# sephiroce/srf

Hardware: AMD Instinct MI355X
Metric: acoustic frames/sec through SRF (123-d fbank, 3-iter DR) at 1/2/4/8 MI355X (higher is better)
Workload: dtype fp32; 1 GPU; wsj_c4: SRF L=6 PH=CH=16 DIM=32 LPAD=RPAD=2 DR iter=3, train step (fwd+bwd+allreduce+Adam); utterances_per_gpu=28, frames_per_utterance=800, global_batch=28, parallelism=dp1, launch=hipgraph (fwd+CTC+bwd)

## Files before the change

### include/srf.h

```cpp
#ifndef SRF_H_
#define SRF_H_
#include <stddef.h>

#ifdef __cplusplus
extern "C" {
#endif

int srf_version(void);
const char* srf_last_error(void);

int srf_route_dr_auto_chunks(int B, int T, int N, int din, int lpad, int rpad, int J, int dout);
size_t srf_route_dr_saved_floats(int B, int T, int J, int dout, int iters);
size_t srf_route_dr_fwd_workspace(int B, int T, int N, int din, int lpad, int rpad, int J, int dout, int iters,
                                  int n_chunks);
size_t srf_route_dr_bwd_workspace(int B, int T, int N, int din, int lpad, int rpad, int J, int dout, int iters,
                                  int n_chunks);
int srf_route_dr_fwd(const float* emb, const float* W, const float* bias, int B, int T, int N, int din, int lpad,
                     int rpad, int J, int dout, int iters, int mask_first, int n_chunks, float* v_out,
                     float* saved, void* workspace, size_t workspace_bytes, void* stream);
size_t srf_route_dr_coupling_floats(int B, int T, int N, int din, int lpad, int rpad, int J, int dout, int iters);
int srf_route_dr_fwd_ex(const float* emb, const float* W, const float* bias, int B, int T, int N, int din, int lpad,
                        int rpad, int J, int dout, int iters, int mask_first, int n_chunks, float* v_out,
                        float* saved, float* couplings, void* workspace, size_t workspace_bytes, void* stream);
int srf_route_dr_bwd_ex(const float* emb, const float* W, const float* bias, int B, int T, int N, int din, int lpad,
                        int rpad, int J, int dout, int iters, int mask_first, int n_chunks, const float* saved,
                        const float* couplings, const float* g_v, float* g_emb, float* g_W, float* g_bias,
                        void* workspace, size_t workspace_bytes, void* stream);
int srf_route_dr_bwd_weights_ex(const float* emb, int B, int T, int N, int din, int lpad, int rpad, int J, int dout,
                                int iters, int mask_first, int n_chunks, const float* saved, const float* couplings,
                                float* g_W, float* g_bias, void* workspace, size_t workspace_bytes, void* stream);
int srf_route_dr_bwd_data_ex(const float* emb, const float* W, const float* bias, int B, int T, int N, int din,
                             int lpad, int rpad, int J, int dout, int iters, int mask_first, int n_chunks,
                             const float* saved, const float* couplings, const float* g_v, float* g_emb,
                             void* workspace, size_t workspace_bytes, void* stream);
int srf_set_seed_source(const void* step_counter);
int srf_set_fault_flag(void* flag);
int srf_route_dr_bwd(const float* emb, const float* W, const float* bias, int B, int T, int N, int din, int lpad,
                     int rpad, int J, int dout, int iters, int mask_first, int n_chunks, const float* saved,
                     const float* g_v, float* g_emb, float* g_W, float* g_bias, void* workspace,
                     size_t workspace_bytes, void* stream);
int srf_route_dr_bwd_data(const float* emb, const float* W, const float* bias, int B, int T, int N, int din,
                          int lpad, int rpad, int J, int dout, int iters, int mask_first, int n_chunks,
                          const float* saved, const float* g_v, float* g_emb, void* workspace,
                          size_t workspace_bytes, void* stream);
int srf_route_dr_bwd_weights(const float* emb, int B, int T, int N, int din, int lpad, int rpad, int J, int dout,
                             int iters, int mask_first, int n_chunks, float* g_W, float* g_bias, void* workspace,
                             size_t workspace_bytes, void* stream);

size_t srf_route_sdr_saved_floats(int B, int T, int J, int dout);
size_t srf_route_sdr_fwd_workspace(int B, int T, int N, int din, int lpad, int rpad, int J, int dout);
size_t srf_route_sdr_bwd_workspace(int B, int T, int N, int din, int lpad, int rpad, int J, int dout, int iters);
int srf_route_sdr_fwd(const float* emb, const float* W, const float* bias, int B, int T, int N, int din, int lpad,
                      int rpad, int J, int dout, int iters, int mask_first, float* v_out, float* saved,
                      void* workspace, size_t workspace_bytes, void* stream);
int srf_route_sdr_bwd(const float* emb, const float* W, const float* bias, int B, int T, int N, int din, int lpad,
                      int rpad, int J, int dout, int iters, int mask_first, const float* saved, const float* g_v,
                      float* g_emb, float* g_W, float* g_bias, void* workspace, size_t workspace_bytes,
                      void* stream);

#define SRF_SDR_MAX_ITEMS 8
typedef struct {
  int t0, t1;
  const float* emb;
  const float* W;
  const float* bias;
  const float* WT;
  float* u;
  int v0, vn;
  float* v;
  float* couplings;
  void* workspace;
  size_t workspace_bytes;
  const float* g_v;
  float* carry;
  float* gu;
  int g0, gn;
  float* g_emb;
  float* g_W;
  float* g_bias;
  int accumulate;
  int u_bf16;
  int group;
  int gu_factored;
} srf_sdr_range;
int srf_route_sdr_pose_n(const srf_sdr_range* ranges, int n, int B, int T, int N, int din, int lpad, int rpad, int J,
                         int dout, int fp8, void* stream);
int srf_route_sdr_recur_fwd_n(const srf_sdr_range* ranges, int n, int B, int T, int in_n, int J, int dout, int iters,
                              int mask_first, void* stream);
int srf_route_sdr_recur_bwd_n(const srf_sdr_range* ranges, int n, int B, int T, int in_n, int J, int dout, int iters,
                              int mask_first, void* stream);
int srf_route_sdr_gx_n(const srf_sdr_range* ranges, int n, int B, int T, int N, int din, int lpad, int rpad, int J,
                       int dout, void* stream);
int srf_route_sdr_gw_n(const srf_sdr_range* ranges, int n, int B, int T, int N, int din, int lpad, int rpad, int J,
                       int dout, void* stream);
int srf_route_sdr_gx_gw_n(const srf_sdr_range* ranges, int n, int B, int T, int N, int din, int lpad, int rpad,
                          int J, int dout, void* stream);
int srf_route_sdr_gx_gw_fact_n(const srf_sdr_range* ranges, int n, int B, int T, int N, int din, int lpad, int rpad,
                               int J, int dout, int iters, void* stream);

int srf_route_sdr_pose(const float* emb, const float* W, const float* bias, int B, int T, int N, int din, int lpad,
                       int rpad, int J, int dout, int t0, int t1, float* u, int v0, int vn, void* stream);
int srf_route_sdr_pose_fp8(const float* emb, const float* W, const float* bias, int B, int T, int N, int din, int lpad,
                           int rpad, int J, int dout, int t0, int t1, float* u, int v0, int vn, void* stream);
size_t srf_route_sdr_recur_workspace(int B, int in_n, int J, int dout, int iters);
size_t srf_route_sdr_recur_zero_range(int B, int in_n, int J, int dout, int iters, size_t* offset_bytes);
size_t srf_route_sdr_coupling_floats(int in_n, int J, int dout, int iters);
int srf_route_sdr_couplings_required(int in_n, int J, int dout, int iters);
size_t srf_route_sdr_fact_floats(int in_n, int J, int dout, int iters);
int srf_route_sdr_recur_fwd(const float* u, int v0, int vn, int B, int T, int in_n, int J, int dout, int iters,
                            int mask_first, int t0, int t1, float* v_out, float* couplings, void* workspace,
                            size_t workspace_bytes, void* stream);
int srf_route_sdr_recur_bwd(const float* u, int v0, int vn, const float* v_saved, const float* couplings,
                            const float* g_v, int B, int T, int in_n, int J, int dout, int iters, int mask_first,
                            int t0, int t1, float* carry, float* gu, int g0, int gn, void* workspace,
                            size_t workspace_bytes, void* stream);
int srf_route_sdr_transpose_w(const float* W, int in_n, int J, int dout, int din, float* WT, void* stream);
int srf_route_sdr_gx(const float* gu, int g0, int gn, const float* WT, int B, int T, int N, int din, int lpad,
                     int rpad, int J, int dout, int t0, int t1, float* g_emb, void* stream);
int srf_route_sdr_gw(const float* gu, int g0, int gn, const float* emb, int B, int T, int N, int din, int lpad,
                     int rpad, int J, int dout, int t0, int t1, int accumulate, float* g_W, float* g_bias,
                     void* stream);

int srf_cnnfe_out_dims(int T, int feat_dim, int* T2, int* F2);
size_t srf_cnnfe_saved_bytes(int B, int T, int feat_dim, int nfilt);
size_t srf_cnnfe_fwd_workspace(int B, int T, int feat_dim, int nfilt);
size_t srf_cnnfe_bwd_workspace(int B, int T, int feat_dim, int nfilt);
int srf_cnnfe_fwd(const float* feats, const int* inp_len, int B, int T, int feat_dim, int nfilt,
                  const float* k0a, const float* b0a, const float* k0b, const float* b0b, const float* gamma0,
                  const float* beta0, const float* k1a, const float* b1a, const float* k1b, const float* b1b,
                  const float* gamma1, const float* beta1, float* mmean0, float* mvar0, float* mmean1, float* mvar1,
                  int training, float drop_p, unsigned long long seed, float* out, void* saved, size_t saved_bytes,
                  void* workspace, size_t workspace_bytes, void* stream);
int srf_cnnfe_bwd(const float* feats, const int* inp_len, int B, int T, int feat_dim, int nfilt, const float* gamma0,
                  const float* k1a, const float* k1b, const float* gamma1, float drop_p, unsigned long long seed,
                  const void* saved, const float* g_out, float* g_k0a, float* g_b0a, float* g_k0b, float* g_b0b,
                  float* g_gamma0, float* g_beta0, float* g_k1a, float* g_b1a, float* g_k1b, float* g_b1b,
                  float* g_gamma1, float* g_beta1, void* workspace, size_t workspace_bytes, void* stream);

#define SRF_CNNFE_BWD_PREP 1
#define SRF_CNNFE_BWD_DATA 2
#define SRF_CNNFE_BWD_WGRAD 4
#define SRF_CNNFE_BWD_ALL 7
int srf_cnnfe_bwd_parts(int parts, const float* feats, const int* inp_len, int B, int T, int feat_dim, int nfilt,
                        const float* gamma0, const float* k1a, const float* k1b, const float* gamma1, float drop_p,
                        unsigned long long seed, const void* saved, const float* g_out, float* g_k0a, float* g_b0a,
                        float* g_k0b, float* g_b0b, float* g_gamma0, float* g_beta0, float* g_k1a, float* g_b1a,
                        float* g_k1b, float* g_b1b, float* g_gamma1, float* g_beta1, void* workspace,
                        size_t workspace_bytes, void* stream);

size_t srf_primary_caps_saved_bytes(int B, int T, int PH, int PD);
size_t srf_primary_caps_bwd_workspace(int B, int T, int K, int PH, int PD);
int srf_primary_caps_fwd(const float* X, const int* inp_len, int B, int T, int K, int PH, int PD, const float* Wp,
                         const float* bp, const float* K1, const float* b1, const float* K2, const float* b2,
                         const float* gamma, const float* beta, int training, float p_caps, float p_in,
                         unsigned long long seed, float* z, void* saved, size_t saved_bytes, void* stream);
int srf_primary_caps_bwd(const float* X, const int* inp_len, int B, int T, int K, int PH, int PD, const float* Wp,
                         const float* K1, const float* K2, const float* gamma, const float* beta, int training,
                         float p_caps, float p_in, unsigned long long seed, const void* saved, const float* g_z,
                         float* g_X, float* g_Wp, float* g_bp, float* g_K1, float* g_b1, float* g_K2, float* g_b2,
                         float* g_gamma, float* g_beta, void* workspace, size_t workspace_bytes, void* stream);
int srf_primary_caps_fwd_ex(const float* X, const int* inp_len, int B, int T, int K, int PH, int PD, const float* Wp,
                            const float* bp, const float* K1, const float* b1, const float* K2, const float* b2,
                            const float* gamma, const float* beta, int training, float p_caps, float p_in,
                            unsigned long long seed, float proj_scale, int pos_enc, float* z, void* saved,
// ... 64 lines not shown
```

### srf_amd/_lib.py

```python
import ctypes
import os

_HERE = os.path.dirname(os.path.abspath(__file__))
LIB_PATH = os.environ.get('SRF_LIB_PATH') or os.path.join(_HERE, 'libsrf.so')

_c_int, _c_size, _vp = ctypes.c_int, ctypes.c_size_t, ctypes.c_void_p

SDR_MAX_ITEMS = 8


class SdrRange(ctypes.Structure):
    _fields_ = [('t0', _c_int), ('t1', _c_int), ('emb', _vp), ('W', _vp), ('bias', _vp), ('WT', _vp),
                ('u', _vp), ('v0', _c_int), ('vn', _c_int), ('v', _vp), ('couplings', _vp),
                ('workspace', _vp), ('workspace_bytes', _c_size), ('g_v', _vp), ('carry', _vp),
                ('gu', _vp), ('g0', _c_int), ('gn', _c_int), ('g_emb', _vp), ('g_W', _vp), ('g_bias', _vp),
                ('accumulate', _c_int), ('u_bf16', _c_int), ('group', _c_int), ('gu_factored', _c_int)]


_ranges = ctypes.POINTER(SdrRange)

CAPSNORM_MAX_ITEMS = 8


class CapsnormRange(ctypes.Structure):
    _fields_ = [('t0', _c_int), ('t1', _c_int), ('layer', _c_int), ('x', _vp), ('gamma', _vp), ('beta', _vp),
                ('y', _vp), ('stat', _vp), ('g_y', _vp), ('g_x', _vp), ('gpart', _vp)]


_cn_ranges = ctypes.POINTER(CapsnormRange)

_SIGNATURES = {
    'srf_version': (_c_int, []),
    'srf_last_error': (ctypes.c_char_p, []),
    'srf_set_seed_source': (_c_int, [_vp]),
    'srf_set_fault_flag': (_c_int, [_vp]),
    'srf_route_dr_auto_chunks': (_c_int, [_c_int] * 8),
    'srf_route_dr_saved_floats': (_c_size, [_c_int] * 5),
    'srf_route_dr_fwd_workspace': (_c_size, [_c_int] * 10),
    'srf_route_dr_bwd_workspace': (_c_size, [_c_int] * 10),
    'srf_route_dr_fwd': (_c_int, [_vp, _vp, _vp] + [_c_int] * 11 + [_vp, _vp, _vp, _c_size, _vp]),
    'srf_route_dr_bwd': (_c_int, [_vp, _vp, _vp] + [_c_int] * 11 + [_vp, _vp, _vp, _vp, _vp, _vp, _c_size, _vp]),
    'srf_route_dr_bwd_data': (_c_int, [_vp, _vp, _vp] + [_c_int] * 11 + [_vp, _vp, _vp, _vp, _c_size, _vp]),
    'srf_route_dr_bwd_weights': (_c_int, [_vp] + [_c_int] * 11 + [_vp, _vp, _vp, _c_size, _vp]),
    'srf_route_dr_coupling_floats': (_c_size, [_c_int] * 9),
    'srf_route_dr_fwd_ex': (_c_int, [_vp, _vp, _vp] + [_c_int] * 11 + [_vp, _vp, _vp, _vp, _c_size, _vp]),
    'srf_route_dr_bwd_ex': (_c_int, [_vp, _vp, _vp] + [_c_int] * 11 + [_vp] * 7 + [_c_size, _vp]),
    'srf_route_dr_bwd_data_ex': (_c_int, [_vp, _vp, _vp] + [_c_int] * 11 + [_vp] * 5 + [_c_size, _vp]),
    'srf_route_dr_bwd_weights_ex': (_c_int, [_vp] + [_c_int] * 11 + [_vp] * 5 + [_c_size, _vp]),
    'srf_route_sdr_saved_floats': (_c_size, [_c_int] * 4),
    'srf_route_sdr_fwd_workspace': (_c_size, [_c_int] * 8),
    'srf_route_sdr_bwd_workspace': (_c_size, [_c_int] * 9),
    'srf_route_sdr_fwd': (_c_int, [_vp, _vp, _vp] + [_c_int] * 10 + [_vp, _vp, _vp, _c_size, _vp]),
    'srf_route_sdr_bwd': (_c_int, [_vp, _vp, _vp] + [_c_int] * 10 + [_vp, _vp, _vp, _vp, _vp, _vp, _c_size, _vp]),
    'srf_route_sdr_pose': (_c_int, [_vp, _vp, _vp] + [_c_int] * 10 + [_vp, _c_int, _c_int, _vp]),
    'srf_route_sdr_pose_fp8': (_c_int, [_vp, _vp, _vp] + [_c_int] * 10 + [_vp, _c_int, _c_int, _vp]),
    'srf_route_sdr_recur_workspace': (_c_size, [_c_int] * 5),
    'srf_route_sdr_recur_zero_range': (_c_size, [_c_int] * 5 + [ctypes.POINTER(_c_size)]),
    'srf_route_sdr_coupling_floats': (_c_size, [_c_int] * 4),
    'srf_route_sdr_couplings_required': (_c_int, [_c_int] * 4),
    'srf_route_sdr_fact_floats': (_c_size, [_c_int] * 4),
    'srf_route_sdr_recur_fwd': (_c_int, [_vp] + [_c_int] * 11 + [_vp, _vp, _vp, _c_size, _vp]),
    'srf_route_sdr_recur_bwd': (_c_int, [_vp, _c_int, _c_int, _vp, _vp, _vp] + [_c_int] * 9
                                + [_vp, _vp, _c_int, _c_int, _vp, _c_size, _vp]),
    'srf_route_sdr_transpose_w': (_c_int, [_vp] + [_c_int] * 4 + [_vp, _vp]),
    'srf_route_sdr_gx': (_c_int, [_vp, _c_int, _c_int, _vp] + [_c_int] * 10 + [_vp, _vp]),
    'srf_route_sdr_gw': (_c_int, [_vp, _c_int, _c_int, _vp] + [_c_int] * 11 + [_vp, _vp, _vp]),
    'srf_route_sdr_pose_n': (_c_int, [_ranges] + [_c_int] * 10 + [_vp]),
    'srf_route_sdr_recur_fwd_n': (_c_int, [_ranges] + [_c_int] * 8 + [_vp]),
    'srf_route_sdr_recur_bwd_n': (_c_int, [_ranges] + [_c_int] * 8 + [_vp]),
    'srf_route_sdr_gx_n': (_c_int, [_ranges] + [_c_int] * 9 + [_vp]),
    'srf_route_sdr_gw_n': (_c_int, [_ranges] + [_c_int] * 9 + [_vp]),
    'srf_route_sdr_gx_gw_n': (_c_int, [_ranges] + [_c_int] * 9 + [_vp]),
    'srf_route_sdr_gx_gw_fact_n': (_c_int, [_ranges] + [_c_int] * 10 + [_vp]),
    'srf_cnnfe_out_dims': (_c_int, [_c_int, _c_int, ctypes.POINTER(_c_int), ctypes.POINTER(_c_int)]),
    'srf_cnnfe_saved_bytes': (_c_size, [_c_int] * 4),
    'srf_cnnfe_fwd_workspace': (_c_size, [_c_int] * 4),
    'srf_cnnfe_bwd_workspace': (_c_size, [_c_int] * 4),
    'srf_cnnfe_fwd': (_c_int, [_vp, _vp] + [_c_int] * 4 + [_vp] * 16 + [_c_int, ctypes.c_float, ctypes.c_ulonglong,
                                                                       _vp, _vp, _c_size, _vp, _c_size, _vp]),
    'srf_cnnfe_bwd': (_c_int, [_vp, _vp] + [_c_int] * 4 + [_vp] * 4 + [ctypes.c_float, ctypes.c_ulonglong]
                      + [_vp] * 15 + [_c_size, _vp]),
    'srf_cnnfe_bwd_parts': (_c_int, [_c_int, _vp, _vp] + [_c_int] * 4 + [_vp] * 4 + [ctypes.c_float, ctypes.c_ulonglong]
                            + [_vp] * 15 + [_c_size, _vp]),
    'srf_primary_caps_saved_bytes': (_c_size, [_c_int] * 4),
    'srf_primary_caps_bwd_workspace': (_c_size, [_c_int] * 5),
    'srf_primary_caps_fwd': (_c_int, [_vp, _vp] + [_c_int] * 5 + [_vp] * 8 + [_c_int, ctypes.c_float, ctypes.c_float,
                                                                           ctypes.c_ulonglong, _vp, _vp, _c_size, _vp]),
    'srf_primary_caps_bwd': (_c_int, [_vp, _vp] + [_c_int] * 5 + [_vp] * 5 + [_c_int, ctypes.c_float, ctypes.c_float,
                                                                           ctypes.c_ulonglong] + [_vp] * 12
                             + [_c_size, _vp]),
    'srf_primary_caps_fwd_ex': (_c_int, [_vp, _vp] + [_c_int] * 5 + [_vp] * 8
                                + [_c_int, ctypes.c_float, ctypes.c_float, ctypes.c_ulonglong, ctypes.c_float, _c_int,
                                   _vp, _vp, _c_size, _vp]),
    'srf_primary_caps_bwd_ex': (_c_int, [_vp, _vp] + [_c_int] * 5 + [_vp] * 5
                                + [_c_int, ctypes.c_float, ctypes.c_float, ctypes.c_ulonglong, ctypes.c_float]
                                + [_vp] * 12 + [_c_size, _vp]),
    'srf_capsnorm_bwd_workspace': (_c_size, [_c_int] * 3),
    'srf_capsnorm_fwd': (_c_int, [_vp, _c_int, _c_int, _vp, _vp, _c_int, ctypes.c_float, ctypes.c_ulonglong, _c_int,
                                  _vp, _vp, _vp]),
    'srf_capsnorm_bwd': (_c_int, [_vp, _c_int, _c_int, _vp, _vp, _c_int, ctypes.c_float, ctypes.c_ulonglong, _c_int]
                         + [_vp] * 6 + [_c_size, _vp]),
    'srf_capsnorm_fwd_range_n': (_c_int, [_cn_ranges] + [_c_int] * 5 + [ctypes.c_float, ctypes.c_ulonglong, _vp]),
    'srf_capsnorm_bwd_range_n': (_c_int, [_cn_ranges] + [_c_int] * 5 + [ctypes.c_float, ctypes.c_ulonglong, _vp]),
    'srf_capsnorm_fwd_range': (_c_int, [_vp] + [_c_int] * 5 + [_vp, _vp, _c_int, ctypes.c_float, ctypes.c_ulonglong,
                                                             _c_int, _vp, _vp, _vp]),
    'srf_capsnorm_bwd_range': (_c_int, [_vp] + [_c_int] * 5 + [_vp, _vp, _c_int, ctypes.c_float, ctypes.c_ulonglong,
                                                             _c_int, _vp, _vp, _vp, _vp, _vp]),
    'srf_capsnorm_params_workspace': (_c_size, [_c_int] * 2),
    'srf_capsnorm_bwd_params': (_c_int, [_vp, _c_int, _c_int, _vp, _vp, _vp, _c_size, _vp]),
    'srf_caps_head_fwd': (_c_int, [_vp, _c_int, _c_int, _c_int] + [_vp] * 4 + [_c_int, ctypes.c_float,
                                                                              ctypes.c_ulonglong, _c_int]
                          + [_vp] * 4),
    'srf_caps_head_fwd_ex': (_c_int, [_vp, _c_int, _c_int, _c_int] + [_vp] * 4
                             + [_c_int, ctypes.c_float, ctypes.c_ulonglong, _c_int, ctypes.c_float] + [_vp] * 4),
    'srf_caps_head_bwd': (_c_int, [_vp, _c_int, _c_int, _c_int] + [_vp] * 3 + [_c_int, ctypes.c_float,
                                                                              ctypes.c_ulonglong, _c_int]
                          + [_vp] * 9 + [_c_size, _vp]),
    'srf_ctc_workspace': (_c_size, [_c_int] * 4),
    'srf_ctc_loss': (_c_int, [_vp] * 4 + [_c_int] * 5 + [ctypes.c_float, _vp, _vp, _vp, _c_size, _vp]),
    'srf_adam_step': (_c_int, [_vp, _vp, _vp, _vp, _c_size, ctypes.c_float, ctypes.c_float, ctypes.c_float,
                               ctypes.c_float, _vp]),
}

_PROF_SIGNATURES = {
    'srf_route_dr_set_timing_events': (_c_int, [_vp, _vp, _c_int]),
}


class SrfError(RuntimeError):
    pass


_lib = None


def lib():
    global _lib
    if _lib is None:
        if not os.path.exists(LIB_PATH):
            raise ImportError(f'{LIB_PATH} is missing: build it with `make -C srf_amd/csrc` '
                              '(or __graft_entry__.build()); there is no fallback path')
        import torch
        h = ctypes.CDLL(LIB_PATH)
        for name, (res, args) in list(_SIGNATURES.items()) + list(_PROF_SIGNATURES.items()):
            fn = getattr(h, name)
            fn.restype = res
            fn.argtypes = args
        _lib = h
    return _lib


def exported_symbols():
    return list(_SIGNATURES)


def prof_symbols():
    return list(_PROF_SIGNATURES)


def check(rc, what):
    if rc != 0:
        msg = lib().srf_last_error().decode(errors='replace')
        raise SrfError(f'{what} failed (rc={rc}): {msg}')
```

### srf_amd/csrc/route_dr.hip

```cpp
#include <algorithm>
#include <cmath>

#include "srf_common.h"
#include "route_fwd32.h"
#include "../../include/srf.h"
#include "../../include/srf_prof.h"

namespace {

constexpr float kSquashEps = 1e-7f;

thread_local hipEvent_t* t_ev_start = nullptr;
thread_local hipEvent_t* t_ev_stop = nullptr;
thread_local int t_ev_n = 0;
constexpr int MODE_FWD = 0;
constexpr int MODE_BWD = 1;

struct Geom {
  int B, T, N, din, lpad, rpad, J, dout, iters, mask_first;
  int F() const { return B * T; }
  int in_n() const { return N * (lpad + rpad + 1); }
  int JD() const { return J * dout; }
  int NT() const { return (J * dout + 15) / 16; }
};
// ... 1437 lines not shown
    } else {
      const int x = idx - NCPL, k = x >> 7, xr = x & 127;
      const int p = xr >> 6, e = (xr >> 1) & 31, hf = xr & 1;
      const int i = i0 + min(k, ncap - 1);
      src[q] = reinterpret_cast<const char*>(x16 + (((size_t)i * NFT * 2 + p) * 32 + e) * 16 + hf * 8);
      dst[q] = k * PCB + CG * 4 + p * (D * 16 * 2) + (e * 16 + ((hf ^ ((e >> 3) & 1)) * 8)) * 2;
      step[q] = 2 * 32 * 16 * 2;
    }
  }
  f4 sv[NQ];
  auto stage_load = [&](int ft) {
#pragma unroll
    for (int q = 0; q < NQ; ++q) sv[q] = *reinterpret_cast<const f4*>(src[q] + (size_t)ft * step[q]);
  };
  auto stage_store = [&](int buf) {
#pragma unroll
    for (int q = 0; q < NQ; ++q) {
      const int idx = q * 256 + threadIdx.x;
      if ((CAP * PQ) % 256 != 0 && idx >= CAP * PQ) continue;
      *reinterpret_cast<f4*>(&stg[buf][dst[q]]) = sv[q];
    }
  };
  const uint32_t nrec = (uint32_t)(FJD * 4);
  __amdgpu_buffer_rsrc_t rs_g[R], rs_v[RV];
#pragma unroll
  for (int r = 0; r < R; ++r) {
    rs_g[r] = __builtin_amdgcn_make_buffer_rsrc(const_cast<float*>(gs + (size_t)r * FJD), 0, (int)nrec, 0x00020000);
    if (r > 0)
      rs_v[r - 1] = __builtin_amdgcn_make_buffer_rsrc(const_cast<float*>(saved + (size_t)(2 * (r - 1) + 1) * FJD), 0,
                                                      (int)nrec, 0x00020000);
  }
  const uint32_t vo0 = (uint32_t)((8 * h) * JD + row) * 4;
  f2 nx[R + RV][4];
  auto vec_load = [&](int ft) {
#pragma unroll
    for (int v = 0; v < 8; ++v) {
      const uint32_t so = (uint32_t)((ft * 16 + v) * JD) * 4;
#pragma unroll
      for (int r = 0; r < R; ++r) {
        nx[r][v >> 1][v & 1] = __builtin_bit_cast(float, __builtin_amdgcn_raw_buffer_load_b32(rs_g[r], vo0, so, 0));
        if (r > 0) nx[R + r - 1][v >> 1][v & 1] = __builtin_bit_cast(float, __builtin_amdgcn_raw_buffer_load_b32(rs_v[r - 1], vo0, so, 0));
      }
    }
  };

  f16v acc[CAP];
  f2 gb[CAP];
#pragma unroll
  for (int k = 0; k < CAP; ++k) {
    gb[k] = f2{0.f, 0.f};
    acc[k] = f16v{};
  }
  if (ft0 < ft1) {
    stage_load(ft0);
    vec_load(ft0);
    stage_store(0);
    if (ft0 + 1 < ft1) stage_load(ft0 + 1);
  }
  const int xoff = CG * 4 + (n * 16 + ((h ^ ((n >> 3) & 1)) * 8)) * 2;
  const float s0 = c0 * sg;
  for (int ft = ft0; ft < ft1; ++ft) {
    const int buf = (ft - ft0) & 1;
    f2 fv[R + RV][4];
#pragma unroll
    for (int v = 0; v < 4; ++v) {
      fv[0][v] = nx[0][v] * s0;
#pragma unroll
      for (int a = 1; a < R + RV; ++a) fv[a][v] = nx[a][v] * sg;
    }
    __syncthreads();
    if (ft + 1 < ft1) {
      stage_store(buf ^ 1);
      if (ft + 2 < ft1) stage_load(ft + 2);
    }
    vec_load(ft + 1 < ft1 ? ft + 1 : ft);
    const unsigned char* sb = stg[buf];
#pragma unroll
    for (int k = 0; k < CAP; ++k) {
      const unsigned char* ck = sb + k * PCB;
      const float* ckf = reinterpret_cast<const float*>(ck);
      f2 gu[4];
#pragma unroll
      for (int v = 0; v < 4; ++v) gu[v] = fv[0][v];
#pragma unroll
      for (int r = 0; r < RV; ++r) {
        const float* cp = ckf + ((r * 2 + 0) * 4 + wv) * 16 + 8 * h;
        const float* gp = ckf + ((r * 2 + 1) * 4 + wv) * 16 + 8 * h;
        const f4 ca = ld4(cp), cb = ld4(cp + 4), ga = ld4(gp), gbv = ld4(gp + 4);
        const f2 c2[4] = {f2{ca[0], ca[1]}, f2{ca[2], ca[3]}, f2{cb[0], cb[1]}, f2{cb[2], cb[3]}};
        const f2 g2[4] = {f2{ga[0], ga[1]}, f2{ga[2], ga[3]}, f2{gbv[0], gbv[1]}, f2{gbv[2], gbv[3]}};
#pragma unroll
        for (int v = 0; v < 4; ++v) {
          gu[v] = __builtin_elementwise_fma(c2[v], fv[r + 1][v], gu[v]);
          gu[v] = __builtin_elementwise_fma(g2[v], fv[R + r][v], gu[v]);
        }
      }
      gb[k] += (gu[0] + gu[1]) + (gu[2] + gu[3]);
      h8 bh, bl;
#pragma unroll
      for (int v = 0; v < 4; ++v) {
        const f2 hi = __builtin_bit_cast(f2, __builtin_bit_cast(u2, gu[v]) & 0xFFFFE000u);
        const f2 lo = gu[v] - hi;
        const h2 ph = __builtin_convertvector(hi, h2);
        const h2 pl = __builtin_convertvector(lo, h2);
        bh[2 * v] = ph[0];
        bh[2 * v + 1] = ph[1];
        bl[2 * v] = pl[0];
        bl[2 * v + 1] = pl[1];
      }
      const h8 xh = *reinterpret_cast<const h8*>(ck + xoff);
      const h8 xl = *reinterpret_cast<const h8*>(ck + xoff + D * 16 * 2);
      acc[k] = mfma32h(xh, bh, acc[k]);
      acc[k] = mfma32h(xh, bl, acc[k]);
      acc[k] = mfma32h(xl, bh, acc[k]);
    }
  }
  float* gw = gwp + (size_t)s * pstride;
  float* gbo = gbp + (size_t)s * pstride;
  const float un = srf_exp2i(-(bx + eg)), ug = srf_exp2i(-eg);
#pragma unroll
  for (int k = 0; k < CAP; ++k) {
    const float a = gb[k][0] + gb[k][1];
    float pa, pb;
    xpair32(a, pa, pb);
    if (k >= ncap || !wave_on) continue;
    const int i = i0 + k;
    if (h == 0) gbo[(size_t)i * JD + row] = (pa + pb) * ug;
#pragma unroll
    for (int q = 0; q < 4; ++q)
      st4(gw + ((size_t)i * JD + row) * D + 8 * q + 4 * h,
          f4{acc[k][4 * q] * un, acc[k][4 * q + 1] * un, acc[k][4 * q + 2] * un, acc[k][4 * q + 3] * un});
  }
}

__global__ void gw_reduce_kernel(const float* __restrict__ part, int S, size_t n4, size_t stride, float* __restrict__ gW,
                                 size_t nw4, float* __restrict__ gb) {
  const size_t idx = (size_t)blockIdx.x * blockDim.x + threadIdx.x;
  if (idx >= n4) return;
  f4 a = ld4(part + idx * 4);
  for (int s = 1; s < S; ++s) a += ld4(part + (size_t)s * stride + idx * 4);
  if (idx < nw4)
    st4(gW + idx * 4, a);
  else
    st4(gb + (idx - nw4) * 4, a);
}

template <int Q>
__device__ __forceinline__ float qsum(float v) {
#pragma unroll
  for (int o = 1; o < Q; o <<= 1) v += __shfl_xor(v, o, 64);
  return v;
}

__device__ __forceinline__ f4 sum_slab4(const float* __restrict__ slab, int n, size_t FJD, size_t off) {
  f4 a = ld4(slab + off);
#pragma unroll 4
  for (int c = 1; c < n; ++c) a += ld4(slab + (size_t)c * FJD + off);
  return a;
}

template <int DOUT>
__global__ void fwd_finish_kernel(const float* __restrict__ slab, int n_chunks, size_t FJD,
                                  const float* __restrict__ vc_in, float* __restrict__ s_out,
                                  float* __restrict__ vc_out, float* __restrict__ v_out) {
  constexpr int Q = DOUT / 4;
  const size_t idx = (size_t)blockIdx.x * blockDim.x + threadIdx.x;
  const bool ok = idx < FJD / 4;
  const size_t off = (ok ? idx : 0) * 4;
  const f4 sv = sum_slab4(slab, n_chunks, FJD, off);
  const float n2 = qsum<Q>((sv.x * sv.x + sv.y * sv.y) + (sv.z * sv.z + sv.w * sv.w));
  if (!ok) return;
  const float fac = n2 / (1.f + n2) / sqrtf(n2 + kSquashEps);
  const f4 v = sv * fac;
  st4(s_out + off, sv);
  st4(vc_out + off, vc_in ? v + ld4(vc_in + off) : v);
  if (v_out) st4(v_out + off, v);
}

template <int DOUT>
__global__ void bwd_finish_kernel(const float* __restrict__ slab, int n_chunks, size_t FJD,
                                  const float* __restrict__ a_init, float* __restrict__ A,
                                  const float* __restrict__ s, float* __restrict__ gs, float* __restrict__ zero4,
                                  size_t nz4, float* __restrict__ zero1) {
  constexpr int Q = DOUT / 4;
  const size_t idx = (size_t)blockIdx.x * blockDim.x + threadIdx.x;
  if (idx < nz4) st4(zero4 + idx * 4, f4{0.f, 0.f, 0.f, 0.f});
  if (zero1 != nullptr && idx == 0) *zero1 = 0.f;
  const bool ok = idx < FJD / 4;
  const size_t off = (ok ? idx : 0) * 4;
  f4 a;
  if (a_init) {
    a = ld4(a_init + off);
    if (ok) st4(A + off, f4{0.f, 0.f, 0.f, 0.f});
  } else {
    a = ld4(A + off) + sum_slab4(slab, n_chunks, FJD, off);
    if (ok) st4(A + off, a);
  }
  const f4 sv = ld4(s + off);
  const float n2 = qsum<Q>((sv.x * sv.x + sv.y * sv.y) + (sv.z * sv.z + sv.w * sv.w));
  const float sa = qsum<Q>((sv.x * a.x + sv.y * a.y) + (sv.z * a.z + sv.w * a.w));
  if (!ok) return;
  const float rs = 1.f / sqrtf(n2 + kSquashEps);
  const float ip = 1.f / (1.f + n2);
  const float gfac = n2 * ip * rs;
  const float dg2 = 2.f * rs * ip * (ip - 0.5f * n2 / (n2 + kSquashEps)) * sa;
  st4(gs + off, a * gfac + sv * dg2);
}

struct PassCfg {
  int TW, NW;
};

PassCfg pass_cfg(const Geom& g) {
  const int NT = g.NT();
  int TW = 8;
  int NW = (NT + TW - 1) / TW;
  if (NW > 8) {
    TW = 16;
    NW = (NT + TW - 1) / TW;
  }
  return {TW, NW};
}

int auto_chunks(const Geom& g, int NW) {
  const int n_ftiles = (g.F() + 15) / 16;
  const int wg_per_cu = std::max(1, 8 / NW);
  const int slots = 256 * wg_per_cu;
  int best = 1;
  double best_cost = 1e30;
  for (int c = 1; c <= std::min(g.in_n(), 96); ++c) {
    const int rounds = (n_ftiles * c + slots - 1) / slots;
    const int len = (g.in_n() + c - 1) / c;
    double cost = (double)rounds * (len + 2);
    if (8 % c != 0 && c % 8 != 0) cost *= 1.05;
    cost *= 1.0 + 0.002 * c;
    if (cost < best_cost) {
      best_cost = cost;
      best = c;
    }
  }
  return best;
}

int check_geom(const Geom& g) {
  SRF_REQUIRE(g.B > 0 && g.T > 0 && g.N > 0 && g.J > 1, "bad shape B=%d T=%d N=%d J=%d", g.B, g.T, g.N, g.J);
  SRF_REQUIRE(g.lpad >= 0 && g.rpad >= 0, "negative window pad");
  SRF_REQUIRE(g.iters >= 1 && g.iters <= 5, "routing iterations must be in [1,5], got %d", g.iters);
  SRF_REQUIRE(g.din == 8 || g.din == 16 || g.din == 32 || g.din == 64, "unsupported in_d %d", g.din);
  SRF_REQUIRE(g.dout == g.din, "in_d (%d) != out_d (%d) is not supported", g.din, g.dout);
  SRF_REQUIRE((long long)g.F() * g.in_n() * g.JD() < (1LL << 40), "problem too large");
  return SRF_OK;
}

template <int D, int TW, int MODE>
void launch_pass(const Geom& g, int NW, int n_chunks, const float* emb, const float* W, const float* bias, int r,
                 const float* vc, const float* gsv, float* slab, float* stats, int want_acc, hipStream_t st) {
  const int n_ftiles = (g.F() + 15) / 16;
  const int chunk_len = (g.in_n() + n_chunks - 1) / n_chunks;
  const size_t shmem = (NW > 1) ? (size_t)2 * NW * 48 * sizeof(float) : 16;
  auto kern = r == 0 ? route_pass_kernel<D, D, TW, MODE, true> : route_pass_kernel<D, D, TW, MODE, false>;
  hipLaunchKernelGGL(kern, dim3(n_ftiles * n_chunks), dim3(64 * NW), shmem, st,
                     emb, W, bias, g.F(), g.T, g.N, g.lpad, g.in_n(), g.J, n_chunks, chunk_len, g.mask_first, r,
                     vc, gsv, slab, stats, want_acc);
}

template <int D, int MODE>
void dispatch_pass(const Geom& g, const PassCfg& pc, int n_chunks, const float* emb, const float* W,
                   const float* bias, int r, const float* vc, const float* gsv, float* slab, float* stats,
                   int want_acc, hipStream_t st) {
  if (pc.TW == 8)
    launch_pass<D, 8, MODE>(g, pc.NW, n_chunks, emb, W, bias, r, vc, gsv, slab, stats, want_acc, st);
  else
    launch_pass<D, 16, MODE>(g, pc.NW, n_chunks, emb, W, bias, r, vc, gsv, slab, stats, want_acc, st);
}

template <int D>
void launch_fwd_finish(const Geom& g, const float* slab, int n_chunks, const float* vc_in, float* s_out,
                       float* vc_out, float* v_out, hipStream_t st) {
  const size_t FJD = (size_t)g.F() * g.JD();
  hipLaunchKernelGGL((fwd_finish_kernel<D>), dim3((FJD / 4 + 255) / 256), dim3(256), 0, st, slab, n_chunks, FJD,
                     vc_in, s_out, vc_out, v_out);
}

template <int D>
void launch_bwd_finish(const Geom& g, const float* slab, int n_chunks, const float* a_init, float* A,
                       const float* s, float* gs, hipStream_t st, float* zero = nullptr, size_t n_zero = 0,
                       float* zero1 = nullptr) {
  const size_t FJD = (size_t)g.F() * g.JD();
  const size_t nz4 = zero ? n_zero / 4 : 0;
  const size_t n = std::max(FJD / 4, nz4);
  hipLaunchKernelGGL((bwd_finish_kernel<D>), dim3((n + 255) / 256), dim3(256), 0, st, slab, n_chunks, FJD, a_init,
                     A, s, gs, zero, nz4, zero1);
}

constexpr int gu_tw(int d) { return d >= 64 ? 4 : 2; }
constexpr int kGuNW = 4;

inline int gu_wgroups(const Geom& g) { return (g.NT() + kGuNW * gu_tw(g.dout) - 1) / (kGuNW * gu_tw(g.dout)); }
inline int padded_frames(const Geom& g) { return (g.F() + 15) / 16 * 16; }
inline int gu_window(const Geom& g) { return g.lpad + g.rpad + 1; }
inline size_t gu_lds_bytes(const Geom& g, int nw, int n_per) {
  return (size_t)nw * (15 + gu_window(g)) * gu_row_stride(n_per, g.din) * sizeof(float);
}
constexpr size_t kGuLdsMax = 64 * 1024;

int gu_n_per(const Geom& g, int nw) {
  const int base = (g.F() + 15) / 16 * gu_wgroups(g);
  const int slots = 256 * 4;
  int best = 1;
  double best_cost = 1e30;
  for (int n_per = 1; n_per <= g.N; ++n_per) {
    if (n_per > 1 && gu_lds_bytes(g, nw, n_per) > kGuLdsMax) break;
    const int chunks = (g.N + n_per - 1) / n_per;
    const int rounds = (base * chunks + slots - 1) / slots;
    const double cost = (double)rounds * (gu_window(g) * n_per + 4);
    if (cost < best_cost) {
      best_cost = cost;
      best = n_per;
    }
  }
  return best;
}

inline size_t gux16_lds_bytes(const Geom& g, int n_per) {
  return (size_t)kGux16NW * (31 + gu_window(g)) * (n_per * 32 + 4) * sizeof(float);
}
constexpr size_t kGux16LdsMax = (160 / kGux16Occ - 4) * 1024;
inline bool use_gux16(const Geom& g) {
  return g.din == 32 && g.dout == 32 && g.iters >= 2 && g.iters <= 4 &&
         gux16_lds_bytes(g, 1) <= kGux16LdsMax;
}
int gux16_n_per(const Geom& g, int jgpw) {
  const int base = (g.F() + 31) / 32 * ((g.J + kGux16NW - 1) / kGux16NW / jgpw);
  const int slots = 256 * kGux16Occ;
  int best = 1;
  double best_cost = 1e30;
  for (int n_per = 1; n_per <= g.N; ++n_per) {
    if (n_per > 1 && gux16_lds_bytes(g, n_per) > kGux16LdsMax) break;
    const int chunks = (g.N + n_per - 1) / n_per;
    const int rounds = (base * chunks + slots - 1) / slots;
    const double cost = (double)rounds * (gu_window(g) * n_per * jgpw + 4);
    if (cost < best_cost) {
      best_cost = cost;
      best = n_per;
    }
  }
  return best;
}

#ifndef SRF_GUX16_JGPW
#define SRF_GUX16_JGPW 2
#endif
template <int R>
void launch_gux16(const Geom& g, const float* WT, const float* hdr, const float* saved, const float* gs,
                  float* g_emb, const float* cst, const float* glst, int JP, float* gumax, hipStream_t st) {
  const int n_all = (g.J + kGux16NW - 1) / kGux16NW;
  const int jgpw = n_all % SRF_GUX16_JGPW == 0 ? SRF_GUX16_JGPW : 1;
  const int n_wgroups = n_all / jgpw;
  const int n_per = gux16_n_per(g, jgpw);
  const int n_chunks = (g.N + n_per - 1) / n_per;
  int grid = (g.F() + 31) / 32 * n_wgroups * n_chunks;
  if (SRF_GUX16_XCD) grid = (grid + 7) / 8 * 8;
  hipLaunchKernelGGL((route_gux16_kernel<R>), dim3(grid), dim3(64 * kGux16NW), gux16_lds_bytes(g, n_per), st, WT, hdr,
                     g.F(), g.T, g.N, g.lpad, g.in_n(), g.J, g.mask_first, n_wgroups, n_chunks, n_per, saved, gs, g_emb,
                     cst, glst, JP, gumax, jgpw);
}

template <int D, int R>
void launch_gu(const Geom& g, const float* emb, const float* W, const float* WT, const float* bias,
               const float* saved, const float* gs, const float* stats, float* gu_t, float* g_emb, hipStream_t st,
               const float* cst, const float* glst, int JP, const float* hdr = nullptr, float* gumax = nullptr) {
  if constexpr (R >= 2 && D == 32) {
    if (cst != nullptr && hdr != nullptr && gumax != nullptr && use_gux16(g)) {
      launch_gux16<R>(g, WT, hdr, saved, gs, g_emb, cst, glst, JP, gumax, st);
      return;
    }
  }
  const int n_ftiles = (g.F() + 15) / 16;
  const int n_wgroups = gu_wgroups(g);
  constexpr int TW = gu_tw(D);
  const int nw = std::min(kGuNW, (g.NT() + TW - 1) / TW);
  const int n_per = gu_n_per(g, nw);
  const int n_chunks = (g.N + n_per - 1) / n_per;
  const int nslots = 15 + gu_window(g);
  const size_t lds = gu_lds_bytes(g, nw, n_per);
  if constexpr (R >= 2 && D <= 32) {
    if (lds <= kGuLdsMax && cst != nullptr) {
      hipLaunchKernelGGL((route_gux_kernel<D, TW, R>), dim3(n_ftiles * n_wgroups * n_chunks), dim3(64 * nw), lds, st,
                         WT, g.F(), g.T, g.N, g.lpad, g.in_n(), g.J, g.mask_first, n_wgroups, n_chunks, n_per, saved,
                         gs, g_emb, nslots, cst, glst, JP);
      return;
    }
  }
  if (lds <= kGuLdsMax)
    hipLaunchKernelGGL((route_gu_kernel<D, D, TW, R, true>), dim3(n_ftiles * n_wgroups * n_chunks),
                       dim3(64 * nw), lds, st, emb, W, WT, bias, g.F(), padded_frames(g), g.T, g.N, g.lpad, g.rpad,
                       g.in_n(), g.J, g.mask_first, n_wgroups, n_chunks, n_per, saved, gs, stats, gu_t, g_emb, nslots,
                       nullptr, nullptr, 0);
  else
    hipLaunchKernelGGL((route_gu_kernel<D, D, TW, R, false>), dim3(n_ftiles * n_wgroups * n_chunks),
                       dim3(64 * nw), 0, st, emb, W, WT, bias, g.F(), padded_frames(g), g.T, g.N, g.lpad, g.rpad,
                       g.in_n(), g.J, g.mask_first, n_wgroups, n_chunks, n_per, saved, gs, stats, gu_t, g_emb, nslots,
                       nullptr, nullptr, 0);
}

template <int D>
void launch_gu_r(const Geom& g, const float* emb, const float* W, const float* WT, const float* bias,
                 const float* saved, const float* gs, const float* stats, float* gu_t, float* g_emb, hipStream_t st,
                 const float* cst = nullptr, const float* glst = nullptr, int JP = 0, const float* hdr = nullptr,
                 float* gumax = nullptr) {
  switch (g.iters) {
    case 1: launch_gu<D, 1>(g, emb, W, WT, bias, saved, gs, stats, gu_t, g_emb, st, nullptr, nullptr, 0); break;
    case 2: launch_gu<D, 2>(g, emb, W, WT, bias, saved, gs, stats, gu_t, g_emb, st, cst, glst, JP, hdr, gumax); break;
    case 3: launch_gu<D, 3>(g, emb, W, WT, bias, saved, gs, stats, gu_t, g_emb, st, cst, glst, JP, hdr, gumax); break;
    case 4: launch_gu<D, 4>(g, emb, W, WT, bias, saved, gs, stats, gu_t, g_emb, st, cst, glst, JP, hdr, gumax); break;
    default: launch_gu<D, 5>(g, emb, W, WT, bias, saved, gs, stats, gu_t, g_emb, st, cst, glst, JP, hdr, gumax); break;
  }
}


struct Gw2Plan {
  int cap, n_rt, n_cc, S, ft_per;
  size_t pstride;
};

inline int gw2_cap_rt(int d) { return d <= 16 ? 8 : (d == 32 ? 4 : 2); }

inline int gw3_cap(const Geom& g) {
  if (g.iters > 3) return 0;
  return g.din <= 16 ? 8 : g.din == 32 ? 4 : 0;
}

inline bool use_gw16s(const Geom& g) { return use_gux16(g) && g.iters <= 3; }

Gw2Plan gw2_plan(const Geom& g) {
  const bool g16 = use_gw16s(g);
  Gw2Plan p{};
  const int NT = g.NT();
  const int NCT = g16 ? 2 : (g.din + 15) / 16;
  p.n_rt = g16 ? (g.J + 3) / 4 : (NT + 3) / 4;
  p.cap = g16 ? kGw16Cap : gw3_cap(g) ? gw3_cap(g) : gw2_cap_rt(g.din);
  const int slots = g16 ? 512 : gw3_cap(g) ? 2 * 768 : 512;
  const double per_tile = g16 ? 120.0 : 200.0;
  p.n_cc = (g.in_n() + p.cap - 1) / p.cap;
  const int NFT = padded_frames(g) / 16;
  p.pstride = (size_t)g.in_n() * g.JD() * (g.din + 1);
  const int base = p.n_rt * p.n_cc;
  double best = 1e30;
  for (int S0 = 1; S0 <= NFT; ++S0) {
    const int ft_per = (NFT + S0 - 1) / S0;
    const int S = (NFT + ft_per - 1) / ft_per;
    const int rounds = (base * S + slots - 1) / slots;
    const double work = (double)rounds * ft_per * p.cap * NCT * per_tile / 2.4e9;
    const double slab = S > 1 ? 2.0 * S * p.pstride * 4 / 4e12 : 0.0;
    if (work + slab < best) {
      best = work + slab;
      p.S = S;
      p.ft_per = ft_per;
    }
  }
  return p;
}
size_t gw2_part_floats(const Geom& g) { return (size_t)gw2_plan(g).S * gw2_plan(g).pstride; }

template <int D>
int launch_gw2(const Geom& g, const Gw2Plan& p, const float* xT, const float* saved, const float* gs,
               const float* cst, const float* glst, int JP, float* gwp, float* gbp, hipStream_t st,
               const float* hdr = nullptr, const float* gumax = nullptr) {
  const int grid = p.n_rt * p.n_cc * p.S;
  if constexpr (D == 32) {
    if (use_gw16s(g)) {
      const int grid16 = SRF_GW16S_XCD ? (grid + 7) / 8 * 8 : grid;
      SRF_REQUIRE(hdr != nullptr && gumax != nullptr, "route_gw16s: needs the forward's header and the gx pass's max");
      const _Float16* x16 = reinterpret_cast<const _Float16*>(xT);
#define SRF_GW16S(R_)                                                                                              \
  hipLaunchKernelGGL((route_gw16s_kernel<R_, kGw16Cap>), dim3(grid16), dim3(256), 0, st, x16, hdr, gumax, saved, gs, \
                     cst, glst, g.F(), padded_frames(g), g.in_n(), g.J, g.mask_first, JP, p.n_rt, p.S, p.ft_per, gwp, \
                     gbp, p.pstride)
      if (g.iters == 2)
        SRF_GW16S(2);
      else
        SRF_GW16S(3);
#undef SRF_GW16S
      SRF_LAUNCH_CHECK("route_gw16s");
      return SRF_OK;
    }
  }
  if constexpr (D <= 32) {
    if (gw3_cap(g)) {
#define SRF_GW3(R_, C_)                                                                                           \
  hipLaunchKernelGGL((route_gw3_kernel<D, R_, C_>), dim3(grid), dim3(256), 0, st, xT, saved, gs, cst, glst, g.F(), \
                     padded_frames(g), g.in_n(), g.J, g.mask_first, JP, p.n_rt, p.S, p.ft_per, gwp, gbp, p.pstride)
#define SRF_GW3C(R_) \
  if (p.cap == 4) SRF_GW3(R_, 4); else SRF_GW3(R_, 8);
      switch (g.iters) {
        case 2: SRF_GW3C(2) break;
        default: SRF_GW3C(3) break;
      }
#undef SRF_GW3C
#undef SRF_GW3
      SRF_LAUNCH_CHECK("route_gw3");
      return SRF_OK;
    }
  }
#define SRF_GW2(R_)                                                                                              \
  hipLaunchKernelGGL((route_gw2_kernel<D, R_>), dim3(grid), dim3(256), 0, st, xT, saved, gs, cst, glst, g.F(),    \
                     padded_frames(g), g.in_n(), g.J, g.mask_first, JP, p.n_rt, p.n_cc, p.S, p.ft_per, gwp, gbp,   \
                     p.pstride)
  switch (g.iters) {
    case 2: SRF_GW2(2); break;
    case 3: SRF_GW2(3); break;
    case 4: SRF_GW2(4); break;
    default: SRF_GW2(5); break;
  }
#undef SRF_GW2
  SRF_LAUNCH_CHECK("route_gw2");
  return SRF_OK;
}

inline bool use_fwd32(const Geom& g) { return srf::fwd32_supported(g.din, g.dout, g.J); }

inline bool coupling_sizes_fit(const Geom& g) {
  constexpr size_t kLim = size_t(1) << 31;
  const srf::Fwd32Plan plan = srf::fwd32_plan(g.B, g.T, g.N, g.din, g.lpad, g.rpad, g.J, g.dout);
  const size_t total = srf::fwd32_cpl_layout(plan, g.F(), g.in_n(), g.din, g.dout, g.J, g.iters).total;
  return total * 4 < kLim && (size_t)g.F() * g.JD() * 4 * g.iters < kLim;
}

inline bool couplings_ok(const Geom& g) {
  if (!use_fwd32(g) || g.iters < 2 || g.din > 32) return false;
  const int TW = gu_tw(g.dout);
  const int nw = std::min(kGuNW, (g.NT() + TW - 1) / TW);
  return gu_lds_bytes(g, nw, 1) <= kGuLdsMax && coupling_sizes_fit(g);
}


template <int D>
int fwd_impl(const Geom& g, int n_chunks, const float* emb, const float* W, const float* bias, float* v_out,
             float* saved, float* couplings, float* slab, hipStream_t st) {
  const PassCfg pc = pass_cfg(g);
  const size_t FJD = (size_t)g.F() * g.JD();
  hipEvent_t* ev0 = t_ev_start;
  hipEvent_t* ev1 = t_ev_stop;
  const int nev = t_ev_n;
  t_ev_start = t_ev_stop = nullptr;
  t_ev_n = 0;
  const bool p32 = use_fwd32(g);
  srf::Fwd32Plan plan{};
  srf::Fwd32Cpl cl{};
  float* bsum = slab + (size_t)n_chunks * FJD;
  void* planes = slab;
  void* scratch = slab;
  if (p32) {
    plan = srf::fwd32_plan(g.B, g.T, g.N, g.din, g.lpad, g.rpad, g.J, g.dout, n_chunks);
    float *WT = nullptr, *xT = nullptr;
    if (couplings != nullptr) {
      cl = srf::fwd32_cpl_layout(plan, g.F(), g.in_n(), g.din, g.dout, g.J, g.iters);
      planes = couplings + cl.planes;
      WT = couplings + cl.WT;
      xT = couplings + cl.xT;
    } else {
      scratch = static_cast<char*>(static_cast<void*>(slab)) + srf::fwd32_planes_bytes(plan);
    }
    const int rc = srf::fwd32_prepare(plan, emb, W, bias, g.B, g.T, g.N, g.din, g.lpad, g.rpad, g.J, g.dout, planes,
                                      scratch, WT, xT, st, WT != nullptr && use_gux16(g),
                                      xT != nullptr && use_gw16s(g));
    if (rc) return rc;
  } else {
    const int chunk_len = (g.in_n() + n_chunks - 1) / n_chunks;
    hipLaunchKernelGGL(bias_chunk_sum_kernel, dim3((n_chunks * g.JD() + 255) / 256), dim3(256), 0, st, bias,
                       g.in_n(), g.JD(), n_chunks, chunk_len, bsum);
    SRF_LAUNCH_CHECK("bias_chunk_sum");
  }
  for (int r = 0; r < g.iters; ++r) {
    const float* vc = r > 0 ? saved + (size_t)(2 * (r - 1) + 1) * FJD : nullptr;
    if (r < nev) SRF_HIP_TRY(hipEventRecord(ev0[r], st));
    if (p32 && r == 0 && srf::fwd32_first_full_supported(plan, g.din, g.dout)) {
      const int rc = srf::fwd32_first_full(plan, planes, scratch, g.B, g.T, g.N, g.din, g.lpad, g.rpad, g.J, g.dout,
                                           g.mask_first, saved, saved + FJD, g.iters == 1 ? v_out : nullptr, st);
      if (rc) return rc;
      if (r < nev) SRF_HIP_TRY(hipEventRecord(ev1[r], st));
      continue;
    }
    if (p32) {
      float *cst = nullptr, *lzst = nullptr;
      if (couplings != nullptr && r > 0) {
        const size_t blk = (size_t)srf::fwd32_frame_stride(g.F()) * g.in_n();
        cst = couplings + cl.c + (size_t)(r - 1) * blk * (plan.JDp / g.dout);
        lzst = couplings + cl.lz + (size_t)(r - 1) * blk;
      }
      const int rc = srf::fwd32_pass(plan, r == 0, planes, scratch, g.B, g.T, g.N, g.din, g.lpad, g.rpad, g.J,
                                     g.dout, g.mask_first, vc, cst, lzst, st);
      if (rc) return rc;
    } else {
      dispatch_pass<D, MODE_FWD>(g, pc, n_chunks, emb, W, bias, r, vc, r == 0 ? bsum : nullptr, slab, nullptr, 1, st);
    }
    SRF_LAUNCH_CHECK("route_pass(fwd)");
    if (r < nev) SRF_HIP_TRY(hipEventRecord(ev1[r], st));
    launch_fwd_finish<D>(g, p32 ? srf::fwd32_slab(plan, scratch) : slab,
                         p32 ? plan.n_chunks : n_chunks, vc,
                         saved + (size_t)(2 * r) * FJD, saved + (size_t)(2 * r + 1) * FJD,
                         r == g.iters - 1 ? v_out : nullptr, st);
    SRF_LAUNCH_CHECK("fwd_finish");
  }
  return SRF_OK;
}

struct BwdWs {
  float *A, *gs, *slab, *stats, *gu_t, *xT, *WT;
  void* p32;
  float* gl;
  float* gwpart;
  float* gumax;
  size_t bytes;
};

BwdWs bwd_layout(const Geom& g, int n_chunks, void* base) {
  const size_t F = g.F(), JD = g.JD(), in_n = g.in_n(), Fp = padded_frames(g);
  size_t off = 0;
  auto take = [&](size_t nfloat) {
    size_t o = off;
    off += srf::align_up(nfloat * sizeof(float), 256);
    return o;
  };
  const size_t oA = take(F * JD), ogs = take((size_t)g.iters * F * JD), oslab = take((size_t)n_chunks * F * JD),
               ostats = take((size_t)(g.iters - 1) * F * in_n * 2), ogu = take(in_n * (size_t)g.NT() * 16 * Fp),
               oxt = take(in_n * g.din * Fp), owt = take(in_n * JD * g.din);
  size_t op32 = 0, ogl = 0, ogwp = 0;
  const size_t ogm = take(64);
  if (use_fwd32(g)) {
    const srf::Fwd32Plan plan = srf::fwd32_plan(g.B, g.T, g.N, g.din, g.lpad, g.rpad, g.J, g.dout, n_chunks);
    op32 = take((srf::fwd32_scratch_bytes(plan) + 3) / 4);
    ogl = take((size_t)std::max(g.iters - 1, 1) * srf::fwd32_frame_stride(g.F()) * in_n * (plan.JDp / g.dout));
    ogwp = take(gw2_part_floats(g));
  }
  char* b = static_cast<char*>(base);
  BwdWs w;
  w.A = (float*)(b + oA);
  w.gs = (float*)(b + ogs);
  w.slab = (float*)(b + oslab);
  w.stats = (float*)(b + ostats);
  w.gu_t = (float*)(b + ogu);
  w.xT = (float*)(b + oxt);
  w.WT = (float*)(b + owt);
  w.p32 = op32 ? (void*)(b + op32) : nullptr;
  w.gl = ogl ? (float*)(b + ogl) : nullptr;
  w.gwpart = ogwp ? (float*)(b + ogwp) : nullptr;
  w.gumax = (float*)(b + ogm);
  w.bytes = off;
  return w;
}

template <int D>
int bwd_weights_impl(const Geom& g, const float* emb, float* g_W, float* g_bias, const BwdWs& w, hipStream_t st,
                     const float* saved = nullptr, const float* couplings = nullptr) {
  const int Fp = padded_frames(g);
  if (couplings != nullptr && w.gl != nullptr && g.iters > 1) {
    const Gw2Plan p = gw2_plan(g);
    const srf::Fwd32Plan plan = srf::fwd32_plan(g.B, g.T, g.N, g.din, g.lpad, g.rpad, g.J, g.dout);
    const srf::Fwd32Cpl cl = srf::fwd32_cpl_layout(plan, g.F(), g.in_n(), g.din, g.dout, g.J, g.iters);
    const bool direct = p.S == 1;
    float* gwp = direct ? g_W : w.gwpart;
    float* gbp = direct ? g_bias : w.gwpart + (size_t)g.in_n() * g.JD() * g.din;
    int rc = launch_gw2<D>(g, p, couplings + cl.xT, saved, w.gs, couplings + cl.c, w.gl, plan.JDp / g.dout, gwp, gbp,
                           st, srf::fwd32_hdr(plan, couplings + cl.planes), w.gumax);
    if (rc || direct) return rc;
    const size_t nw4 = (size_t)g.in_n() * g.JD() * g.din / 4, n4 = p.pstride / 4;
    hipLaunchKernelGGL(gw_reduce_kernel, dim3((n4 + 255) / 256), dim3(256), 0, st, w.gwpart, p.S, n4, p.pstride, g_W,
                       nw4, g_bias);
    SRF_LAUNCH_CHECK("gw_reduce");
    return SRF_OK;
  }
  {
    SRF_REQUIRE(g.din <= 64, "window_xt tile holds din <= 64, got %d", g.din);
    const int tiles = (Fp + kXtFrames - 1) / kXtFrames;
    hipLaunchKernelGGL(window_xt_kernel, dim3(g.in_n() * tiles), dim3(256), 0, st, emb, g.F(), Fp, g.T, g.N, g.din,
                       g.lpad, g.in_n(), w.xT);
    SRF_LAUNCH_CHECK("window_xt");
  }
  {
    const int tasks = g.in_n() * g.NT();
    hipLaunchKernelGGL((route_gw_kernel<D>), dim3((tasks + 3) / 4), dim3(256), 0, st, w.gu_t, w.xT, Fp, g.in_n(),
                       g.JD(), g_W, g_bias);
    SRF_LAUNCH_CHECK("route_gw");
  }
  return SRF_OK;
}

template <int D>
int bwd_impl(const Geom& g, int n_chunks, const float* emb, const float* W, const float* bias, const float* saved,
             const float* couplings, const float* g_v, float* g_emb, float* g_W, float* g_bias, const BwdWs& w,
             hipStream_t st, bool with_weights) {
  const PassCfg pc = pass_cfg(g);
  const size_t FJD = (size_t)g.F() * g.JD();
  const int R = g.iters;
  const int Fp = padded_frames(g);
  const bool p32 = couplings != nullptr && w.p32 != nullptr && R > 1;
  const size_t n_emb = (size_t)g.F() * g.N * g.din;
  launch_bwd_finish<D>(g, nullptr, n_chunks, g_v, w.A, saved + (size_t)(2 * (R - 1)) * FJD,
                       w.gs + (size_t)(R - 1) * FJD, st, p32 ? g_emb : nullptr, n_emb, p32 ? w.gumax : nullptr);
  SRF_LAUNCH_CHECK("bwd_finish");
  srf::Fwd32Plan plan{};
  srf::Fwd32Cpl cl{};
  if (p32) {
    plan = srf::fwd32_plan(g.B, g.T, g.N, g.din, g.lpad, g.rpad, g.J, g.dout, n_chunks);
    cl = srf::fwd32_cpl_layout(plan, g.F(), g.in_n(), g.din, g.dout, g.J, g.iters);
  }
  for (int r = R - 1; r >= 1; --r) {
    const float* vc = saved + (size_t)(2 * (r - 1) + 1) * FJD;
    float* stats_r = w.stats + (size_t)(r - 1) * g.F() * g.in_n() * 2;
    if (p32) {
      const size_t blk = (size_t)srf::fwd32_frame_stride(g.F()) * g.in_n();
      const int JP = plan.JDp / g.dout;
      const int rc = srf::bwd32_pass(plan, couplings + cl.planes, w.p32, g.B, g.T, g.N, g.din, g.lpad, g.rpad, g.J,
                                     g.dout, couplings + cl.c + (size_t)(r - 1) * blk * JP,
                                     couplings + cl.lz + (size_t)(r - 1) * blk,
                                     w.gs + (size_t)r * FJD, stats_r, w.gl + (size_t)(r - 1) * blk * JP, st);
      if (rc) return rc;
      launch_bwd_finish<D>(g, srf::fwd32_slab(plan, w.p32), plan.n_chunks, nullptr, w.A,
                             saved + (size_t)(2 * (r - 1)) * FJD, w.gs + (size_t)(r - 1) * FJD, st);
    } else {
      dispatch_pass<D, MODE_BWD>(g, pc, n_chunks, emb, W, bias, r, vc, w.gs + (size_t)r * FJD, w.slab, stats_r, 1,
                                 st);
      SRF_LAUNCH_CHECK("route_pass(bwd)");
      launch_bwd_finish<D>(g, w.slab, n_chunks, nullptr, w.A, saved + (size_t)(2 * (r - 1)) * FJD,
                           w.gs + (size_t)(r - 1) * FJD, st);
    }
    SRF_LAUNCH_CHECK("bwd_finish");
  }
  if (!p32) {
    const size_t total = (size_t)g.in_n() * g.JD() * g.din + n_emb;
    hipLaunchKernelGGL(transpose_w_kernel, dim3((total + 255) / 256), dim3(256), 0, st, W, g.in_n(), g.JD(), g.din,
                       w.WT, g_emb, n_emb);
    SRF_LAUNCH_CHECK("transpose_w");
  }
  if (p32) {
    launch_gu_r<D>(g, emb, W, couplings + cl.WT, bias, saved, w.gs, w.stats, w.gu_t, g_emb, st, couplings + cl.c,
                   w.gl, plan.JDp / g.dout, srf::fwd32_hdr(plan, couplings + cl.planes), w.gumax);
  } else
    launch_gu_r<D>(g, emb, W, w.WT, bias, saved, w.gs, w.stats, w.gu_t, g_emb, st);
  SRF_LAUNCH_CHECK("route_gu");
  (void)Fp;
  return with_weights ? bwd_weights_impl<D>(g, emb, g_W, g_bias, w, st, saved, p32 ? couplings : nullptr) : SRF_OK;
}

}

extern "C" {

int srf_route_dr_set_timing_events(void* const* starts, void* const* stops, int n) {
  SRF_REQUIRE(n >= 0 && (n == 0 || (starts && stops)), "bad timing event arrays");
  t_ev_start = (hipEvent_t*)starts;
  t_ev_stop = (hipEvent_t*)stops;
  t_ev_n = n;
  return SRF_OK;
}

int srf_route_dr_auto_chunks(int B, int T, int N, int din, int lpad, int rpad, int J, int dout) {
  Geom g{B, T, N, din, lpad, rpad, J, dout, 1, 0};
  if (use_fwd32(g)) return srf::fwd32_plan(B, T, N, din, lpad, rpad, J, dout).n_chunks;
  return auto_chunks(g, pass_cfg(g).NW);
}

size_t srf_route_dr_saved_floats(int B, int T, int J, int dout, int iters) {
  return (size_t)2 * iters * B * T * J * dout;
}

size_t srf_route_dr_fwd_workspace(int B, int T, int N, int din, int lpad, int rpad, int J, int dout, int iters,
                                  int n_chunks) {
  (void)iters;
  size_t need = (size_t)n_chunks * ((size_t)B * T + 1) * J * dout * sizeof(float);
  Geom g{B, T, N, din, lpad, rpad, J, dout, 1, 0};
  if (use_fwd32(g))
    need = std::max(need, srf::fwd32_workspace(srf::fwd32_plan(B, T, N, din, lpad, rpad, J, dout, n_chunks)));
  return need;
}

size_t srf_route_dr_bwd_workspace(int B, int T, int N, int din, int lpad, int rpad, int J, int dout, int iters,
                                  int n_chunks) {
  Geom g{B, T, N, din, lpad, rpad, J, dout, iters, 0};
  return bwd_layout(g, n_chunks, nullptr).bytes;
}

size_t srf_route_dr_coupling_floats(int B, int T, int N, int din, int lpad, int rpad, int J, int dout, int iters) {
  Geom g{B, T, N, din, lpad, rpad, J, dout, iters, 0};
  if (!couplings_ok(g)) return 0;
  return srf::fwd32_cpl_layout(srf::fwd32_plan(B, T, N, din, lpad, rpad, J, dout), B * T, g.in_n(), din, dout, J, iters)
      .total;
}

int srf_route_dr_fwd(const float* emb, const float* W, const float* bias, int B, int T, int N, int din, int lpad,
                     int rpad, int J, int dout, int iters, int mask_first, int n_chunks, float* v_out, float* saved,
                     void* workspace, size_t workspace_bytes, void* stream) {
  return srf_route_dr_fwd_ex(emb, W, bias, B, T, N, din, lpad, rpad, J, dout, iters, mask_first, n_chunks, v_out,
                             saved, nullptr, workspace, workspace_bytes, stream);
}

int srf_route_dr_fwd_ex(const float* emb, const float* W, const float* bias, int B, int T, int N, int din, int lpad,
                        int rpad, int J, int dout, int iters, int mask_first, int n_chunks, float* v_out,
                        float* saved, float* couplings, void* workspace, size_t workspace_bytes, void* stream) {
  Geom g{B, T, N, din, lpad, rpad, J, dout, iters, mask_first ? 1 : 0};
  int rc = check_geom(g);
  if (rc) return rc;
  SRF_REQUIRE(emb && W && bias && v_out && saved && workspace, "null pointer argument");
  SRF_REQUIRE(n_chunks >= 1 && n_chunks <= g.in_n(), "n_chunks %d out of [1, %d]", n_chunks, g.in_n());
  const size_t need = srf_route_dr_fwd_workspace(B, T, N, din, lpad, rpad, J, dout, iters, n_chunks);
  if (workspace_bytes < need) {
    srf::set_error("forward workspace too small: %zu < %zu", workspace_bytes, need);
    return SRF_EWORKSPACE;
  }
  hipStream_t st = static_cast<hipStream_t>(stream);
  float* slab = static_cast<float*>(workspace);
  if (couplings != nullptr && !couplings_ok(g)) couplings = nullptr;
  switch (din) {
    case 8: return fwd_impl<8>(g, n_chunks, emb, W, bias, v_out, saved, couplings, slab, st);
    case 16: return fwd_impl<16>(g, n_chunks, emb, W, bias, v_out, saved, couplings, slab, st);
    case 32: return fwd_impl<32>(g, n_chunks, emb, W, bias, v_out, saved, couplings, slab, st);
    default: return fwd_impl<64>(g, n_chunks, emb, W, bias, v_out, saved, couplings, slab, st);
  }
}

namespace {
int route_dr_bwd_entry(const float* emb, const float* W, const float* bias, int B, int T, int N, int din, int lpad,
                       int rpad, int J, int dout, int iters, int mask_first, int n_chunks, const float* saved,
                       const float* couplings, const float* g_v, float* g_emb, float* g_W, float* g_bias,
                       void* workspace, size_t workspace_bytes, void* stream, bool with_weights) {
  Geom g{B, T, N, din, lpad, rpad, J, dout, iters, mask_first ? 1 : 0};
  int rc = check_geom(g);
  if (rc) return rc;
  SRF_REQUIRE(emb && W && bias && saved && g_v && g_emb && g_W && g_bias && workspace, "null pointer argument");
  SRF_REQUIRE(n_chunks >= 1 && n_chunks <= g.in_n(), "n_chunks %d out of [1, %d]", n_chunks, g.in_n());
  BwdWs w = bwd_layout(g, n_chunks, workspace);
  if (workspace_bytes < w.bytes) {
    srf::set_error("backward workspace too small: %zu < %zu", workspace_bytes, w.bytes);
    return SRF_EWORKSPACE;
  }
  hipStream_t st = static_cast<hipStream_t>(stream);
  if (couplings != nullptr && !couplings_ok(g)) couplings = nullptr;
  switch (din) {
    case 8:
      return bwd_impl<8>(g, n_chunks, emb, W, bias, saved, couplings, g_v, g_emb, g_W, g_bias, w, st, with_weights);
    case 16:
      return bwd_impl<16>(g, n_chunks, emb, W, bias, saved, couplings, g_v, g_emb, g_W, g_bias, w, st, with_weights);
    case 32:
      return bwd_impl<32>(g, n_chunks, emb, W, bias, saved, couplings, g_v, g_emb, g_W, g_bias, w, st, with_weights);
    default:
      return bwd_impl<64>(g, n_chunks, emb, W, bias, saved, couplings, g_v, g_emb, g_W, g_bias, w, st, with_weights);
  }
}
}

int srf_route_dr_bwd(const float* emb, const float* W, const float* bias, int B, int T, int N, int din, int lpad,
                     int rpad, int J, int dout, int iters, int mask_first, int n_chunks, const float* saved,
                     const float* g_v, float* g_emb, float* g_W, float* g_bias, void* workspace,
                     size_t workspace_bytes, void* stream) {
  return route_dr_bwd_entry(emb, W, bias, B, T, N, din, lpad, rpad, J, dout, iters, mask_first, n_chunks, saved,
                            nullptr, g_v, g_emb, g_W, g_bias, workspace, workspace_bytes, stream, true);
}

int srf_route_dr_bwd_ex(const float* emb, const float* W, const float* bias, int B, int T, int N, int din, int lpad,
                        int rpad, int J, int dout, int iters, int mask_first, int n_chunks, const float* saved,
                        const float* couplings, const float* g_v, float* g_emb, float* g_W, float* g_bias,
                        void* workspace, size_t workspace_bytes, void* stream) {
  return route_dr_bwd_entry(emb, W, bias, B, T, N, din, lpad, rpad, J, dout, iters, mask_first, n_chunks, saved,
                            couplings, g_v, g_emb, g_W, g_bias, workspace, workspace_bytes, stream, true);
}

int srf_route_dr_bwd_data(const float* emb, const float* W, const float* bias, int B, int T, int N, int din,
                          int lpad, int rpad, int J, int dout, int iters, int mask_first, int n_chunks,
                          const float* saved, const float* g_v, float* g_emb, void* workspace,
                          size_t workspace_bytes, void* stream) {
  float* unused = reinterpret_cast<float*>(workspace);
  return route_dr_bwd_entry(emb, W, bias, B, T, N, din, lpad, rpad, J, dout, iters, mask_first, n_chunks, saved,
                            nullptr, g_v, g_emb, unused, unused, workspace, workspace_bytes, stream, false);
}

int srf_route_dr_bwd_data_ex(const float* emb, const float* W, const float* bias, int B, int T, int N, int din,
                             int lpad, int rpad, int J, int dout, int iters, int mask_first, int n_chunks,
                             const float* saved, const float* couplings, const float* g_v, float* g_emb,
                             void* workspace, size_t workspace_bytes, void* stream) {
  float* unused = reinterpret_cast<float*>(workspace);
  return route_dr_bwd_entry(emb, W, bias, B, T, N, din, lpad, rpad, J, dout, iters, mask_first, n_chunks, saved,
                            couplings, g_v, g_emb, unused, unused, workspace, workspace_bytes, stream, false);
}

int srf_route_dr_bwd_weights(const float* emb, int B, int T, int N, int din, int lpad, int rpad, int J, int dout,
                             int iters, int mask_first, int n_chunks, float* g_W, float* g_bias, void* workspace,
                             size_t workspace_bytes, void* stream) {
  return srf_route_dr_bwd_weights_ex(emb, B, T, N, din, lpad, rpad, J, dout, iters, mask_first, n_chunks, nullptr,
                                     nullptr, g_W, g_bias, workspace, workspace_bytes, stream);
}

int srf_route_dr_bwd_weights_ex(const float* emb, int B, int T, int N, int din, int lpad, int rpad, int J, int dout,
                                int iters, int mask_first, int n_chunks, const float* saved, const float* couplings,
                                float* g_W, float* g_bias, void* workspace, size_t workspace_bytes, void* stream) {
  Geom g{B, T, N, din, lpad, rpad, J, dout, iters, mask_first ? 1 : 0};
  int rc = check_geom(g);
  if (rc) return rc;
  SRF_REQUIRE(emb && g_W && g_bias && workspace, "null pointer argument");
  SRF_REQUIRE(n_chunks >= 1 && n_chunks <= g.in_n(), "n_chunks %d out of [1, %d]", n_chunks, g.in_n());
  BwdWs w = bwd_layout(g, n_chunks, workspace);
  if (workspace_bytes < w.bytes) {
    srf::set_error("backward workspace too small: %zu < %zu", workspace_bytes, w.bytes);
    return SRF_EWORKSPACE;
  }
  hipStream_t st = static_cast<hipStream_t>(stream);
  if (couplings != nullptr && (!couplings_ok(g) || saved == nullptr)) couplings = nullptr;
  switch (din) {
    case 8: return bwd_weights_impl<8>(g, emb, g_W, g_bias, w, st, saved, couplings);
    case 16: return bwd_weights_impl<16>(g, emb, g_W, g_bias, w, st, saved, couplings);
    case 32: return bwd_weights_impl<32>(g, emb, g_W, g_bias, w, st, saved, couplings);
    default: return bwd_weights_impl<64>(g, emb, g_W, g_bias, w, st, saved, couplings);
  }
}

}
```

### srf_amd/csrc/route_fwd32.h

```cpp
#pragma once
#include <hip/hip_runtime.h>
#include <cstddef>

namespace srf {

constexpr int kFwd32TW = 4;
__host__ __device__ inline int fwd32_frame_stride(int F) { return (F + 31) / 32 * 32; }

struct Fwd32Plan {
  int NW;
  int TW;
  int JDp;
  int xpad;
  int n_chunks, chunk_len, n_ftiles;
  size_t xplane;
  size_t ws_w, ws_b, ws_x, ws_h, ws_bsum, ws_slab;
};

bool fwd32_supported(int din, int dout, int J);
Fwd32Plan fwd32_plan(int B, int T, int N, int din, int lpad, int rpad, int J, int dout, int n_chunks = 0);
size_t fwd32_planes_bytes(const Fwd32Plan& p);
size_t fwd32_scratch_bytes(const Fwd32Plan& p);
size_t fwd32_workspace(const Fwd32Plan& p);
size_t fwd32_lds(const Fwd32Plan& p);
float* fwd32_slab(const Fwd32Plan& p, void* scratch);
const float* fwd32_hdr(const Fwd32Plan& p, const void* planes);
int fwd32_prepare(const Fwd32Plan& p, const float* emb, const float* W, const float* bias, int B, int T, int N,
                  int din, int lpad, int rpad, int J, int dout, void* planes, void* scratch, float* WT, float* xT,
                  hipStream_t st, bool wt16 = false, bool xt16 = false);
int fwd32_pass(const Fwd32Plan& p, bool first, const void* planes, void* scratch, int B, int T,
               int N, int din, int lpad, int rpad, int J, int dout, int mask_first, const float* vc, float* cst,
               float* lzst, hipStream_t st);
bool fwd32_first_full_supported(const Fwd32Plan& p, int din, int dout);
int fwd32_first_full(const Fwd32Plan& p, const void* planes, void* scratch, int B, int T, int N, int din, int lpad,
                     int rpad, int J, int dout, int mask_first, float* s_out, float* vc_out, float* v_out,
                     hipStream_t st);
struct Fwd32Cpl {
  size_t c, lz, planes, WT, xT, total;
};
Fwd32Cpl fwd32_cpl_layout(const Fwd32Plan& p, int F, int in_n, int din, int dout, int J, int iters);
int bwd32_pass(const Fwd32Plan& p, const void* planes, void* scratch, int B, int T, int N, int din, int lpad,
               int rpad, int J, int dout, const float* cst, const float* lz, const float* gs, float* stats,
               float* glst, hipStream_t st);

}
```

### srf_amd/csrc/route_fwd32.hip

```cpp
#include <cmath>
#include <cstdint>
#include <cstdlib>
#include <algorithm>
#include <type_traits>

#include "srf_common.h"
#include "route_fwd32.h"


#ifndef SRF_DR_IL
#define SRF_DR_IL 1
#endif

namespace {

typedef __bf16 bf8 __attribute__((ext_vector_type(8)));
typedef __bf16 bf4 __attribute__((ext_vector_type(4)));
typedef _Float16 h8 __attribute__((ext_vector_type(8)));
typedef float f16v __attribute__((ext_vector_type(16)));

__device__ __forceinline__ f16v mfma32(const bf8& a, const bf8& b, const f16v& c) {
  return __builtin_amdgcn_mfma_f32_32x32x16_bf16(a, b, c, 0, 0, 0);
}
__device__ __forceinline__ f16v mfma32h(const h8& a, const h8& b, const f16v& c) {
  return __builtin_amdgcn_mfma_f32_32x32x16_f16(a, b, c, 0, 0, 0);
}

__device__ __forceinline__ float exp2i(int e) { return srf_exp2i(e); }
__device__ __forceinline__ int split_exp(float m) { return srf_split_exp(m); }

__device__ __forceinline__ void split3(float a, __bf16& a1, __bf16& a2, __bf16& a3) {
  a1 = (__bf16)a;
  const float r = a - (float)a1;
  a2 = (__bf16)r;
  a3 = (__bf16)(r - (float)a2);
}

__device__ __forceinline__ void split2h(float a, _Float16& a1, _Float16& a2) { srf_split2h(a, a1, a2); }

__device__ __forceinline__ void split8h(const float* __restrict__ src, bool ok, float s, _Float16* d1,
                                        _Float16* d2) {
  f4 lo = {0.f, 0.f, 0.f, 0.f}, hi = lo;
  if (ok) {
    lo = *reinterpret_cast<const f4*>(src);
    hi = *reinterpret_cast<const f4*>(src + 4);
  }
  const float v[8] = {lo.x, lo.y, lo.z, lo.w, hi.x, hi.y, hi.z, hi.w};
  h8 p1, p2;
#pragma unroll
  for (int k = 0; k < 8; ++k) {
    _Float16 a1, a2;
    split2h(v[k] * s, a1, a2);
    p1[k] = a1;
    p2[k] = a2;
  }
  *reinterpret_cast<h8*>(d1) = p1;
  *reinterpret_cast<h8*>(d2) = p2;
}

constexpr int kAbsBlocks = 128;
__global__ __launch_bounds__(256) void absmax_kernel(const float* __restrict__ a, size_t na,
                                                     const float* __restrict__ b, size_t nb, float* part) {
  const float* p = blockIdx.y ? b : a;
  const size_t n = blockIdx.y ? nb : na;
  float m = 0.f;
  const size_t stride = (size_t)gridDim.x * blockDim.x;
  size_t i = (size_t)blockIdx.x * blockDim.x + threadIdx.x;
  if ((reinterpret_cast<uintptr_t>(p) & 15) == 0) {
    const size_t n4 = n / 4;
    for (; i < n4; i += stride) {
      const f4 v = reinterpret_cast<const f4*>(p)[i];
      m = fmaxf(m, fmaxf(fmaxf(fabsf(v.x), fabsf(v.y)), fmaxf(fabsf(v.z), fabsf(v.w))));
    }
    i = n4 * 4 + (size_t)blockIdx.x * blockDim.x + threadIdx.x;
  }
  for (; i < n; i += stride) m = fmaxf(m, fabsf(p[i]));
#pragma unroll
  for (int o = 32; o >= 1; o >>= 1) m = fmaxf(m, __shfl_xor(m, o, 64));
  __shared__ float wm[4];
  if ((threadIdx.x & 63) == 0) wm[threadIdx.x >> 6] = m;
  __syncthreads();
  if (threadIdx.x == 0) part[blockIdx.y * kAbsBlocks + blockIdx.x] = fmaxf(fmaxf(wm[0], wm[1]), fmaxf(wm[2], wm[3]));
}

struct PrepArgs {
  const float *W, *bias, *emb;
  _Float16 *Ws, *xs;
  __bf16* bs;
  float *bsum, *WT, *xT;
  const float* part;
  float* hdr;
  int in_n, JD, JDp, din, n_chunks, chunk_len, F, N, T, lpad, Fp;
  int wt16;
  int xt16;
  size_t xplane;
  size_t n_a, n_b, n_c, n_d, n_e;
  size_t n_f, xt_block0;
};

constexpr int kXtTile = 64;

__global__ __launch_bounds__(256) void prep32_kernel(PrepArgs P) {
  if (P.n_f && blockIdx.x >= P.xt_block0) {
    __shared__ float tile[kXtTile][32 + 1];
    __shared__ int sbx;
    const int ntile = (P.Fp + kXtTile - 1) / kXtTile;
    const int blk = blockIdx.x - (int)P.xt_block0;
    const int i = blk / ntile, f0 = (blk - i * ntile) * kXtTile;
    const int w = i / P.N, n = i - w * P.N;
    if (P.xt16 && threadIdx.x < 64) {
      float m = 0.f;
      for (int k = threadIdx.x; k < kAbsBlocks; k += 64) m = fmaxf(m, P.part[kAbsBlocks + k]);
#pragma unroll
      for (int o = 32; o >= 1; o >>= 1) m = fmaxf(m, __shfl_xor(m, o, 64));
      if (threadIdx.x == 0) sbx = split_exp(m);
    }
    for (int k = threadIdx.x; k < kXtTile * P.din; k += blockDim.x) {
      const int fl = k / P.din, e = k - fl * P.din;
      const int f = f0 + fl;
      float v = 0.f;
      if (f < P.F) {
        const int b = f / P.T, t = f - b * P.T;
        const int ts = t + w - P.lpad;
        if (ts >= 0 && ts < P.T) v = P.emb[((size_t)(b * P.T + ts) * P.N + n) * P.din + e];
      }
      tile[fl][e] = v;
    }
    __syncthreads();
    if (P.xt16) {
      const float sc = exp2i(sbx);
      _Float16* x16 = reinterpret_cast<_Float16*>(P.xT);
      for (int k = threadIdx.x; k < (kXtTile / 16) * 32 * 2; k += blockDim.x) {
        const int hf = k & 1, e = (k >> 1) & 31, kb = k >> 6;
        const int fb = f0 + kb * 16;
        if (fb >= P.Fp) continue;
        h8 p1, p2;
#pragma unroll
        for (int q = 0; q < 8; ++q) {
          _Float16 a1, a2;
          split2h(tile[kb * 16 + hf * 8 + q][e] * sc, a1, a2);
          p1[q] = a1;
          p2[q] = a2;
        }
        const size_t base = (((size_t)i * (P.Fp / 16) + fb / 16) * 2 * 32 + e) * 16 + hf * 8;
        *reinterpret_cast<h8*>(x16 + base) = p1;
        *reinterpret_cast<h8*>(x16 + base + 32 * 16) = p2;
      }
      return;
    }
    for (int k = threadIdx.x; k < kXtTile * P.din; k += blockDim.x) {
      const int e = k / kXtTile, fl = k - e * kXtTile;
      const int f = f0 + fl;
      if (f < P.Fp) P.xT[((size_t)i * P.din + e) * P.Fp + f] = tile[fl][e];
    }
    return;
  }
  __shared__ int sexp[2];
  const size_t b0 = (size_t)blockIdx.x * blockDim.x, b1 = b0 + blockDim.x;
  const size_t ec = P.n_a + P.n_b, sd = ec + P.n_c, ed = sd + P.n_d;
  const bool split_work = b0 < ec || (b1 > sd && b0 < ed) || (P.wt16 && b1 > ed && b0 < ed + P.n_e);
  if (split_work && threadIdx.x < 128) {
    const int y = threadIdx.x >> 6, l = threadIdx.x & 63;
    float m = 0.f;
    for (int k = l; k < kAbsBlocks; k += 64) m = fmaxf(m, P.part[y * kAbsBlocks + k]);
// ... 270 lines not shown
    if constexpr (XJ) {
    } else if constexpr (XL) {
      fr.b[1] = xl_read(xl + 1 * kXlPiece);
      fr.b[3] = xl_read(xl + 3 * kXlPiece);
    } else {
      fr.b[1] = hload(rs.x, xvo, xplane_b);
      fr.b[3] = hload(rs.x, xvo, xplane_b + 32);
    }
    __builtin_amdgcn_sched_barrier(0);
#pragma unroll
    for (int t = 0; t < TW; ++t) {
      u[t] = mfma32h(fr.a[t][0], fr.b[0], u[t]);
      u[t] = mfma32h(fr.a[t][2], fr.b[2], u[t]);
    }
    __builtin_amdgcn_sched_barrier(0);
#pragma unroll
    for (int t = 0; t < TW; ++t) {
      fr.a[t][0] = hload(rs.w, wvo + t * TSTEP, wcap_b);
      fr.a[t][2] = hload(rs.w, wvo + t * TSTEP, wcap_b + 32);
    }
    if constexpr (XJ) {
    } else if constexpr (XL) {
      fr.b[0] = xl_read(xl);
      fr.b[2] = xl_read(xl + 2 * kXlPiece);
    } else {
      fr.b[0] = hload(rs.x, xvo, 0);
      fr.b[2] = hload(rs.x, xvo, 32);
    }
    __builtin_amdgcn_sched_barrier(0);
    return;
  } else if constexpr (DIN == 16) {
#pragma unroll
    for (int t = 0; t < TW; ++t) u[t] = mfma32h(fr.a[t][1], fr.b[0], u[t]);
    __builtin_amdgcn_sched_barrier(0);
    {
#pragma unroll
      for (int t = 0; t < TW; ++t) fr.a[t][1] = hload(rs.w, wvo + t * TSTEP, wcap_b + wplane_b);
    }
    __builtin_amdgcn_sched_barrier(0);
#pragma unroll
    for (int t = 0; t < TW; ++t) u[t] = mfma32h(fr.a[t][0], fr.b[1], u[t]);
    __builtin_amdgcn_sched_barrier(0);
    fr.b[1] = hload(rs.x, xvo, xplane_b);
    __builtin_amdgcn_sched_barrier(0);
  } else {
#pragma unroll
    for (int t = 0; t < TW; ++t) u[t] = mfma32h(fr.a[t][0], fr.b[1], u[t]);
    __builtin_amdgcn_sched_barrier(0);
    fr.b[1] = hload(rs.x, h ? zero_off : xvo, h ? 0u : xplane_b);
    __builtin_amdgcn_sched_barrier(0);
  }
#pragma unroll
  for (int t = 0; t < TW; ++t) u[t] = mfma32h(fr.a[t][0], fr.b[0], u[t]);
  __builtin_amdgcn_sched_barrier(0);
  {
#pragma unroll
    for (int t = 0; t < TW; ++t) fr.a[t][0] = hload(rs.w, wvo + t * TSTEP + (DIN == 8 && h ? wplane_b : 0), wcap_b);
    fr.b[0] = hload(rs.x, xvo, 0);
  }
  __builtin_amdgcn_sched_barrier(0);
}

template <int K, int V>
__device__ __forceinline__ void mfma_valu_hint() {
#pragma unroll
  for (int k = 0; k < K; ++k) {
    __builtin_amdgcn_sched_group_barrier(0x008, 1, 0);
    __builtin_amdgcn_sched_group_barrier(0x002, V, 0);
  }
}

template <int TW, int V1, int V2, int V3, class Fill>
__device__ __forceinline__ void pose_prog32i(Frags32<32, TW>& fr, const bf8& ones, f16v (&u)[TW], const Rsrc3& rs,
                                             uint32_t wvo, uint32_t bvo, uint32_t wplane_b, uint32_t wcap_b,
                                             uint32_t bcap_b, const char* xl, Fill&& fill) {
  constexpr uint32_t TSTEP = 32 * 32 * 2;
  asm volatile("s_waitcnt lgkmcnt(0)" : "+v"(fr.b[0]), "+v"(fr.b[1]), "+v"(fr.b[2]), "+v"(fr.b[3]));
  fill(std::integral_constant<int, 0>{});
#pragma unroll
  for (int t = 0; t < TW; ++t) u[t] = mfma32(fr.bias[t], ones, f16v{});
  __builtin_amdgcn_sched_barrier(0);
#pragma unroll
  for (int t = 0; t < TW; ++t) {
    const auto v2 = __builtin_amdgcn_raw_buffer_load_b64(rs.b, bvo + t * 32 * 8, bcap_b, 0);
    fr.bias[t] = __builtin_bit_cast(bf8, (unsigned __attribute__((ext_vector_type(4)))){v2[0], v2[1], 0u, 0u});
  }
  __builtin_amdgcn_sched_barrier(0);
#pragma unroll
  for (int t = 0; t < TW; ++t) {
    u[t] = mfma32h(fr.a[t][1], fr.b[0], u[t]);
    u[t] = mfma32h(fr.a[t][3], fr.b[2], u[t]);
  }
  fill(std::integral_constant<int, 1>{});
  mfma_valu_hint<2 * TW, V1>();
  __builtin_amdgcn_sched_barrier(0);
#pragma unroll
  for (int t = 0; t < TW; ++t) {
    fr.a[t][1] = hload(rs.w, wvo + t * TSTEP, wcap_b + wplane_b);
    fr.a[t][3] = hload(rs.w, wvo + t * TSTEP, wcap_b + wplane_b + 32);
  }
  __builtin_amdgcn_sched_barrier(0);
#pragma unroll
  for (int t = 0; t < TW; ++t) {
    u[t] = mfma32h(fr.a[t][0], fr.b[1], u[t]);
    u[t] = mfma32h(fr.a[t][2], fr.b[3], u[t]);
  }
  fill(std::integral_constant<int, 2>{});
  mfma_valu_hint<2 * TW, V2>();
  __builtin_amdgcn_sched_barrier(0);
  fr.b[1] = xl_read(xl + 1 * kXlPiece);
  fr.b[3] = xl_read(xl + 3 * kXlPiece);
  __builtin_amdgcn_sched_barrier(0);
#pragma unroll
  for (int t = 0; t < TW; ++t) {
    u[t] = mfma32h(fr.a[t][0], fr.b[0], u[t]);
    u[t] = mfma32h(fr.a[t][2], fr.b[2], u[t]);
  }
  fill(std::integral_constant<int, 3>{});
  mfma_valu_hint<2 * TW, V3>();
  __builtin_amdgcn_sched_barrier(0);
#pragma unroll
  for (int t = 0; t < TW; ++t) {
    fr.a[t][0] = hload(rs.w, wvo + t * TSTEP, wcap_b);
    fr.a[t][2] = hload(rs.w, wvo + t * TSTEP, wcap_b + 32);
  }
  fr.b[0] = xl_read(xl);
  fr.b[2] = xl_read(xl + 2 * kXlPiece);
  __builtin_amdgcn_sched_barrier(0);
}

__device__ __forceinline__ bf8 ones_frag(int h) {
  const __bf16 o = (__bf16)(h == 0 ? 1.f : 0.f), z = (__bf16)0.f;
  bf8 v = {o, o, o, z, z, z, z, z};
  return v;
}

template <int DOUT>
__device__ __forceinline__ constexpr int kpart(int t, int v) {
  return DOUT == 8 ? 4 * t + (v >> 2) : DOUT == 16 ? 2 * t + (v >> 3) : t;
}

struct Args32 {
  const void *Ws, *bs, *xs;
  const float* hdr;
  size_t ws_bytes, bs_bytes, xs_bytes;
  uint32_t wplane_b, xplane_b, zero_off;
  int F, T, N, lpad, in_n, J, JDp, n_chunks, chunk_len, mask_first, n_tgroups;
  const float* vc;
  const float* bsum;
  float* slab;
  float* cst;
  float* lzst;
  int JP, Fs;
};



constexpr int kFTW = 2;
constexpr int kFFB = 2;

template <int DIN>
struct FirstFrags {
  h8 a[kFTW][SplitFrags<DIN>::NA];
  h8 b[kFFB][SplitFrags<DIN>::NB];
};

template <int DIN, int DOUT>
__global__ __launch_bounds__(256) __attribute__((amdgpu_waves_per_eu(2))) void route_fwd32_first_kernel(Args32 A) {
  const int lane = threadIdx.x & 63, r = lane & 31, h = lane >> 5;
  int blk = blockIdx.x;
  {
    const int nb = gridDim.x, q = nb >> 3, rem = nb & 7, x = blk & 7, idx = blk >> 3;
    blk = (x < rem ? x * (q + 1) : rem * (q + 1) + (x - rem) * q) + idx;
  }
  const int task = blk * 4 + (threadIdx.x >> 6);
  const int nfp = (A.F + 32 * kFFB - 1) / (32 * kFFB);
  const int tg = task % A.n_tgroups;
  const int rest = task / A.n_tgroups;
  const int fp = rest % nfp, chunk = rest / nfp;
  if (chunk >= A.n_chunks) return;
  const int tbase = tg * kFTW;
  const int JD = A.J * DOUT;
  const Rsrc3 rs{make_rsrc(A.Ws, A.ws_bytes), make_rsrc(A.bs, A.bs_bytes), make_rsrc(A.xs, A.xs_bytes)};
  int f[kFFB], ftt[kFFB];
  bool fv[kFFB];
#pragma unroll
  for (int b = 0; b < kFFB; ++b) {
    f[b] = (fp * kFFB + b) * 32 + r;
    const int fc = min(f[b], A.F - 1);
    ftt[b] = fc - (fc / A.T) * A.T;
    fv[b] = f[b] < A.F;
  }
  const uint32_t wvo = (uint32_t)(((tbase * 32 + r) * DIN + (DIN >= 16 ? 8 * h : 0)) * 2);
  const int i0 = chunk * A.chunk_len, i1 = min(A.in_n, i0 + A.chunk_len);
  const uint32_t capb = (uint32_t)A.JDp * DIN * 2;
  constexpr uint32_t TSTEP = 32 * DIN * 2;
  f16v acc[kFTW][kFFB];
#pragma unroll
  for (int t = 0; t < kFTW; ++t)
#pragma unroll
    for (int b = 0; b < kFFB; ++b) acc[t][b] = f16v{};
  auto fetch = [&](int i, FirstFrags<DIN>& fr) {
#pragma unroll
    for (int b = 0; b < kFFB; ++b)
      fetch_x<DIN>(rs, x_voff<DIN>(i, A.N, A.lpad, A.T, A.F, f[b], ftt[b], fv[b], h, A.zero_off), h, A.xplane_b,
                   A.zero_off, fr.b[b]);
#pragma unroll
    for (int t = 0; t < kFTW; ++t) fetch_w<DIN>(rs, wvo + t * TSTEP, h, A.wplane_b, (uint32_t)i * capb, fr.a[t]);
  };
  auto mfmas = [&](const FirstFrags<DIN>& fr) {
#pragma unroll
    for (int t = 0; t < kFTW; ++t)
#pragma unroll
      for (int b = 0; b < kFFB; ++b) acc[t][b] = pose_chain<DIN>(fr.a[t], fr.b[b], acc[t][b]);
  };
  if (i0 < i1) {
    FirstFrags<DIN> f0, f1;
    fetch(i0, f0);
    int i = i0;
    for (; i + 1 < i1; i += 2) {
      fetch(i + 1, f1);
      mfmas(f0);
      if (i + 2 < i1) fetch(i + 2, f0);
      mfmas(f1);
    }
    if (i < i1) mfmas(f0);
  }
  const int Jeff = A.J - (A.mask_first ? 1 : 0);
  const float inv = A.hdr[0];
#pragma unroll
  for (int t = 0; t < kFTW; ++t)
#pragma unroll
    for (int q = 0; q < 4; ++q) {
      const int row = (tbase + t) * 32 + 8 * q + 4 * h;
      const int j = row / DOUT;
      const float c0 = (j < A.J && !(A.mask_first && j == 0)) ? 1.f / (float)Jeff : 0.f;
      if (row < JD) {
        const f4 bsv = *reinterpret_cast<const f4*>(A.bsum + (size_t)chunk * JD + row);
#pragma unroll
        for (int b = 0; b < kFFB; ++b) {
          if (!fv[b]) continue;
          f4 v = {acc[t][b][4 * q], acc[t][b][4 * q + 1], acc[t][b][4 * q + 2], acc[t][b][4 * q + 3]};
          *reinterpret_cast<f4*>(A.slab + ((size_t)chunk * A.F + f[b]) * JD + row) = (v * inv + bsv) * c0;
        }
      }
    }
}

constexpr int kFfBM = 128;
constexpr int kFfA = 2 * kFfBM * 64;
template <int BN>
constexpr int ff_stage() { return kFfA + 2 * BN * 64; }


__device__ __forceinline__ uint32_t ff_slot(int r, int c) { return (uint32_t)(4 * r + (c ^ ((r >> 2) & 3))); }

__device__ __forceinline__ void glds16(const void* src, char* lds_dst) {
  __builtin_amdgcn_global_load_lds((const __attribute__((address_space(1))) void*)src,
                                   (__attribute__((address_space(3))) void*)lds_dst, 16, 0, 0);
}

__device__ __forceinline__ void x_dma(const char* xs, uint32_t xplane_b, uint32_t xvo, int wv, char* dst) {
  const int q = __builtin_amdgcn_readfirstlane(wv) & 3;
  const char* base = xs + (q & 1) * xplane_b + (q >> 1) * 32;
  const uint32_t m0 = __builtin_amdgcn_readfirstlane((uint32_t)reinterpret_cast<uintptr_t>(dst + q * kXlPiece));
  asm volatile("s_mov_b32 m0, %0\n\ts_nop 0\n\tglobal_load_lds_dwordx4 %1, %2" ::"s"(m0), "v"(xvo), "s"(base)
               : "memory", "m0");
}
__device__ __forceinline__ int lane_asm() {
  int lid;
  asm volatile("v_mbcnt_lo_u32_b32 %0, -1, 0\n\tv_mbcnt_hi_u32_b32 %0, -1, %0" : "=v"(lid));
  return lid;
}
template <int K = 0>
__device__ __forceinline__ void xl_wait() {
  asm volatile("s_waitcnt vmcnt(%0)" ::"n"(K) : "memory");
}

template <int BN, int CPS = 1>
__global__ __launch_bounds__(64 * 2 * (BN / 32)) void route_fwd32_first_full_kernel(
    Args32 A, float* __restrict__ s_out, float* __restrict__ vc_out, float* __restrict__ v_out) {
  constexpr int NWF = BN / 32, NWV = 2 * NWF;
  constexpr int NPA = kFfA / 1024, NPB = 2 * BN * 64 / 1024, NP = NPA + NPB;
  constexpr int NPW = (NP + NWV - 1) / NWV;
  constexpr int BPP = BN / 16;
  constexpr int kCap = ff_stage<BN>();
  constexpr int kStage = CPS * kCap;
  extern __shared__ __attribute__((aligned(16))) char smem[];
  const int tid = threadIdx.x, lane = tid & 63, wv = tid >> 6;
  const int r32 = lane & 31, h = lane >> 5;
  const int n_rt = A.JDp / kFfBM;
  int blk = blockIdx.x;
  {
    const int nb = gridDim.x, q = nb >> 3, rem = nb & 7, x = blk & 7, idx = blk >> 3;
    blk = (x < rem ? x * (q + 1) : rem * (q + 1) + (x - rem) * q) + idx;
  }
  const int rt = blk % n_rt, ft = blk / n_rt;
  const int row0 = rt * kFfBM, f0 = ft * BN;
  const int wr = wv / NWF, wc = wv - wr * NWF;
  const char* Wb = static_cast<const char*>(A.Ws);
  const char* Xb = static_cast<const char*>(A.xs);
  const size_t capb = (size_t)A.JDp * 64;
  uint32_t src_o[NPW];
  const char* src_b[NPW];
  bool is_b[NPW], live[NPW];
  int bf_[NPW], btt[NPW];
  bool bok[NPW];
#pragma unroll
  for (int k = 0; k < NPW; ++k) {
    const int q = wv + k * NWV;
    live[k] = q < NP;
    is_b[k] = q >= NPA;
    if (!is_b[k]) {
      const int slot = (q & 7) * 64 + lane, r = slot >> 2, c = (slot & 3) ^ ((r >> 2) & 3);
      src_b[k] = Wb + (size_t)(q >> 3) * A.wplane_b;
      src_o[k] = (uint32_t)((row0 + r) * 64 + c * 16);
      bf_[k] = 0, btt[k] = 0, bok[k] = false;
    } else {
      const int qb = q - NPA;
      const int slot = (qb % BPP) * 64 + lane, r = slot >> 2, c = (slot & 3) ^ ((r >> 2) & 3);
      src_b[k] = Xb + (size_t)(qb / BPP) * A.xplane_b;
      src_o[k] = (uint32_t)(c * 16);
      bf_[k] = f0 + r;
      bok[k] = bf_[k] < A.F;
      const int fc = min(bf_[k], A.F - 1);
      btt[k] = fc - (fc / A.T) * A.T;
    }
  }
  auto stage = [&](int i0, int buf) {
#pragma unroll
    for (int c = 0; c < CPS; ++c) {
      const int i = min(i0 + c, A.in_n - 1);
      char* dst = smem + buf * kStage + c * kCap;
#pragma unroll
      for (int k = 0; k < NPW; ++k) {
        if (!live[k]) continue;
        const int q = wv + k * NWV;
        if (!is_b[k])
          glds16(src_b[k] + (size_t)i * capb + src_o[k], dst + q * 1024);
        else
          glds16(src_b[k] +
                     x_voff<32>(i, A.N, A.lpad, A.T, A.F, bf_[k], btt[k], bok[k] && i0 + c < A.in_n, 0,
                                A.zero_off) +
                     src_o[k],
                 dst + q * 1024);
      }
    }
  };
  auto afrag = [&](const char* base, int t, int plane, int sstep) -> h8 {
    const int r = wr * 64 + t * 32 + r32;
    return *reinterpret_cast<const h8*>(base + plane * (kFfBM * 64) + ff_slot(r, 2 * sstep + h) * 16);
  };
  auto bfrag = [&](const char* base, int plane, int sstep) -> h8 {
    const int r = wc * 32 + r32;
    return *reinterpret_cast<const h8*>(base + kFfA + plane * (BN * 64) + ff_slot(r, 2 * sstep + h) * 16);
  };
  f16v acc[2] = {f16v{}, f16v{}};
  const int n_in = A.in_n;
  stage(0, 0);
  for (int i = 0, buf = 0; i < n_in; i += CPS, buf ^= 1) {
    asm volatile("s_waitcnt vmcnt(0)" ::: "memory");
    __syncthreads();
    if (i + CPS < n_in) stage(i + CPS, buf ^ 1);
    auto frags = [&](const char* base, h8 (&b)[4], h8 (&a)[2][4]) {
#pragma unroll
      for (int s = 0; s < 4; ++s) b[s] = bfrag(base, s & 1, s >> 1);
#pragma unroll
      for (int t = 0; t < 2; ++t)
#pragma unroll
        for (int s = 0; s < 4; ++s) a[t][s] = afrag(base, t, s & 1, s >> 1);
    };
    auto pose2 = [&](const h8 (&a)[2][4], const h8 (&b)[4]) {
      constexpr int ka[6] = {1, 3, 0, 2, 0, 2}, kb[6] = {0, 2, 1, 3, 0, 2};
#pragma unroll
      for (int k = 0; k < 6; ++k)
#pragma unroll
        for (int t = 0; t < 2; ++t) acc[t] = mfma32h(a[t][ka[k]], b[kb[k]], acc[t]);
    };
    const char* base0 = smem + buf * kStage;
    h8 b0[4], a0[2][4];
    frags(base0, b0, a0);
    if constexpr (CPS == 2) {
      h8 b1[4], a1[2][4];
      __builtin_amdgcn_sched_barrier(0);
      frags(base0 + kCap, b1, a1);
      pose2(a0, b0);
#pragma unroll
      for (int k = 0; k < 12; ++k) {
        __builtin_amdgcn_sched_group_barrier(0x008, 1, 0);
        __builtin_amdgcn_sched_group_barrier(0x100, 1, 0);
      }
      __builtin_amdgcn_sched_barrier(0);
      pose2(a1, b1);
    } else {
      pose2(a0, b0);
    }
  }
  const int f = f0 + wc * 32 + r32;
  const bool fv = f < A.F;
  const int JD = A.J * 32;
  const int Jeff = A.J - (A.mask_first ? 1 : 0);
  const float inv = A.hdr[0];
#pragma unroll
  for (int t = 0; t < 2; ++t) {
    const int rbase = row0 + wr * 64 + t * 32;
    const int j = rbase / 32;
    const float c0 = (j < A.J && !(A.mask_first && j == 0)) ? 1.f / (float)Jeff : 0.f;
    f4 sv[4];
    float n2 = 0.f;
#pragma unroll
    for (int q = 0; q < 4; ++q) {
      const int row = rbase + 8 * q + 4 * h;
      f4 bs = {0.f, 0.f, 0.f, 0.f};
      if (row < JD)
        for (int ch = 0; ch < A.n_chunks; ++ch) bs += *reinterpret_cast<const f4*>(A.bsum + (size_t)ch * JD + row);
      const f4 u = {acc[t][4 * q], acc[t][4 * q + 1], acc[t][4 * q + 2], acc[t][4 * q + 3]};
      sv[q] = (u * inv + bs) * c0;
      n2 += (sv[q].x * sv[q].x + sv[q].y * sv[q].y) + (sv[q].z * sv[q].z + sv[q].w * sv[q].w);
    }
    n2 = xor32_sum(n2);
    const float fac = n2 / (1.f + n2) / sqrtf(n2 + 1e-7f);
    if (fv && rbase < JD) {
#pragma unroll
      for (int q = 0; q < 4; ++q) {
        const size_t o = (size_t)f * JD + rbase + 8 * q + 4 * h;
        *reinterpret_cast<f4*>(s_out + o) = sv[q];
        const f4 v = sv[q] * fac;
        *reinterpret_cast<f4*>(vc_out + o) = v;
        if (v_out) *reinterpret_cast<f4*>(v_out + o) = v;
      }
    }
  }
}

template <int DIN, int DOUT, int NW, int TW>
__global__ __launch_bounds__(64 * NW) __attribute__((amdgpu_waves_per_eu(kWavesPerEU))) void route_fwd32_kernel(Args32 A) {
  constexpr int CP = TW * 32 / DOUT;
  constexpr int OWN = CP / 2;
  extern __shared__ __attribute__((aligned(16))) float lds[];
  const int JD = A.J * DOUT;
  const int lane = threadIdx.x & 63, wv = threadIdx.x >> 6;
  const int wvu = __builtin_amdgcn_readfirstlane(wv);
  const int r = lane & 31, h = lane >> 5;
  const int bid = blockIdx.x;
  const int ft = bid / A.n_chunks, chunk = bid - ft * A.n_chunks;
  const int f = ft * 32 + r;
  const int fc = min(f, A.F - 1);
  const int fb = fc / A.T, ftt = fc - fb * A.T;
  const bool fvalid = f < A.F;
  const int i0 = chunk * A.chunk_len, i1 = min(A.in_n, i0 + A.chunk_len);
  const int tbase = __builtin_amdgcn_readfirstlane(wv * TW);
  const int j0 = tbase * 32 / DOUT;
  const Rsrc3 rs{make_rsrc(A.Ws, A.ws_bytes), make_rsrc(A.bs, A.bs_bytes), make_rsrc(A.xs, A.xs_bytes)};
  if (DIN <= 16 && NW > 1 && wv >= NW / 2) __builtin_amdgcn_s_setprio(1);
  const uint32_t wvo = (uint32_t)(((tbase * 32 + r) * DIN + (DIN >= 16 ? 8 * h : 0)) * 2);
  const uint32_t bvo = (uint32_t)((tbase * 32 + r) * 8);
  const __amdgpu_buffer_rsrc_t crs = make_rsrc(A.cst, A.cst ? (size_t)A.in_n * A.JP * A.Fs * 4 : 0);
  const __amdgpu_buffer_rsrc_t lzs = make_rsrc(A.lzst, A.cst ? (size_t)A.in_n * A.Fs * 4 : 0);

  f4* vcl = reinterpret_cast<f4*>(lds) + (size_t)wv * TW * 4 * 64;
  float2* st = reinterpret_cast<float2*>(lds + (size_t)NW * TW * 4 * 64 * 4);
  constexpr bool XJ = DIN == 32 && NW > 1;
  __shared__ __attribute__((aligned(16))) char xls[XJ ? 2 * 4 * kXlPiece : 16];
  const char* xs_b = static_cast<const char*>(A.xs);
  auto xsrc = [&](int c) { return x_voff<DIN>(min(c, i1 - 1), A.N, A.lpad, A.T, A.F, f, ftt, fvalid, h, A.zero_off); };
  auto xbuf = [&](int c) { return xls + (c & 1) * 4 * kXlPiece; };
#pragma unroll
  for (int t = 0; t < TW; ++t)
#pragma unroll
    for (int q = 0; q < 4; ++q) {
      const int row = (tbase + t) * 32 + 8 * q + 4 * h;
      f4 v = {0.f, 0.f, 0.f, 0.f};
      if (fvalid && row < JD) v = *reinterpret_cast<const f4*>(A.vc + (size_t)f * JD + row);
      vcl[(t * 4 + q) * 64 + lane] = v;
    }
  float mk[OWN];
#pragma unroll
  for (int a = 0; a < OWN; ++a) {
    const int j = j0 + 2 * a + h;
    mk[a] = (j < A.J && !(A.mask_first && j == 0)) ? 0.f : -INFINITY;
  }
  const bf8 ones = ones_frag(h);
  const float inv = A.hdr[0];
  f16v acc[TW];
#pragma unroll
  for (int t = 0; t < TW; ++t) acc[t] = f16v{};
  int par = 0;
  if (i0 < i1) {
    Frags32<DIN, TW> fr;
    fetch32<DIN, TW, true>(rs, wvo, bvo, x_voff<DIN>(i0, A.N, A.lpad, A.T, A.F, f, ftt, fvalid, h, A.zero_off), h,
                           A.wplane_b, A.xplane_b, A.zero_off, (uint32_t)i0 * A.JDp * DIN * 2, (uint32_t)i0 * A.JDp * 8,
                           fr);
    if constexpr (XJ) {
      x_dma(xs_b, A.xplane_b, xsrc(i0), wv, xbuf(i0));
      x_dma(xs_b, A.xplane_b, xsrc(i0 + 1), wv, xbuf(i0 + 1));
      xl_wait();
      __syncthreads();
    }
    for (int i = i0; i < i1; ++i) {
      f16v u[TW];
      f2 P2[CP];
#pragma unroll
      for (int k = 0; k < CP; ++k) P2[k] = f2{0.f, 0.f};
      if constexpr (DIN <= 16) {
      {
        constexpr uint32_t TSTEP = 32 * DIN * 2;
        const int in = min(i + 1, i1 - 1);
        const uint32_t wcap = (uint32_t)in * A.JDp * DIN * 2, bcap = (uint32_t)in * A.JDp * 8;
        const uint32_t xvn = x_voff<DIN>(in, A.N, A.lpad, A.T, A.F, f, ftt, fvalid, h, A.zero_off);
        f4 vv[4];
        auto dots = [&](int t) {
#pragma unroll
          for (int q = 0; q < 4; ++q) {
            const int k = kpart<DOUT>(t, 4 * q);
            P2[k] += f2{u[t][4 * q], u[t][4 * q + 1]} * f2{vv[q].x, vv[q].y};
            P2[k] += f2{u[t][4 * q + 2], u[t][4 * q + 3]} * f2{vv[q].z, vv[q].w};
          }
        };
#pragma unroll
        for (int t = 0; t < TW; ++t) {
          if (t > 0) {
#pragma unroll
            for (int q = 0; q < 4; ++q) vv[q] = vcl[((t - 1) * 4 + q) * 64 + lane];
          }
          __builtin_amdgcn_sched_barrier(0);
          u[t] = pose_chain<DIN>(fr.a[t], fr.b, mfma32(fr.bias[t], ones, f16v{}));
          __builtin_amdgcn_sched_barrier(0);
          fetch_w<DIN>(rs, wvo + t * TSTEP, h, A.wplane_b, wcap, fr.a[t]);
          {
            const auto v2 = __builtin_amdgcn_raw_buffer_load_b64(rs.b, bvo + t * 32 * 8, bcap, 0);
            fr.bias[t] = __builtin_bit_cast(bf8, (unsigned __attribute__((ext_vector_type(4)))){v2[0], v2[1], 0u, 0u});
          }
          if (t == TW - 1) fetch_x<DIN>(rs, xvn, h, A.xplane_b, A.zero_off, fr.b);
          __builtin_amdgcn_sched_barrier(0);
          if (t > 0) dots(t - 1);
          __builtin_amdgcn_sched_barrier(0);
        }
#pragma unroll
        for (int q = 0; q < 4; ++q) vv[q] = vcl[((TW - 1) * 4 + q) * 64 + lane];
        dots(TW - 1);
      }
      } else {
      const int in = min(i + 1, i1 - 1);
      pose_prog<DIN, TW, XJ, XJ>(fr, ones, u, rs, wvo, bvo,
                                 x_voff<DIN>(in, A.N, A.lpad, A.T, A.F, f, ftt, fvalid, h, A.zero_off), h,
                                 A.wplane_b, A.xplane_b, A.zero_off, (uint32_t)in * A.JDp * DIN * 2,
                                 (uint32_t)in * A.JDp * 8, xbuf(i) + lane * 16);
#pragma unroll
      for (int t = 0; t < TW; ++t)
#pragma unroll
        for (int q = 0; q < 4; ++q) {
          const f4 vv = vcl[(t * 4 + q) * 64 + lane];
          const int k = kpart<DOUT>(t, 4 * q);
          P2[k] += f2{u[t][4 * q], u[t][4 * q + 1]} * f2{vv.x, vv.y};
          P2[k] += f2{u[t][4 * q + 2], u[t][4 * q + 3]} * f2{vv.z, vv.w};
        }
      }
      float L[OWN], e[OWN];
      float m = -1e30f;
#pragma unroll
      for (int a = 0; a < OWN; ++a) {
        const float pa = P2[2 * a].x + P2[2 * a].y, pb = P2[2 * a + 1].x + P2[2 * a + 1].y;
        const auto sw = __builtin_amdgcn_permlane32_swap(__float_as_uint(pa), __float_as_uint(pb), false, false);
        L[a] = (__uint_as_float(sw[0]) + __uint_as_float(sw[1])) * inv + mk[a];
        m = fmaxf(m, L[a]);
      }
      float z = 0.f;
#pragma unroll
      for (int a = 0; a < OWN; ++a) {
        e[a] = __expf(L[a] - m);
        z += e[a];
      }
      float M, Z;
      {
        float m0, m1, z0, z1;
        xpair32(m, m0, m1);
        xpair32(z, z0, z1);
        M = fmaxf(m0, m1);
        Z = z0 * __expf(m0 - M) + z1 * __expf(m1 - M);
      }
      if constexpr (NW > 1) {
        int lid;
        asm volatile("v_mbcnt_lo_u32_b32 %0, -1, 0\n\tv_mbcnt_hi_u32_b32 %0, -1, %0" : "=v"(lid));
        const int sr = lid & 31, sh = lid >> 5;
        float2* slot = st + par * NW * 32;
        if (sh == 0) slot[wvu * 32 + sr] = make_float2(M, Z);
        if constexpr (XJ) xl_wait<5 * TW + OWN + 1>();
        __syncthreads();
        if constexpr (XJ) x_dma(xs_b, A.xplane_b, xsrc(i + 2), wv, xbuf(i + 2));
        constexpr int HW = NW / 2;
        float2 sv[HW];
#pragma unroll
        for (int w = 0; w < HW; ++w) sv[w] = slot[(sh * HW + w) * 32 + sr];
        float mh = sv[0].x;
#pragma unroll
        for (int w = 1; w < HW; ++w) mh = fmaxf(mh, sv[w].x);
        float zh = 0.f;
#pragma unroll
        for (int w = 0; w < HW; ++w) zh += sv[w].y * __expf(sv[w].x - mh);
        float m0, m1, z0, z1;
        xpair32(mh, m0, m1);
        xpair32(zh, z0, z1);
        const float MM = fmaxf(m0, m1);
        Z = z0 * __expf(m0 - MM) + z1 * __expf(m1 - MM);
        M = MM;
        par ^= 1;
      }
      __builtin_amdgcn_sched_barrier(0);
      const float sc = __expf(m - M) * __builtin_amdgcn_rcpf(Z);
      {
#pragma unroll
        for (int a = 0; a < OWN; ++a)
          bstore(crs, fvalid ? e[a] * sc : 0.f, (uint32_t)((j0 + h + 2 * a) * A.Fs + f) * 4u,
                 (uint32_t)i * A.JP * A.Fs * 4u);
        bstore(lzs, M + __builtin_amdgcn_logf(Z) * 0.69314718f, (h == 0 && wv == 0 && fvalid) ? (uint32_t)f * 4u : kNoStore,
               (uint32_t)i * A.Fs * 4u);
      }
      float c[CP];
#pragma unroll
      for (int a = 0; a < OWN; ++a) {
        float c0, c1;
        xpair32(e[a] * sc, c0, c1);
        c[2 * a] = c0;
        c[2 * a + 1] = c1;
      }
#pragma unroll
      for (int t = 0; t < TW; ++t)
#pragma unroll
        for (int v = 0; v < 16; v += 2) {
          const float cv = c[kpart<DOUT>(t, v)];
          f2 a2 = {acc[t][v], acc[t][v + 1]};
          a2 += f2{cv, cv} * f2{u[t][v], u[t][v + 1]};
          acc[t][v] = a2.x;
          acc[t][v + 1] = a2.y;
        }
    }
  }
#pragma unroll
  for (int t = 0; t < TW; ++t)
#pragma unroll
    for (int q = 0; q < 4; ++q) {
      const int row = (tbase + t) * 32 + 8 * q + 4 * h;
      if (fvalid && row < JD) {
        f4 v = {acc[t][4 * q], acc[t][4 * q + 1], acc[t][4 * q + 2], acc[t][4 * q + 3]};
        *reinterpret_cast<f4*>(A.slab + ((size_t)chunk * A.F + f) * JD + row) = v * inv;
      }
    }
}


template <int DIN, int DOUT, int NW, int TW>
__global__ __launch_bounds__(64 * NW) __attribute__((amdgpu_waves_per_eu(kWavesPerEU))) void route_fwd32p_kernel(Args32 A) {
  constexpr int CP = TW * 32 / DOUT;
  constexpr int OWN = CP / 2;
  static_assert(NW > 1, "the pipelined pass exchanges softmax stats between waves");
  extern __shared__ __attribute__((aligned(16))) float lds[];
  const int JD = A.J * DOUT;
  const int lane = threadIdx.x & 63, wv = threadIdx.x >> 6;
  const int r = lane & 31, h = lane >> 5;
  const int bid = blockIdx.x;
  const int ft = bid / A.n_chunks, chunk = bid - ft * A.n_chunks;
  const int f = ft * 32 + r;
  const int fc = min(f, A.F - 1);
  const int fb = fc / A.T, ftt = fc - fb * A.T;
  const bool fvalid = f < A.F;
  const int i0 = chunk * A.chunk_len, i1 = min(A.in_n, i0 + A.chunk_len);
  const int tbase = __builtin_amdgcn_readfirstlane(wv * TW);
  const int j0 = tbase * 32 / DOUT;
  const Rsrc3 rs{make_rsrc(A.Ws, A.ws_bytes), make_rsrc(A.bs, A.bs_bytes), make_rsrc(A.xs, A.xs_bytes)};
  const uint32_t wvo = (uint32_t)(((tbase * 32 + r) * DIN + (DIN >= 16 ? 8 * h : 0)) * 2);
  const uint32_t bvo = (uint32_t)((tbase * 32 + r) * 8);
  const __amdgpu_buffer_rsrc_t crs = make_rsrc(A.cst, A.cst ? (size_t)A.in_n * A.JP * A.Fs * 4 : 0);
  const __amdgpu_buffer_rsrc_t lzs = make_rsrc(A.lzst, A.cst ? (size_t)A.in_n * A.Fs * 4 : 0);
  float2* st = reinterpret_cast<float2*>(lds);
  constexpr bool XL = DIN == 32;
  f4 vcr[TW][4];
  __shared__ __attribute__((aligned(16))) char xls[XL ? 2 * 4 * kXlPiece : 16];
  char* xb = xls;
  const char* xs_b = static_cast<const char*>(A.xs);
  auto xsrc = [&](int c) { return x_voff<DIN>(min(c, i1 - 1), A.N, A.lpad, A.T, A.F, f, ftt, fvalid, h, A.zero_off); };
  auto xbuf = [&](int c) { return xb + (c & 1) * 4 * kXlPiece; };
#pragma unroll
  for (int t = 0; t < TW; ++t)
#pragma unroll
    for (int q = 0; q < 4; ++q) {
      const int row = (tbase + t) * 32 + 8 * q + 4 * h;
      f4 v = {0.f, 0.f, 0.f, 0.f};
      if (fvalid && row < JD) v = *reinterpret_cast<const f4*>(A.vc + (size_t)f * JD + row);
      vcr[t][q] = v;
    }
  float mk[OWN];
#pragma unroll
  for (int a = 0; a < OWN; ++a) {
    const int j = j0 + 2 * a + h;
    mk[a] = (j < A.J && !(A.mask_first && j == 0)) ? 0.f : -INFINITY;
  }
  const bf8 ones = ones_frag(h);
  const float inv = A.hdr[0];
  f16v acc[TW];
#pragma unroll
  for (int t = 0; t < TW; ++t) acc[t] = f16v{};
  if (i0 < i1) {
    Frags32<DIN, TW> fr;
    fetch32<DIN, TW, true>(rs, wvo, bvo, x_voff<DIN>(i0, A.N, A.lpad, A.T, A.F, f, ftt, fvalid, h, A.zero_off), h,
                           A.wplane_b, A.xplane_b, A.zero_off, (uint32_t)i0 * A.JDp * DIN * 2, (uint32_t)i0 * A.JDp * 8,
                           fr);
    f16v uc[TW], un[TW];
    float e[OWN], m;
    if constexpr (XL) {
      x_dma(xs_b, A.xplane_b, xsrc(i0 + 1), wv, xbuf(i0 + 1));
      x_dma(xs_b, A.xplane_b, xsrc(i0 + 2), wv, xbuf(i0 + 2));
      xl_wait();
      __syncthreads();
    }
    auto logits = [&](const f16v (&u)[TW], int slot_par) {
      f2 P2[CP];
#pragma unroll
      for (int k = 0; k < CP; ++k) P2[k] = f2{0.f, 0.f};
#pragma unroll
      for (int t = 0; t < TW; ++t)
#pragma unroll
        for (int q = 0; q < 4; ++q) {
          const f4 vv = vcr[t][q];
          const int k = kpart<DOUT>(t, 4 * q);
          P2[k] += f2{u[t][4 * q], u[t][4 * q + 1]} * f2{vv.x, vv.y};
          P2[k] += f2{u[t][4 * q + 2], u[t][4 * q + 3]} * f2{vv.z, vv.w};
        }
      float L[OWN];
      m = -1e30f;
#pragma unroll
      for (int a = 0; a < OWN; ++a) {
        const float pa = P2[2 * a].x + P2[2 * a].y, pb = P2[2 * a + 1].x + P2[2 * a + 1].y;
        const auto sw = __builtin_amdgcn_permlane32_swap(__float_as_uint(pa), __float_as_uint(pb), false, false);
        L[a] = (__uint_as_float(sw[0]) + __uint_as_float(sw[1])) * inv + mk[a];
        m = fmaxf(m, L[a]);
      }
      float z = 0.f;
#pragma unroll
      for (int a = 0; a < OWN; ++a) {
        e[a] = __expf(L[a] - m);
        z += e[a];
      }
      float m0, m1, z0, z1;
      xpair32(m, m0, m1);
      xpair32(z, z0, z1);
      const float M = fmaxf(m0, m1);
      const float Z = z0 * __expf(m0 - M) + z1 * __expf(m1 - M);
      if (h == 0) st[(slot_par * NW + wv) * 32 + r] = make_float2(M, Z);
    };
    int par = 0;
    pose_prog<DIN, TW, XL>(fr, ones, uc, rs, wvo, bvo,
                           x_voff<DIN>(min(i0 + 1, i1 - 1), A.N, A.lpad, A.T, A.F, f, ftt, fvalid, h, A.zero_off), h,
                           A.wplane_b, A.xplane_b, A.zero_off, (uint32_t)min(i0 + 1, i1 - 1) * A.JDp * DIN * 2,
                           (uint32_t)min(i0 + 1, i1 - 1) * A.JDp * 8, xbuf(i0 + 1) + lane * 16);
    logits(uc, par);
    __syncthreads();
    auto step_il = [&](int i, f16v (&ucur)[TW], f16v (&unext)[TW]) __attribute__((always_inline)) {
      if constexpr (DIN == 32) {
      const bool more = i + 1 < i1;
      x_dma(xs_b, A.xplane_b, xsrc(i + 3), wv, xbuf(i + 3));
      constexpr int HW = NW / 2;
      float2 sv[HW];
      float M, Z, sc;
      float c[CP];
      auto cfma = [&](int t0, int t1) __attribute__((always_inline)) {
#pragma unroll
        for (int t = t0; t < t1; ++t) {
#pragma unroll
          for (int v = 0; v < 16; ++v) acc[t][v] = fmaf(c[kpart<DOUT>(t, v)], ucur[t][v], acc[t][v]);
          asm volatile("" : "+v"(acc[t]));
        }
      };
      auto fill = [&](auto stage) __attribute__((always_inline)) {
        constexpr int S = decltype(stage)::value;
        if constexpr (S == 0) {
          const float2* slot = st + par * NW * 32;
#pragma unroll
          for (int w = 0; w < HW; ++w) sv[w] = slot[(h * HW + w) * 32 + r];
        } else if constexpr (S == 1) {
          float mh = sv[0].x;
#pragma unroll
          for (int w = 1; w < HW; ++w) mh = fmaxf(mh, sv[w].x);
          float zh = 0.f;
#pragma unroll
          for (int w = 0; w < HW; ++w) zh += sv[w].y * __expf(sv[w].x - mh);
          float m0, m1, z0, z1;
          xpair32(mh, m0, m1);
          xpair32(zh, z0, z1);
          M = fmaxf(m0, m1);
          Z = z0 * __expf(m0 - M) + z1 * __expf(m1 - M);
          sc = __expf(m - M) * __builtin_amdgcn_rcpf(Z);
        } else if constexpr (S == 2) {
#pragma unroll
          for (int a = 0; a < OWN; ++a)
            bstore(crs, fvalid ? e[a] * sc : 0.f, (uint32_t)((j0 + h + 2 * a) * A.Fs + f) * 4u,
                   (uint32_t)i * A.JP * A.Fs * 4u);
          bstore(lzs, M + __builtin_amdgcn_logf(Z) * 0.69314718f,
                 (h == 0 && wv == 0 && fvalid) ? (uint32_t)f * 4u : kNoStore, (uint32_t)i * A.Fs * 4u);
#pragma unroll
          for (int a = 0; a < OWN; ++a) {
            float c0, c1;
            xpair32(e[a] * sc, c0, c1);
            c[2 * a] = c0;
            c[2 * a + 1] = c1;
          }
          cfma(0, TW / 2);
        } else {
          cfma(TW / 2, TW);
        }
      };
      {
        const int in = min(i + 2, i1 - 1);
        pose_prog32i<TW, 6, 6, 5>(fr, ones, unext, rs, wvo, bvo, A.wplane_b, (uint32_t)in * A.JDp * DIN * 2,
                                  (uint32_t)in * A.JDp * 8, xbuf(i + 2) + lane * 16, fill);
      }
      if (more) {
        par ^= 1;
        logits(unext, par);
        xl_wait<5 * TW + OWN + 1>();
        __syncthreads();
      }
      }
    };
    auto step = [&](int i, f16v (&ucur)[TW], f16v (&unext)[TW]) __attribute__((always_inline)) {
      const bool more = i + 1 < i1;
      if constexpr (XL)
        x_dma(xs_b, A.xplane_b, xsrc(i + 3), wv, xbuf(i + 3));
      if (more) {
        const int in = min(i + 2, i1 - 1);
        pose_prog<DIN, TW, XL>(fr, ones, unext, rs, wvo, bvo,
                               x_voff<DIN>(in, A.N, A.lpad, A.T, A.F, f, ftt, fvalid, h, A.zero_off), h, A.wplane_b,
                               A.xplane_b, A.zero_off, (uint32_t)in * A.JDp * DIN * 2, (uint32_t)in * A.JDp * 8,
                               xbuf(i + 2) + lane * 16);
      }
      float M, Z;
      {
        constexpr int HW = NW / 2;
        const float2* slot = st + par * NW * 32;
        float2 sv[HW];
#pragma unroll
        for (int w = 0; w < HW; ++w) sv[w] = slot[(h * HW + w) * 32 + r];
        float mh = sv[0].x;
#pragma unroll
        for (int w = 1; w < HW; ++w) mh = fmaxf(mh, sv[w].x);
        float zh = 0.f;
#pragma unroll
        for (int w = 0; w < HW; ++w) zh += sv[w].y * __expf(sv[w].x - mh);
        float m0, m1, z0, z1;
        xpair32(mh, m0, m1);
        xpair32(zh, z0, z1);
        M = fmaxf(m0, m1);
        Z = z0 * __expf(m0 - M) + z1 * __expf(m1 - M);
      }
      const float sc = __expf(m - M) * __builtin_amdgcn_rcpf(Z);
#pragma unroll
      for (int a = 0; a < OWN; ++a)
        bstore(crs, fvalid ? e[a] * sc : 0.f, (uint32_t)((j0 + h + 2 * a) * A.Fs + f) * 4u,
               (uint32_t)i * A.JP * A.Fs * 4u);
      bstore(lzs, M + __builtin_amdgcn_logf(Z) * 0.69314718f, (h == 0 && wv == 0 && fvalid) ? (uint32_t)f * 4u : kNoStore,
             (uint32_t)i * A.Fs * 4u);
      float c[CP];
#pragma unroll
      for (int a = 0; a < OWN; ++a) {
        float c0, c1;
        xpair32(e[a] * sc, c0, c1);
        c[2 * a] = c0;
        c[2 * a + 1] = c1;
      }
#pragma unroll
      for (int t = 0; t < TW; ++t)
#pragma unroll
        for (int v = 0; v < 16; v += 2) {
          const float cv = c[kpart<DOUT>(t, v)];
          f2 a2 = {acc[t][v], acc[t][v + 1]};
          a2 += f2{cv, cv} * f2{ucur[t][v], ucur[t][v + 1]};
          acc[t][v] = a2.x;
          acc[t][v + 1] = a2.y;
        }
      if (more) {
        par ^= 1;
        logits(unext, par);
        if constexpr (XL) xl_wait<5 * TW + OWN + 1>();
        __syncthreads();
      }
    };
    if constexpr (XL && SRF_DR_IL) {
      for (int i = i0; i < i1; i += 2) {
        step_il(i, uc, un);
        if (i + 1 < i1) step_il(i + 1, un, uc);
      }
    } else {
      for (int i = i0; i < i1; i += 2) {
        step(i, uc, un);
        if (i + 1 < i1) step(i + 1, un, uc);
      }
    }
    if constexpr (XL) xl_wait();
  }
#pragma unroll
  for (int t = 0; t < TW; ++t)
#pragma unroll
    for (int q = 0; q < 4; ++q) {
      const int row = (tbase + t) * 32 + 8 * q + 4 * h;
      if (fvalid && row < JD) {
        f4 v = {acc[t][4 * q], acc[t][4 * q + 1], acc[t][4 * q + 2], acc[t][4 * q + 3]};
        *reinterpret_cast<f4*>(A.slab + ((size_t)chunk * A.F + f) * JD + row) = v * inv;
      }
    }
}

struct Bwd32Args {
  const float* cst;
  const float* lz;
  const float* gs;
  float* stats;
  float* glst;
};

template <int OWN>
__device__ __forceinline__ void load_c(const float* __restrict__ p, size_t fs, float (&c)[OWN]) {
#pragma unroll
  for (int a = 0; a < OWN; ++a) c[a] = p[2 * a * fs];
}

template <int DIN, int DOUT, int NW, int TW>
__global__ __launch_bounds__(64 * NW) __attribute__((amdgpu_waves_per_eu(kWavesPerEU))) void route_bwd32_kernel(
    Args32 A, Bwd32Args Bk) {
  constexpr int CP = TW * 32 / DOUT;
  constexpr int OWN = CP / 2;
  extern __shared__ __attribute__((aligned(16))) float lds[];
  const int JD = A.J * DOUT;
  const int lane = threadIdx.x & 63, wv = threadIdx.x >> 6;
  const int wvu = __builtin_amdgcn_readfirstlane(wv);
  const int r = lane & 31, h = lane >> 5;
  const int bid = blockIdx.x;
  const int ft = bid / A.n_chunks, chunk = bid - ft * A.n_chunks;
  const int f = ft * 32 + r;
  const int fc = min(f, A.F - 1);
  const int fb = fc / A.T, ftt = fc - fb * A.T;
  const bool fvalid = f < A.F;
  const int i0 = chunk * A.chunk_len, i1 = min(A.in_n, i0 + A.chunk_len);
  const int tbase = __builtin_amdgcn_readfirstlane(wv * TW);
  const int j0 = tbase * 32 / DOUT;
  const Rsrc3 rs{make_rsrc(A.Ws, A.ws_bytes), make_rsrc(A.bs, A.bs_bytes), make_rsrc(A.xs, A.xs_bytes)};
  if (DIN <= 16 && NW > 1 && wv >= NW / 2) __builtin_amdgcn_s_setprio(1);
  const uint32_t wvo = (uint32_t)(((tbase * 32 + r) * DIN + (DIN >= 16 ? 8 * h : 0)) * 2);
  const uint32_t bvo = (uint32_t)((tbase * 32 + r) * 8);
  const __amdgpu_buffer_rsrc_t lzr = make_rsrc(Bk.lz, (size_t)A.in_n * A.Fs * 4);

  f4* gsl = reinterpret_cast<f4*>(lds) + (size_t)wv * TW * 4 * 64;
  float* st = lds + (size_t)NW * TW * 4 * 64 * 4;
  constexpr bool XJ = DIN == 32 && NW > 1;
  __shared__ __attribute__((aligned(16))) char xls[XJ ? 2 * 4 * kXlPiece : 16];
  const char* xs_b = static_cast<const char*>(A.xs);
  auto xsrc = [&](int c) { return x_voff<DIN>(min(c, i1 - 1), A.N, A.lpad, A.T, A.F, f, ftt, fvalid, h, A.zero_off); };
  auto xbuf = [&](int c) { return xls + (c & 1) * 4 * kXlPiece; };
#pragma unroll
  for (int t = 0; t < TW; ++t)
#pragma unroll
    for (int q = 0; q < 4; ++q) {
      const int row = (tbase + t) * 32 + 8 * q + 4 * h;
      f4 v = {0.f, 0.f, 0.f, 0.f};
      if (fvalid && row < JD) v = *reinterpret_cast<const f4*>(Bk.gs + (size_t)f * JD + row);
      gsl[(t * 4 + q) * 64 + lane] = v;
    }
  const bf8 ones = ones_frag(h);
  const float inv = A.hdr[0];
  f16v acc[TW];
#pragma unroll
  for (int t = 0; t < TW; ++t) acc[t] = f16v{};
  const float* crow = Bk.cst + (size_t)(j0 + h) * A.Fs + fc;
  const __amdgpu_buffer_rsrc_t sts = make_rsrc(Bk.stats, (size_t)A.F * A.in_n * 8);
  const size_t cstep = (size_t)A.JP * A.Fs;
  int par = 0;
  if (i0 < i1) {
    Frags32<DIN, TW> fr;
    fetch32<DIN, TW, true>(rs, wvo, bvo, x_voff<DIN>(i0, A.N, A.lpad, A.T, A.F, f, ftt, fvalid, h, A.zero_off), h,
                           A.wplane_b, A.xplane_b, A.zero_off, (uint32_t)i0 * A.JDp * DIN * 2, (uint32_t)i0 * A.JDp * 8,
                           fr);
    if constexpr (XJ) {
      x_dma(xs_b, A.xplane_b, xsrc(i0), wv, xbuf(i0));
      x_dma(xs_b, A.xplane_b, xsrc(i0 + 1), wv, xbuf(i0 + 1));
      xl_wait();
      __syncthreads();
    }
    for (int i = i0; i < i1; ++i) {
      f16v u[TW];
      f2 P2[CP];
#pragma unroll
      for (int k = 0; k < CP; ++k) P2[k] = f2{0.f, 0.f};
      float cc[OWN];
      if constexpr (DIN <= 16) {
      load_c<OWN>(crow + (size_t)i * cstep, A.Fs, cc);
      {
        constexpr uint32_t TSTEP = 32 * DIN * 2;
        const int in = min(i + 1, i1 - 1);
        const uint32_t wcap = (uint32_t)in * A.JDp * DIN * 2, bcap = (uint32_t)in * A.JDp * 8;
        const uint32_t xvn = x_voff<DIN>(in, A.N, A.lpad, A.T, A.F, f, ftt, fvalid, h, A.zero_off);
        f4 gq[4];
        auto dots = [&](int t) {
#pragma unroll
          for (int q = 0; q < 4; ++q) {
            const int k = kpart<DOUT>(t, 4 * q);
            P2[k] += f2{u[t][4 * q], u[t][4 * q + 1]} * f2{gq[q].x, gq[q].y};
            P2[k] += f2{u[t][4 * q + 2], u[t][4 * q + 3]} * f2{gq[q].z, gq[q].w};
          }
        };
#pragma unroll
        for (int t = 0; t < TW; ++t) {
          if (t > 0) {
#pragma unroll
            for (int q = 0; q < 4; ++q) gq[q] = gsl[((t - 1) * 4 + q) * 64 + lane];
          }
          __builtin_amdgcn_sched_barrier(0);
          u[t] = pose_chain<DIN>(fr.a[t], fr.b, mfma32(fr.bias[t], ones, f16v{}));
          __builtin_amdgcn_sched_barrier(0);
          fetch_w<DIN>(rs, wvo + t * TSTEP, h, A.wplane_b, wcap, fr.a[t]);
          {
            const auto v2 = __builtin_amdgcn_raw_buffer_load_b64(rs.b, bvo + t * 32 * 8, bcap, 0);
            fr.bias[t] = __builtin_bit_cast(bf8, (unsigned __attribute__((ext_vector_type(4)))){v2[0], v2[1], 0u, 0u});
          }
          if (t == TW - 1) fetch_x<DIN>(rs, xvn, h, A.xplane_b, A.zero_off, fr.b);
          __builtin_amdgcn_sched_barrier(0);
          if (t > 0) dots(t - 1);
          __builtin_amdgcn_sched_barrier(0);
        }
#pragma unroll
        for (int q = 0; q < 4; ++q) gq[q] = gsl[((TW - 1) * 4 + q) * 64 + lane];
        dots(TW - 1);
      }
      } else {
      const int in = min(i + 1, i1 - 1);
      pose_prog<DIN, TW, XJ, XJ>(fr, ones, u, rs, wvo, bvo,
                                 x_voff<DIN>(in, A.N, A.lpad, A.T, A.F, f, ftt, fvalid, h, A.zero_off), h,
                                 A.wplane_b, A.xplane_b, A.zero_off, (uint32_t)in * A.JDp * DIN * 2,
                                 (uint32_t)in * A.JDp * 8, xbuf(i) + lane_asm() * 16);
      load_c<OWN>(crow + (size_t)i * cstep, A.Fs, cc);
#pragma unroll
      for (int t = 0; t < TW; ++t)
#pragma unroll
        for (int q = 0; q < 4; ++q) {
          const f4 gv = gsl[(t * 4 + q) * 64 + lane];
          const int k = kpart<DOUT>(t, 4 * q);
          P2[k] += f2{u[t][4 * q], u[t][4 * q + 1]} * f2{gv.x, gv.y};
          P2[k] += f2{u[t][4 * q + 2], u[t][4 * q + 3]} * f2{gv.z, gv.w};
        }
      }
      float Q[OWN];
      float sp = 0.f;
#pragma unroll
      for (int a = 0; a < OWN; ++a) {
        const float pa = P2[2 * a].x + P2[2 * a].y, pb = P2[2 * a + 1].x + P2[2 * a + 1].y;
        const auto sw = __builtin_amdgcn_permlane32_swap(__float_as_uint(pa), __float_as_uint(pb), false, false);
        Q[a] = (__uint_as_float(sw[0]) + __uint_as_float(sw[1])) * inv;
        sp += cc[a] * Q[a];
      }
      float S;
      {
        float s0, s1;
        xpair32(sp, s0, s1);
        S = s0 + s1;
      }
      if constexpr (NW > 1) {
        int lid;
        asm volatile("v_mbcnt_lo_u32_b32 %0, -1, 0\n\tv_mbcnt_hi_u32_b32 %0, -1, %0" : "=v"(lid));
        const int sr = lid & 31, shf = lid >> 5;
        float* slot = st + par * NW * 32;
        if (shf == 0) slot[wvu * 32 + sr] = S;
        if constexpr (XJ) xl_wait();
        __syncthreads();
        if constexpr (XJ) x_dma(xs_b, A.xplane_b, xsrc(i + 2), wv, xbuf(i + 2));
        constexpr int HW = NW / 2;
        float sh = 0.f;
#pragma unroll
        for (int w = 0; w < HW; ++w) sh += slot[(shf * HW + w) * 32 + sr];
        float s0, s1;
        xpair32(sh, s0, s1);
        S = s0 + s1;
        par ^= 1;
      }
      const float lzv =
          __builtin_bit_cast(float, __builtin_amdgcn_raw_buffer_load_b32(lzr, (uint32_t)fc * 4u, (uint32_t)i * A.Fs * 4u, 0));
      __builtin_amdgcn_sched_barrier(0);
      {
        __builtin_amdgcn_raw_buffer_store_b64(
            (unsigned __attribute__((ext_vector_type(2)))){__float_as_uint(lzv), __float_as_uint(S)}, sts,
            (wv == 0 && h == 0 && fvalid) ? (uint32_t)(f * A.in_n) * 8u : kNoStore, (uint32_t)i * 8u, 0);
      }
      float gown[OWN];
#pragma unroll
      for (int a = 0; a < OWN; ++a) gown[a] = cc[a] * (Q[a] - S);
      {
        float* dst = Bk.glst + ((size_t)i * A.JP + j0 + h) * A.Fs + f;
#pragma unroll
        for (int a = 0; a < OWN; ++a) dst[(size_t)2 * a * A.Fs] = fvalid ? gown[a] : 0.f;
      }
      float g[CP];
#pragma unroll
      for (int a = 0; a < OWN; ++a) {
        float g0, g1;
        xpair32(gown[a], g0, g1);
        g[2 * a] = g0;
        g[2 * a + 1] = g1;
      }
#pragma unroll
      for (int t = 0; t < TW; ++t)
#pragma unroll
        for (int v = 0; v < 16; v += 2) {
          const float gv = g[kpart<DOUT>(t, v)];
          f2 a2 = {acc[t][v], acc[t][v + 1]};
          a2 += f2{gv, gv} * f2{u[t][v], u[t][v + 1]};
          acc[t][v] = a2.x;
          acc[t][v + 1] = a2.y;
        }
    }
  }
#pragma unroll
  for (int t = 0; t < TW; ++t)
#pragma unroll
    for (int q = 0; q < 4; ++q) {
      const int row = (tbase + t) * 32 + 8 * q + 4 * h;
      if (fvalid && row < JD) {
        f4 v = {acc[t][4 * q], acc[t][4 * q + 1], acc[t][4 * q + 2], acc[t][4 * q + 3]};
        *reinterpret_cast<f4*>(A.slab + ((size_t)chunk * A.F + f) * JD + row) = v * inv;
      }
    }
}


template <int DIN, int DOUT, int NW, int TW>
__global__ __launch_bounds__(64 * NW) __attribute__((amdgpu_waves_per_eu(kWavesPerEU))) void route_bwd32p_kernel(
    Args32 A, Bwd32Args Bk) {
  constexpr int CP = TW * 32 / DOUT;
  constexpr int OWN = CP / 2;
  static_assert(NW > 1, "the pipelined pass exchanges sigma partials between waves");
  extern __shared__ __attribute__((aligned(16))) float lds[];
  const int JD = A.J * DOUT;
  const int lane = threadIdx.x & 63, wv = threadIdx.x >> 6;
  const int r = lane & 31, h = lane >> 5;
  const int bid = blockIdx.x;
  const int ft = bid / A.n_chunks, chunk = bid - ft * A.n_chunks;
  const int f = ft * 32 + r;
  const int fc = min(f, A.F - 1);
  const int fb = fc / A.T, ftt = fc - fb * A.T;
  const bool fvalid = f < A.F;
  const int i0 = chunk * A.chunk_len, i1 = min(A.in_n, i0 + A.chunk_len);
  const int tbase = __builtin_amdgcn_readfirstlane(wv * TW);
  const int j0 = tbase * 32 / DOUT;
  const Rsrc3 rs{make_rsrc(A.Ws, A.ws_bytes), make_rsrc(A.bs, A.bs_bytes), make_rsrc(A.xs, A.xs_bytes)};
  const uint32_t wvo = (uint32_t)(((tbase * 32 + r) * DIN + (DIN >= 16 ? 8 * h : 0)) * 2);
  const uint32_t bvo = (uint32_t)((tbase * 32 + r) * 8);
  f4* gsl = reinterpret_cast<f4*>(lds) + (size_t)wv * TW * 4 * 64;
  float* st = lds + (size_t)NW * TW * 4 * 64 * 4;
  constexpr bool XL = DIN == 32;
  __shared__ __attribute__((aligned(16))) char xls[XL ? 2 * 4 * kXlPiece : 16];
  char* xb = xls;
  const char* xs_b = static_cast<const char*>(A.xs);
  auto xsrc = [&](int c) { return x_voff<DIN>(min(c, i1 - 1), A.N, A.lpad, A.T, A.F, f, ftt, fvalid, h, A.zero_off); };
  auto xbuf = [&](int c) { return xb + (c & 1) * 4 * kXlPiece; };
#pragma unroll
  for (int t = 0; t < TW; ++t)
#pragma unroll
    for (int q = 0; q < 4; ++q) {
      const int row = (tbase + t) * 32 + 8 * q + 4 * h;
      f4 v = {0.f, 0.f, 0.f, 0.f};
      if (fvalid && row < JD) v = *reinterpret_cast<const f4*>(Bk.gs + (size_t)f * JD + row);
      gsl[(t * 4 + q) * 64 + lane] = v;
    }
  const bf8 ones = ones_frag(h);
  const float inv = A.hdr[0];
  f16v acc[TW];
#pragma unroll
  for (int t = 0; t < TW; ++t) acc[t] = f16v{};
  const float* crow = Bk.cst + (size_t)(j0 + h) * A.Fs + fc;
  const __amdgpu_buffer_rsrc_t sts = make_rsrc(Bk.stats, (size_t)A.F * A.in_n * 8);
  const size_t cstep = (size_t)A.JP * A.Fs;
  if (i0 < i1) {
    Frags32<DIN, TW> fr;
    fetch32<DIN, TW, true>(rs, wvo, bvo, x_voff<DIN>(i0, A.N, A.lpad, A.T, A.F, f, ftt, fvalid, h, A.zero_off), h,
                           A.wplane_b, A.xplane_b, A.zero_off, (uint32_t)i0 * A.JDp * DIN * 2, (uint32_t)i0 * A.JDp * 8,
                           fr);
    f16v uc[TW], un[TW];
    float cc[OWN], cn[OWN], Q[OWN];
    auto dots = [&](const f16v (&u)[TW], const float (&c)[OWN], int slot_par) {
      f2 P2[CP];
#pragma unroll
      for (int k = 0; k < CP; ++k) P2[k] = f2{0.f, 0.f};
#pragma unroll
      for (int t = 0; t < TW; ++t)
#pragma unroll
        for (int q = 0; q < 4; ++q) {
          const f4 gv = gsl[(t * 4 + q) * 64 + lane];
          const int k = kpart<DOUT>(t, 4 * q);
          P2[k] += f2{u[t][4 * q], u[t][4 * q + 1]} * f2{gv.x, gv.y};
          P2[k] += f2{u[t][4 * q + 2], u[t][4 * q + 3]} * f2{gv.z, gv.w};
        }
      float sp = 0.f;
#pragma unroll
      for (int a = 0; a < OWN; ++a) {
        const float pa = P2[2 * a].x + P2[2 * a].y, pb = P2[2 * a + 1].x + P2[2 * a + 1].y;
        const auto sw = __builtin_amdgcn_permlane32_swap(__float_as_uint(pa), __float_as_uint(pb), false, false);
        Q[a] = (__uint_as_float(sw[0]) + __uint_as_float(sw[1])) * inv;
        sp += c[a] * Q[a];
      }
      float s0, s1;
      xpair32(sp, s0, s1);
      if (h == 0) st[(slot_par * NW + wv) * 32 + r] = s0 + s1;
    };
    int par = 0;
    if constexpr (XL) {
      x_dma(xs_b, A.xplane_b, xsrc(i0 + 1), wv, xbuf(i0 + 1));
      x_dma(xs_b, A.xplane_b, xsrc(i0 + 2), wv, xbuf(i0 + 2));
      xl_wait();
      __syncthreads();
    }
    load_c<OWN>(crow + (size_t)i0 * cstep, A.Fs, cc);
    pose_prog<DIN, TW, XL>(fr, ones, uc, rs, wvo, bvo,
                           x_voff<DIN>(min(i0 + 1, i1 - 1), A.N, A.lpad, A.T, A.F, f, ftt, fvalid, h, A.zero_off), h,
                           A.wplane_b, A.xplane_b, A.zero_off, (uint32_t)min(i0 + 1, i1 - 1) * A.JDp * DIN * 2,
                           (uint32_t)min(i0 + 1, i1 - 1) * A.JDp * 8, xbuf(i0 + 1) + lane * 16);
    dots(uc, cc, par);
    __syncthreads();
    auto step_il = [&](int i, f16v (&ucur)[TW], f16v (&unext)[TW], float (&ccur)[OWN], float (&cnext)[OWN])
        __attribute__((always_inline)) {
      if constexpr (DIN == 32) {
      const bool more = i + 1 < i1;
      x_dma(xs_b, A.xplane_b, xsrc(i + 3), wv, xbuf(i + 3));
      const float lzv = Bk.lz[(size_t)i * A.Fs + fc];
      load_c<OWN>(crow + (size_t)min(i + 1, i1 - 1) * cstep, A.Fs, cnext);
      constexpr int HW = NW / 2;
      float sv[HW];
      float g[CP];
      auto gfma = [&](int t0, int t1) __attribute__((always_inline)) {
#pragma unroll
        for (int t = t0; t < t1; ++t) {
#pragma unroll
          for (int v = 0; v < 16; ++v) acc[t][v] = fmaf(g[kpart<DOUT>(t, v)], ucur[t][v], acc[t][v]);
          asm volatile("" : "+v"(acc[t]));
        }
      };
      auto fill = [&](auto stage) __attribute__((always_inline)) {
        constexpr int S = decltype(stage)::value;
        if constexpr (S == 0) {
          const float* slot = st + par * NW * 32;
#pragma unroll
          for (int w = 0; w < HW; ++w) sv[w] = slot[(h * HW + w) * 32 + r];
        } else if constexpr (S == 1) {
          float sh = 0.f;
#pragma unroll
          for (int w = 0; w < HW; ++w) sh += sv[w];
          float s0, s1;
          xpair32(sh, s0, s1);
          const float Sg = s0 + s1;
          __builtin_amdgcn_raw_buffer_store_b64(
              (unsigned __attribute__((ext_vector_type(2)))){__float_as_uint(lzv), __float_as_uint(Sg)}, sts,
              (wv == 0 && h == 0 && fvalid) ? (uint32_t)(f * A.in_n) * 8u : kNoStore, (uint32_t)i * 8u, 0);
          float gown[OWN];
#pragma unroll
          for (int a = 0; a < OWN; ++a) gown[a] = ccur[a] * (Q[a] - Sg);
          float* dst = Bk.glst + ((size_t)i * A.JP + j0 + h) * A.Fs + f;
#pragma unroll
          for (int a = 0; a < OWN; ++a) dst[(size_t)2 * a * A.Fs] = fvalid ? gown[a] : 0.f;
#pragma unroll
          for (int a = 0; a < OWN; ++a) {
            float g0, g1;
            xpair32(gown[a], g0, g1);
            g[2 * a] = g0;
            g[2 * a + 1] = g1;
          }
        } else if constexpr (S == 2) {
          gfma(0, TW / 2);
        } else {
          gfma(TW / 2, TW);
        }
      };
      {
        const int in = min(i + 2, i1 - 1);
        pose_prog32i<TW, 4, 6, 6>(fr, ones, unext, rs, wvo, bvo, A.wplane_b, (uint32_t)in * A.JDp * DIN * 2,
                                  (uint32_t)in * A.JDp * 8, xbuf(i + 2) + lane * 16, fill);
      }
      if (more) {
        par ^= 1;
        dots(unext, cnext, par);
        xl_wait<1 + OWN + 5 * TW + 1 + OWN>();
        __syncthreads();
      }
      }
    };
    auto step = [&](int i, f16v (&ucur)[TW], f16v (&unext)[TW], float (&ccur)[OWN], float (&cnext)[OWN])
        __attribute__((always_inline)) {
      const bool more = i + 1 < i1;
      if constexpr (XL)
        x_dma(xs_b, A.xplane_b, xsrc(i + 3), wv, xbuf(i + 3));
      const float lzv = Bk.lz[(size_t)i * A.Fs + fc];
      {
        load_c<OWN>(crow + (size_t)min(i + 1, i1 - 1) * cstep, A.Fs, cnext);
        const int in = min(i + 2, i1 - 1);
        pose_prog<DIN, TW, XL>(fr, ones, unext, rs, wvo, bvo,
                               x_voff<DIN>(in, A.N, A.lpad, A.T, A.F, f, ftt, fvalid, h, A.zero_off), h, A.wplane_b,
                               A.xplane_b, A.zero_off, (uint32_t)in * A.JDp * DIN * 2, (uint32_t)in * A.JDp * 8,
                               xbuf(i + 2) + lane * 16);
      }
      float S;
      {
        constexpr int HW = NW / 2;
        const float* slot = st + par * NW * 32;
        float sh = 0.f;
#pragma unroll
        for (int w = 0; w < HW; ++w) sh += slot[(h * HW + w) * 32 + r];
        float s0, s1;
        xpair32(sh, s0, s1);
        S = s0 + s1;
      }
      __builtin_amdgcn_raw_buffer_store_b64(
          (unsigned __attribute__((ext_vector_type(2)))){__float_as_uint(lzv), __float_as_uint(S)}, sts,
          (wv == 0 && h == 0 && fvalid) ? (uint32_t)(f * A.in_n) * 8u : kNoStore, (uint32_t)i * 8u, 0);
      float gown[OWN];
#pragma unroll
      for (int a = 0; a < OWN; ++a) gown[a] = ccur[a] * (Q[a] - S);
      {
        float* dst = Bk.glst + ((size_t)i * A.JP + j0 + h) * A.Fs + f;
#pragma unroll
        for (int a = 0; a < OWN; ++a) dst[(size_t)2 * a * A.Fs] = fvalid ? gown[a] : 0.f;
      }
      float g[CP];
#pragma unroll
      for (int a = 0; a < OWN; ++a) {
        float g0, g1;
        xpair32(gown[a], g0, g1);
        g[2 * a] = g0;
        g[2 * a + 1] = g1;
      }
#pragma unroll
      for (int t = 0; t < TW; ++t)
#pragma unroll
        for (int v = 0; v < 16; v += 2) {
          const float gv = g[kpart<DOUT>(t, v)];
          f2 a2 = {acc[t][v], acc[t][v + 1]};
          a2 += f2{gv, gv} * f2{ucur[t][v], ucur[t][v + 1]};
          acc[t][v] = a2.x;
          acc[t][v + 1] = a2.y;
        }
      if (more) {
        par ^= 1;
        dots(unext, cnext, par);
        if constexpr (XL) xl_wait<1 + OWN + 5 * TW + 1 + OWN>();
        __syncthreads();
      }
    };
    if constexpr (XL && SRF_DR_IL) {
      for (int i = i0; i < i1; i += 2) {
        step_il(i, uc, un, cc, cn);
        if (i + 1 < i1) step_il(i + 1, un, uc, cn, cc);
      }
    } else {
      for (int i = i0; i < i1; i += 2) {
        step(i, uc, un, cc, cn);
        if (i + 1 < i1) step(i + 1, un, uc, cn, cc);
      }
    }
    if constexpr (XL) xl_wait();
  }
#pragma unroll
  for (int t = 0; t < TW; ++t)
#pragma unroll
    for (int q = 0; q < 4; ++q) {
      const int row = (tbase + t) * 32 + 8 * q + 4 * h;
      if (fvalid && row < JD) {
        f4 v = {acc[t][4 * q], acc[t][4 * q + 1], acc[t][4 * q + 2], acc[t][4 * q + 3]};
        *reinterpret_cast<f4*>(A.slab + ((size_t)chunk * A.F + f) * JD + row) = v * inv;
      }
    }
}

}

namespace srf {

bool fwd32_supported(int din, int dout, int J) {
  return (din == 8 || din == 16 || din == 32) && (dout == 8 || dout == 16 || dout == 32) && din <= dout &&
         J * dout <= 32 * kTW * kMaxNW && (J * dout) % 8 == 0;
}

static int plan_tw(int din, int JD) {
  if (din <= 16) return JD <= 128 ? 2 : kTW;
  return (din == 32 && JD <= 32 * 2 * kMaxNW) ? 2 : kTW;
}

Fwd32Plan fwd32_plan(int B, int T, int N, int din, int lpad, int rpad, int J, int dout, int n_chunks) {
  Fwd32Plan p;
  const int in_n = N * (lpad + rpad + 1);
  const int JD = J * dout;
  const int NT = (JD + 31) / 32;
  p.TW = plan_tw(din, JD);
  p.NW = 1;
  while (p.NW * p.TW < NT) p.NW *= 2;
  p.JDp = p.NW * p.TW * 32;
  p.xpad = din == 32 ? 32 : 16;
  const int F = B * T;
  const int n_ftiles = (F + 31) / 32;
  const int per_cu = std::max(1, std::min(8 / p.NW, (int)(160 * 1024 / fwd32_lds(p))));
  const int slots = p.NW > 1 ? 256 * per_cu : 1024;
  int best = 1;
  double best_cost = 1e30;
  const int forced = n_chunks;
  for (int c = 1; c <= std::min(in_n, 96); ++c) {
    const int rounds = (n_ftiles * c + slots - 1) / slots;
    const int len = (in_n + c - 1) / c;
    double cost = (double)rounds * (len + 3) * (1.0 + 0.002 * c);
    if (forced > 0) cost = (c == std::min(forced, in_n)) ? 0.0 : 1.0;
    if (cost < best_cost) {
      best_cost = cost;
      best = c;
    }
  }
  p.n_chunks = best;
  p.chunk_len = (in_n + best - 1) / best;
  p.n_ftiles = n_ftiles;
  p.xplane = (size_t)F * N * din + p.xpad;
  p.ws_w = srf::align_up((size_t)2 * in_n * p.JDp * din * 2, 256);
  p.ws_b = srf::align_up((size_t)in_n * p.JDp * 4 * 2, 256);
  p.ws_x = srf::align_up((size_t)2 * p.xplane * 2, 256);
  p.ws_h = (size_t)(2 * kAbsBlocks + 64) * 4;
  p.ws_bsum = srf::align_up((size_t)best * JD * 4, 256);
  p.ws_slab = srf::align_up((size_t)best * F * JD * 4, 256);
  return p;
}

const float* fwd32_hdr(const Fwd32Plan& p, const void* planes) {
  return reinterpret_cast<const float*>(static_cast<const char*>(planes) + p.ws_w + p.ws_b + p.ws_x);
}
size_t fwd32_planes_bytes(const Fwd32Plan& p) { return p.ws_w + p.ws_b + p.ws_x + p.ws_h; }
size_t fwd32_scratch_bytes(const Fwd32Plan& p) { return p.ws_bsum + p.ws_slab; }
size_t fwd32_workspace(const Fwd32Plan& p) { return fwd32_planes_bytes(p) + fwd32_scratch_bytes(p); }
float* fwd32_slab(const Fwd32Plan& p, void* scratch) {
  return reinterpret_cast<float*>(static_cast<char*>(scratch) + p.ws_bsum);
}

size_t fwd32_lds(const Fwd32Plan& p) {
  return (size_t)p.NW * p.TW * 4 * 64 * 16 + (p.NW > 1 ? (size_t)2 * 32 * p.NW * 8 : 0);
}

int fwd32_prepare(const Fwd32Plan& p, const float* emb, const float* W, const float* bias, int B, int T, int N,
                  int din, int lpad, int rpad, int J, int dout, void* planes, void* scratch, float* WT, float* xT,
                  hipStream_t st, bool wt16, bool xt16) {
  char* base = static_cast<char*>(planes);
  float* hdr = reinterpret_cast<float*>(base + p.ws_w + p.ws_b + p.ws_x);
  const int in_n = N * (lpad + rpad + 1);
  hipLaunchKernelGGL(absmax_kernel, dim3(kAbsBlocks, 2), dim3(256), 0, st, W, (size_t)in_n * J * dout * din, emb,
                     (size_t)B * T * N * din, hdr + 64);
  SRF_LAUNCH_CHECK("absmax");
  PrepArgs P;
  P.W = W;
  P.bias = bias;
  P.emb = emb;
  P.Ws = reinterpret_cast<_Float16*>(base);
  P.bs = reinterpret_cast<__bf16*>(base + p.ws_w);
  P.xs = reinterpret_cast<_Float16*>(base + p.ws_w + p.ws_b);
  P.part = hdr + 64;
  P.hdr = hdr;
  P.bsum = reinterpret_cast<float*>(scratch);
  P.WT = WT;
  P.xT = xT;
  P.T = T;
  P.lpad = lpad;
  P.Fp = (B * T + 15) / 16 * 16;
  P.in_n = N * (lpad + rpad + 1);
  P.JD = J * dout;
  P.JDp = p.JDp;
  P.din = din;
  P.n_chunks = p.n_chunks;
  P.chunk_len = p.chunk_len;
  P.F = B * T;
  P.N = N;
  P.xplane = p.xplane;
  P.n_a = (size_t)P.in_n * p.JDp * din / 8;
  P.n_b = (size_t)P.in_n * p.JDp;
  P.n_c = (size_t)p.n_chunks * P.JD;
  P.n_d = p.xplane / 8;
  SRF_REQUIRE(!wt16 || din == 32, "prep32: split W^T planes need din 32, got %d", din);
  P.wt16 = wt16 ? 1 : 0;
  SRF_REQUIRE(!xt16 || din == 32, "prep32: split x^T planes need din 32, got %d", din);
  P.xt16 = xt16 ? 1 : 0;
  P.n_e = WT ? (size_t)P.in_n * ((P.JD + 15) / 16) * (wt16 ? 2 : 4) * din : 0;
  SRF_REQUIRE(din <= 32, "prep32: xT tile holds din <= 32, got %d", din);
  P.n_f = xT ? (size_t)P.in_n * ((P.Fp + kXtTile - 1) / kXtTile) : 0;
  P.xt_block0 = (P.n_a + P.n_b + P.n_c + P.n_d + P.n_e + 255) / 256;
  hipLaunchKernelGGL(prep32_kernel, dim3(P.xt_block0 + P.n_f), dim3(256), 0, st, P);
  SRF_LAUNCH_CHECK("prep32");
  return SRF_OK;
}

template <int DIN, int DOUT, int NW, int TW = kTW>
static int launch_rpass(const Fwd32Plan& p, const Args32& a, hipStream_t st) {
  const size_t lds = fwd32_lds(p);
  auto kern = (NW > 1 && TW <= 2) ? route_fwd32p_kernel<DIN, DOUT, (NW > 1 ? NW : 2), (TW <= 2 ? TW : 2)>
                                                    : route_fwd32_kernel<DIN, DOUT, NW, TW>;
  if (lds > 64 * 1024)
    SRF_HIP_TRY(hipFuncSetAttribute((const void*)kern, hipFuncAttributeMaxDynamicSharedMemorySize, (int)lds));
  hipLaunchKernelGGL(kern, dim3(p.n_ftiles * p.n_chunks), dim3(64 * NW), lds, st, a);
  SRF_LAUNCH_CHECK("route_fwd32");
  return SRF_OK;
}

template <int DIN, int DOUT>
static int launch_pass32_t(const Fwd32Plan& p, bool first, const Args32& a, hipStream_t st) {
  if (first) {
    Args32 b = a;
    b.n_tgroups = p.JDp / (32 * kFTW);
    const int tasks = (p.n_ftiles + kFFB - 1) / kFFB * b.n_tgroups * p.n_chunks;
    hipLaunchKernelGGL((route_fwd32_first_kernel<DIN, DOUT>), dim3((tasks + 3) / 4), dim3(256), 0, st, b);
    SRF_LAUNCH_CHECK("route_fwd32_first");
    return SRF_OK;
  }
  if constexpr (DIN <= 16) {
    if (p.TW == 2) return p.NW == 1 ? launch_rpass<DIN, DOUT, 1, 2>(p, a, st) : launch_rpass<DIN, DOUT, 2, 2>(p, a, st);
  }
  if constexpr (DIN == 32) {
    if (p.TW == 2) {
      switch (p.NW) {
        case 1: return launch_rpass<DIN, DOUT, 1, 2>(p, a, st);
        case 2: return launch_rpass<DIN, DOUT, 2, 2>(p, a, st);
        case 4: return launch_rpass<DIN, DOUT, 4, 2>(p, a, st);
        default: return launch_rpass<DIN, DOUT, 8, 2>(p, a, st);
      }
    }
  }
  switch (p.NW) {
    case 1: return launch_rpass<DIN, DOUT, 1>(p, a, st);
    case 2: return launch_rpass<DIN, DOUT, 2>(p, a, st);
    case 4: return launch_rpass<DIN, DOUT, 4>(p, a, st);
    case 8: return launch_rpass<DIN, DOUT, 8>(p, a, st);
    default: return launch_rpass<DIN, DOUT, kMaxNW>(p, a, st);
  }
}

static Args32 make_args32(const Fwd32Plan& p, const void* planes, void* scratch, int B, int T, int N, int din,
                          int lpad, int rpad, int J, int dout, int mask_first) {
  const int in_n = N * (lpad + rpad + 1);
  const char* base = static_cast<const char*>(planes);
  Args32 a{};
  a.Ws = base;
  a.bs = base + p.ws_w;
  a.xs = base + p.ws_w + p.ws_b;
  a.hdr = reinterpret_cast<const float*>(base + p.ws_w + p.ws_b + p.ws_x);
  a.ws_bytes = p.ws_w;
  a.bs_bytes = (size_t)in_n * p.JDp * 8;
  a.xs_bytes = 2 * p.xplane * 2;
  a.wplane_b = (uint32_t)((size_t)in_n * p.JDp * din * 2);
  a.xplane_b = (uint32_t)(p.xplane * 2);
  a.zero_off = (uint32_t)((p.xplane - p.xpad) * 2);
  a.F = B * T;
  a.T = T;
  a.N = N;
  a.lpad = lpad;
  a.in_n = in_n;
  a.J = J;
  a.JDp = p.JDp;
  a.n_chunks = p.n_chunks;
  a.chunk_len = p.chunk_len;
  a.mask_first = mask_first;
  a.n_tgroups = p.NW;
  a.vc = nullptr;
  a.bsum = reinterpret_cast<const float*>(scratch);
  a.slab = fwd32_slab(p, scratch);
  a.cst = nullptr;
  a.lzst = nullptr;
  a.JP = p.JDp / dout;
  a.Fs = fwd32_frame_stride(B * T);
  return a;
}

Fwd32Cpl fwd32_cpl_layout(const Fwd32Plan& p, int F, int in_n, int din, int dout, int J, int iters) {
  Fwd32Cpl c{};
  const size_t blk = (size_t)fwd32_frame_stride(F) * in_n;
  const int R1 = std::max(iters - 1, 0);
  c.c = 0;
  c.lz = (size_t)R1 * blk * (p.JDp / dout);
  size_t off = c.lz + (size_t)R1 * blk;
  off = (off + 63) / 64 * 64;
  c.planes = off;
  off += (fwd32_planes_bytes(p) + 255) / 256 * 64;
  c.WT = off;
  off += ((size_t)in_n * din * ((J * dout + 15) / 16 * 16) + 63) / 64 * 64;
  c.xT = off;
  off += ((size_t)in_n * din * ((F + 15) / 16 * 16) + 63) / 64 * 64;
  c.total = off;
  return c;
}

bool fwd32_first_full_supported(const Fwd32Plan& p, int din, int dout) {
  return din == 32 && dout == 32 && p.JDp % kFfBM == 0;
}

#ifndef SRF_FF_BN
#define SRF_FF_BN 0
#endif
static int ff_frames(int n_rt, int F) {
  if (SRF_FF_BN) return SRF_FF_BN;
  int dev = 0, cus = 256;
  if (hipGetDevice(&dev) != hipSuccess || hipDeviceGetAttribute(&cus, hipDeviceAttributeMultiprocessorCount, dev) != hipSuccess)
    cus = 256;
  for (int bn : {192, 128, 96})
    if ((long)n_rt * ((F + bn - 1) / bn) >= cus * 9 / 10) return bn;
  return 64;
}

int fwd32_first_full(const Fwd32Plan& p, const void* planes, void* scratch, int B, int T, int N, int din, int lpad,
                     int rpad, int J, int dout, int mask_first, float* s_out, float* vc_out, float* v_out,
                     hipStream_t st) {
  SRF_REQUIRE(fwd32_first_full_supported(p, din, dout), "fwd32_first_full: din %d dout %d JDp %d", din, dout, p.JDp);
  SRF_REQUIRE(2 * p.xplane * 2 < (1ull << 31) && p.ws_w < (1ull << 31), "fwd32: operand planes exceed 2 GiB");
  const Args32 a = make_args32(p, planes, scratch, B, T, N, din, lpad, rpad, J, dout, mask_first);
  const int bn = ff_frames(p.JDp / kFfBM, B * T);
  const int nb = (p.JDp / kFfBM) * ((B * T + bn - 1) / bn);
#define SRF_FF_LAUNCH(BN)                                                                                          \
  if (bn == BN) {                                                                                                 \
    constexpr int CPS_ = BN >= 96 ? 2 : 1;                                                                        \
    const size_t lds = 2 * CPS_ * (size_t)ff_stage<BN>();                                                        \
    if (lds > 64 * 1024)                                                                                          \
      SRF_HIP_TRY(hipFuncSetAttribute((const void*)route_fwd32_first_full_kernel<BN, CPS_>,                       \
                                      hipFuncAttributeMaxDynamicSharedMemorySize, (int)lds));                      \
    hipLaunchKernelGGL((route_fwd32_first_full_kernel<BN, CPS_>), dim3(nb), dim3(64 * 2 * (BN / 32)), lds, st, a, \
                       s_out, vc_out, v_out);                                                                     \
  }
  SRF_FF_LAUNCH(64)
  SRF_FF_LAUNCH(96)
  SRF_FF_LAUNCH(128)
  SRF_FF_LAUNCH(192)
#undef SRF_FF_LAUNCH
  SRF_LAUNCH_CHECK("route_fwd32_first_full");
  return SRF_OK;
}

int fwd32_pass(const Fwd32Plan& p, bool first, const void* planes, void* scratch, int B, int T,
               int N, int din, int lpad, int rpad, int J, int dout, int mask_first, const float* vc, float* cst,
               float* lzst, hipStream_t st) {
  Args32 a = make_args32(p, planes, scratch, B, T, N, din, lpad, rpad, J, dout, mask_first);
  a.vc = vc;
  a.cst = first ? nullptr : cst;
  a.lzst = first ? nullptr : lzst;
  SRF_REQUIRE(2 * p.xplane * 2 < (1ull << 31) && p.ws_w < (1ull << 31), "fwd32: operand planes exceed 2 GiB");
#define SRF_P32(DI, DO) \
  if (din == DI && dout == DO) return launch_pass32_t<DI, DO>(p, first, a, st);
  SRF_P32(8, 8)
  SRF_P32(8, 16)
  SRF_P32(8, 32)
  SRF_P32(16, 16)
  SRF_P32(16, 32)
  SRF_P32(32, 32)
#undef SRF_P32
  srf::set_error("fwd32: unsupported din %d dout %d", din, dout);
  return SRF_EUNSUPPORTED;
}

template <int DIN, int DOUT, int NW, int TW = kTW>
static int launch_bpass(const Fwd32Plan& p, const Args32& a, const Bwd32Args& b, hipStream_t st) {
  const size_t lds = fwd32_lds(p);
  auto kern = (NW > 1 && TW <= 2) ? route_bwd32p_kernel<DIN, DOUT, (NW > 1 ? NW : 2), (TW <= 2 ? TW : 2)>
                                                    : route_bwd32_kernel<DIN, DOUT, NW, TW>;
  if (lds > 64 * 1024)
    SRF_HIP_TRY(hipFuncSetAttribute((const void*)kern, hipFuncAttributeMaxDynamicSharedMemorySize, (int)lds));
  hipLaunchKernelGGL(kern, dim3(p.n_ftiles * p.n_chunks), dim3(64 * NW), lds, st, a, b);
  SRF_LAUNCH_CHECK("route_bwd32");
  return SRF_OK;
}

template <int DIN, int DOUT>
static int launch_bpass_t(const Fwd32Plan& p, const Args32& a, const Bwd32Args& b, hipStream_t st) {
  if constexpr (DIN <= 16) {
    if (p.TW == 2)
      return p.NW == 1 ? launch_bpass<DIN, DOUT, 1, 2>(p, a, b, st) : launch_bpass<DIN, DOUT, 2, 2>(p, a, b, st);
  }
  if constexpr (DIN == 32) {
    if (p.TW == 2) {
      switch (p.NW) {
        case 1: return launch_bpass<DIN, DOUT, 1, 2>(p, a, b, st);
        case 2: return launch_bpass<DIN, DOUT, 2, 2>(p, a, b, st);
        case 4: return launch_bpass<DIN, DOUT, 4, 2>(p, a, b, st);
        default: return launch_bpass<DIN, DOUT, 8, 2>(p, a, b, st);
      }
    }
  }
  switch (p.NW) {
    case 1: return launch_bpass<DIN, DOUT, 1>(p, a, b, st);
    case 2: return launch_bpass<DIN, DOUT, 2>(p, a, b, st);
    case 4: return launch_bpass<DIN, DOUT, 4>(p, a, b, st);
    case 8: return launch_bpass<DIN, DOUT, 8>(p, a, b, st);
    default: return launch_bpass<DIN, DOUT, kMaxNW>(p, a, b, st);
  }
}

int bwd32_pass(const Fwd32Plan& p, const void* planes, void* scratch, int B, int T, int N, int din, int lpad,
               int rpad, int J, int dout, const float* cst, const float* lz, const float* gs, float* stats,
               float* glst, hipStream_t st) {
  Args32 a = make_args32(p, planes, scratch, B, T, N, din, lpad, rpad, J, dout, 0);
  Bwd32Args b{cst, lz, gs, stats, glst};
#define SRF_B32(DI, DO) \
  if (din == DI && dout == DO) return launch_bpass_t<DI, DO>(p, a, b, st);
  SRF_B32(8, 8)
  SRF_B32(8, 16)
  SRF_B32(8, 32)
  SRF_B32(16, 16)
  SRF_B32(16, 32)
  SRF_B32(32, 32)
#undef SRF_B32
  srf::set_error("bwd32: unsupported din %d dout %d", din, dout);
  return SRF_EUNSUPPORTED;
}

}
```

Before: 2.779 million frames/s.

## Balance 32x32 routing passes by splitting frame-tile×input work evenly across workgroups

```diff
diff --git a/include/srf.h b/include/srf.h
--- a/include/srf.h
+++ b/include/srf.h
@@ -10,6 +10,8 @@
 const char* srf_last_error(void);
 
 int srf_route_dr_auto_chunks(int B, int T, int N, int din, int lpad, int rpad, int J, int dout);
+int srf_route_dr_split_table(int B, int T, int N, int din, int lpad, int rpad, int J, int dout, int n_chunks,
+                             int* info, int* table, int capacity);
 size_t srf_route_dr_saved_floats(int B, int T, int J, int dout, int iters);
 size_t srf_route_dr_fwd_workspace(int B, int T, int N, int din, int lpad, int rpad, int J, int dout, int iters,
                                   int n_chunks);
diff --git a/srf_amd/_lib.py b/srf_amd/_lib.py
--- a/srf_amd/_lib.py
+++ b/srf_amd/_lib.py
@@ -35,6 +35,7 @@
     'srf_set_seed_source': (_c_int, [_vp]),
     'srf_set_fault_flag': (_c_int, [_vp]),
     'srf_route_dr_auto_chunks': (_c_int, [_c_int] * 8),
+    'srf_route_dr_split_table': (_c_int, [_c_int] * 9 + [_vp, _vp, _c_int]),
     'srf_route_dr_saved_floats': (_c_size, [_c_int] * 5),
     'srf_route_dr_fwd_workspace': (_c_size, [_c_int] * 10),
     'srf_route_dr_bwd_workspace': (_c_size, [_c_int] * 10),
diff --git a/srf_amd/csrc/route_dr.hip b/srf_amd/csrc/route_dr.hip
--- a/srf_amd/csrc/route_dr.hip
+++ b/srf_amd/csrc/route_dr.hip
@@ -1613,7 +1613,19 @@
   return v;
 }
 
-__device__ __forceinline__ f4 sum_slab4(const float* __restrict__ slab, int n, size_t FJD, size_t off) {
+struct SlabSplit {
+  int n;
+  int G, U, in_n, JD;
+};
+
+__device__ __forceinline__ int slab_count(const SlabSplit& sp, size_t FJD, size_t off) {
+  if (sp.G <= 0) return sp.n;
+  const uint32_t f = FJD <= 0xffffffffu ? (uint32_t)off / (uint32_t)sp.JD : (uint32_t)(off / (size_t)sp.JD);
+  return srf::bal_tile_slots((int)(f >> 5), sp.in_n, sp.U, sp.G);
+}
+
+__device__ __forceinline__ f4 sum_slab4(const float* __restrict__ slab, const SlabSplit& sp, size_t FJD, size_t off) {
+  const int n = slab_count(sp, FJD, off);
   f4 a = ld4(slab + off);
 #pragma unroll 4
   for (int c = 1; c < n; ++c) a += ld4(slab + (size_t)c * FJD + off);
@@ -1621,25 +1633,25 @@
 }
 
 template <int DOUT>
-__global__ void fwd_finish_kernel(const float* __restrict__ slab, int n_chunks, size_t FJD,
+__global__ void fwd_finish_kernel(const float* __restrict__ slab, SlabSplit sp, size_t FJD,
                                   const float* __restrict__ vc_in, float* __restrict__ s_out,
                                   float* __restrict__ vc_out, float* __restrict__ v_out) {
   constexpr int Q = DOUT / 4;
   const size_t idx = (size_t)blockIdx.x * blockDim.x + threadIdx.x;
   const bool ok = idx < FJD / 4;
   const size_t off = (ok ? idx : 0) * 4;
-  const f4 sv = sum_slab4(slab, n_chunks, FJD, off);
+  const f4 sv = sum_slab4(slab, sp, FJD, off);
   const float n2 = qsum<Q>((sv.x * sv.x + sv.y * sv.y) + (sv.z * sv.z + sv.w * sv.w));
   if (!ok) return;
   const float fac = n2 / (1.f + n2) / sqrtf(n2 + kSquashEps);
   const f4 v = sv * fac;
   st4(s_out + off, sv);
-  st4(vc_out + off, vc_in ? v + ld4(vc_in + off) : v);
+  if (vc_out) st4(vc_out + off, vc_in ? v + ld4(vc_in + off) : v);
   if (v_out) st4(v_out + off, v);
 }
 
 template <int DOUT>
-__global__ void bwd_finish_kernel(const float* __restrict__ slab, int n_chunks, size_t FJD,
+__global__ void bwd_finish_kernel(const float* __restrict__ slab, SlabSplit sp, size_t FJD,
                                   const float* __restrict__ a_init, float* __restrict__ A,
                                   const float* __restrict__ s, float* __restrict__ gs, float* __restrict__ zero4,
                                   size_t nz4, float* __restrict__ zero1) {
@@ -1654,7 +1666,7 @@
     a = ld4(a_init + off);
     if (ok) st4(A + off, f4{0.f, 0.f, 0.f, 0.f});
   } else {
-    a = ld4(A + off) + sum_slab4(slab, n_chunks, FJD, off);
+    a = ld4(A + off) + sum_slab4(slab, sp, FJD, off);
     if (ok) st4(A + off, a);
   }
   const f4 sv = ld4(s + off);
@@ -1736,21 +1748,21 @@
 }
 
 template <int D>
-void launch_fwd_finish(const Geom& g, const float* slab, int n_chunks, const float* vc_in, float* s_out,
+void launch_fwd_finish(const Geom& g, const float* slab, const SlabSplit& sp, const float* vc_in, float* s_out,
                        float* vc_out, float* v_out, hipStream_t st) {
   const size_t FJD = (size_t)g.F() * g.JD();
-  hipLaunchKernelGGL((fwd_finish_kernel<D>), dim3((FJD / 4 + 255) / 256), dim3(256), 0, st, slab, n_chunks, FJD,
+  hipLaunchKernelGGL((fwd_finish_kernel<D>), dim3((FJD / 4 + 255) / 256), dim3(256), 0, st, slab, sp, FJD,
                      vc_in, s_out, vc_out, v_out);
 }
 
 template <int D>
-void launch_bwd_finish(const Geom& g, const float* slab, int n_chunks, const float* a_init, float* A,
+void launch_bwd_finish(const Geom& g, const float* slab, const SlabSplit& sp, const float* a_init, float* A,
                        const float* s, float* gs, hipStream_t st, float* zero = nullptr, size_t n_zero = 0,
                        float* zero1 = nullptr) {
   const size_t FJD = (size_t)g.F() * g.JD();
   const size_t nz4 = zero ? n_zero / 4 : 0;
   const size_t n = std::max(FJD / 4, nz4);
-  hipLaunchKernelGGL((bwd_finish_kernel<D>), dim3((n + 255) / 256), dim3(256), 0, st, slab, n_chunks, FJD, a_init,
+  hipLaunchKernelGGL((bwd_finish_kernel<D>), dim3((n + 255) / 256), dim3(256), 0, st, slab, sp, FJD, a_init,
                      A, s, gs, zero, nz4, zero1);
 }
 
@@ -1980,6 +1992,18 @@
 }
 
 inline bool use_fwd32(const Geom& g) { return srf::fwd32_supported(g.din, g.dout, g.J); }
+
+inline bool plan_balanced(int n_chunks) { return n_chunks > 0 && (n_chunks & srf::kBalFlag) != 0; }
+inline bool plan_arg_ok(const Geom& g, int n_chunks) {
+  return plan_balanced(n_chunks) ? use_fwd32(g) : (n_chunks >= 1 && n_chunks <= g.in_n());
+}
+inline int legacy_chunks(const Geom& g, int n_chunks) {
+  return plan_balanced(n_chunks) ? auto_chunks(g, pass_cfg(g).NW) : n_chunks;
+}
+inline SlabSplit uniform_split(int n) { return SlabSplit{n, 0, 0, 0, 0}; }
+inline SlabSplit pass_split(const Geom& g, const srf::Fwd32Plan& p) {
+  return p.bal_G > 0 ? SlabSplit{p.n_slots, p.bal_G, p.bal_U, g.in_n(), g.JD()} : uniform_split(p.n_chunks);
+}
 
 inline bool coupling_sizes_fit(const Geom& g) {
   constexpr size_t kLim = size_t(1) << 31;
@@ -2058,10 +2082,11 @@
     }
     SRF_LAUNCH_CHECK("route_pass(fwd)");
     if (r < nev) SRF_HIP_TRY(hipEventRecord(ev1[r], st));
+    const bool last = r == g.iters - 1;
     launch_fwd_finish<D>(g, p32 ? srf::fwd32_slab(plan, scratch) : slab,
-                         p32 ? plan.n_chunks : n_chunks, vc,
-                         saved + (size_t)(2 * r) * FJD, saved + (size_t)(2 * r + 1) * FJD,
-                         r == g.iters - 1 ? v_out : nullptr, st);
+                         !p32 ? uniform_split(n_chunks) : r == 0 ? uniform_split(plan.n_chunks) : pass_split(g, plan),
+                         vc, saved + (size_t)(2 * r) * FJD, last ? nullptr : saved + (size_t)(2 * r + 1) * FJD,
+                         last ? v_out : nullptr, st);
     SRF_LAUNCH_CHECK("fwd_finish");
   }
   return SRF_OK;
@@ -2084,7 +2109,7 @@
     off += srf::align_up(nfloat * sizeof(float), 256);
     return o;
   };
-  const size_t oA = take(F * JD), ogs = take((size_t)g.iters * F * JD), oslab = take((size_t)n_chunks * F * JD),
+  const size_t oA = take(F * JD), ogs = take((size_t)g.iters * F * JD), oslab = take((size_t)legacy_chunks(g, n_chunks) * F * JD),
                ostats = take((size_t)(g.iters - 1) * F * in_n * 2), ogu = take(in_n * (size_t)g.NT() * 16 * Fp),
                oxt = take(in_n * g.din * Fp), owt = take(in_n * JD * g.din);
   size_t op32 = 0, ogl = 0, ogwp = 0;
@@ -2158,7 +2183,7 @@
   const int Fp = padded_frames(g);
   const bool p32 = couplings != nullptr && w.p32 != nullptr && R > 1;
   const size_t n_emb = (size_t)g.F() * g.N * g.din;
-  launch_bwd_finish<D>(g, nullptr, n_chunks, g_v, w.A, saved + (size_t)(2 * (R - 1)) * FJD,
+  launch_bwd_finish<D>(g, nullptr, uniform_split(1), g_v, w.A, saved + (size_t)(2 * (R - 1)) * FJD,
                        w.gs + (size_t)(R - 1) * FJD, st, p32 ? g_emb : nullptr, n_emb, p32 ? w.gumax : nullptr);
   SRF_LAUNCH_CHECK("bwd_finish");
   srf::Fwd32Plan plan{};
@@ -2178,13 +2203,13 @@
                                      couplings + cl.lz + (size_t)(r - 1) * blk,
                                      w.gs + (size_t)r * FJD, stats_r, w.gl + (size_t)(r - 1) * blk * JP, st);
       if (rc) return rc;
-      launch_bwd_finish<D>(g, srf::fwd32_slab(plan, w.p32), plan.n_chunks, nullptr, w.A,
+      launch_bwd_finish<D>(g, srf::fwd32_slab(plan, w.p32), pass_split(g, plan), nullptr, w.A,
                              saved + (size_t)(2 * (r - 1)) * FJD, w.gs + (size_t)(r - 1) * FJD, st);
     } else {
-      dispatch_pass<D, MODE_BWD>(g, pc, n_chunks, emb, W, bias, r, vc, w.gs + (size_t)r * FJD, w.slab, stats_r, 1,
-                                 st);
+      const int lc = legacy_chunks(g, n_chunks);
+      dispatch_pass<D, MODE_BWD>(g, pc, lc, emb, W, bias, r, vc, w.gs + (size_t)r * FJD, w.slab, stats_r, 1, st);
       SRF_LAUNCH_CHECK("route_pass(bwd)");
-      launch_bwd_finish<D>(g, w.slab, n_chunks, nullptr, w.A, saved + (size_t)(2 * (r - 1)) * FJD,
+      launch_bwd_finish<D>(g, w.slab, uniform_split(lc), nullptr, w.A, saved + (size_t)(2 * (r - 1)) * FJD,
                            w.gs + (size_t)(r - 1) * FJD, st);
     }
     SRF_LAUNCH_CHECK("bwd_finish");
@@ -2219,8 +2244,49 @@
 
 int srf_route_dr_auto_chunks(int B, int T, int N, int din, int lpad, int rpad, int J, int dout) {
   Geom g{B, T, N, din, lpad, rpad, J, dout, 1, 0};
-  if (use_fwd32(g)) return srf::fwd32_plan(B, T, N, din, lpad, rpad, J, dout).n_chunks;
+  if (use_fwd32(g)) return srf::fwd32_plan(B, T, N, din, lpad, rpad, J, dout).plan_arg;
   return auto_chunks(g, pass_cfg(g).NW);
+}
+
+int srf_route_dr_split_table(int B, int T, int N, int din, int lpad, int rpad, int J, int dout, int n_chunks,
+                             int* info, int* table, int capacity) {
+  Geom g{B, T, N, din, lpad, rpad, J, dout, 1, 0};
+  SRF_REQUIRE(B > 0 && T > 0 && N > 0 && lpad >= 0 && rpad >= 0 && use_fwd32(g), "split_table: not a 32x32-pass shape");
+  SRF_REQUIRE(n_chunks == 0 || plan_arg_ok(g, n_chunks), "split_table: bad plan argument %d", n_chunks);
+  SRF_REQUIRE(info != nullptr && capacity >= 0 && (table != nullptr || capacity == 0), "split_table: null argument");
+  const srf::Fwd32Plan p = srf::fwd32_plan(B, T, N, din, lpad, rpad, J, dout, n_chunks);
+  const int in_n = g.in_n();
+  const bool bal = p.bal_G > 0;
+  const int n_wg = bal ? p.bal_G : p.n_ftiles * p.n_chunks;
+  info[0] = bal ? 1 : 0;
+  info[1] = n_wg;
+  info[2] = p.n_ftiles * in_n;
+  info[3] = p.n_slots;
+  info[4] = p.plan_arg;
+  int n = 0;
+  auto emit = [&](int w, int ft, int i0, int i1, int slot) {
+    if (n < capacity) {
+      int* row = table + (size_t)n * 5;
+      row[0] = w, row[1] = ft, row[2] = i0, row[3] = i1, row[4] = slot;
+    }
+    ++n;
+  };
+  for (int w = 0; w < n_wg; ++w) {
+    if (!bal) {
+      const int ft = w / p.n_chunks, slot = w - ft * p.n_chunks;
+      const int i0 = slot * p.chunk_len;
+      emit(w, ft, std::min(i0, in_n), std::min(in_n, i0 + p.chunk_len), slot);
+      continue;
+    }
+    int u = srf::bal_first(w, p.bal_U, p.bal_G);
+    const int u1 = srf::bal_first(w + 1, p.bal_U, p.bal_G);
+    while (u < u1) {
+      const int ft = u / in_n, i0 = u - ft * in_n, i1 = std::min(in_n, i0 + (u1 - u));
+      emit(w, ft, i0, i1, w - srf::bal_owner(ft * in_n, p.bal_U, p.bal_G));
+      u += i1 - i0;
+    }
+  }
+  return n;
 }
 
 size_t srf_route_dr_saved_floats(int B, int T, int J, int dout, int iters) {
@@ -2230,8 +2296,8 @@
 size_t srf_route_dr_fwd_workspace(int B, int T, int N, int din, int lpad, int rpad, int J, int dout, int iters,
                                   int n_chunks) {
   (void)iters;
-  size_t need = (size_t)n_chunks * ((size_t)B * T + 1) * J * dout * sizeof(float);
   Geom g{B, T, N, din, lpad, rpad, J, dout, 1, 0};
+  size_t need = plan_balanced(n_chunks) ? 0 : (size_t)n_chunks * ((size_t)B * T + 1) * J * dout * sizeof(float);
   if (use_fwd32(g))
     need = std::max(need, srf::fwd32_workspace(srf::fwd32_plan(B, T, N, din, lpad, rpad, J, dout, n_chunks)));
   return need;
@@ -2264,7 +2330,8 @@
   int rc = check_geom(g);
   if (rc) return rc;
   SRF_REQUIRE(emb && W && bias && v_out && saved && workspace, "null pointer argument");
-  SRF_REQUIRE(n_chunks >= 1 && n_chunks <= g.in_n(), "n_chunks %d out of [1, %d]", n_chunks, g.in_n());
+  SRF_REQUIRE(plan_arg_ok(g, n_chunks), "n_chunks %d: neither in [1, %d] nor a balanced plan of the 32x32 passes",
+              n_chunks, g.in_n());
   const size_t need = srf_route_dr_fwd_workspace(B, T, N, din, lpad, rpad, J, dout, iters, n_chunks);
   if (workspace_bytes < need) {
     srf::set_error("forward workspace too small: %zu < %zu", workspace_bytes, need);
@@ -2290,7 +2357,8 @@
   int rc = check_geom(g);
   if (rc) return rc;
   SRF_REQUIRE(emb && W && bias && saved && g_v && g_emb && g_W && g_bias && workspace, "null pointer argument");
-  SRF_REQUIRE(n_chunks >= 1 && n_chunks <= g.in_n(), "n_chunks %d out of [1, %d]", n_chunks, g.in_n());
+  SRF_REQUIRE(plan_arg_ok(g, n_chunks), "n_chunks %d: neither in [1, %d] nor a balanced plan of the 32x32 passes",
+              n_chunks, g.in_n());
   BwdWs w = bwd_layout(g, n_chunks, workspace);
   if (workspace_bytes < w.bytes) {
     srf::set_error("backward workspace too small: %zu < %zu", workspace_bytes, w.bytes);
@@ -2359,7 +2427,8 @@
   int rc = check_geom(g);
   if (rc) return rc;
   SRF_REQUIRE(emb && g_W && g_bias && workspace, "null pointer argument");
-  SRF_REQUIRE(n_chunks >= 1 && n_chunks <= g.in_n(), "n_chunks %d out of [1, %d]", n_chunks, g.in_n());
+  SRF_REQUIRE(plan_arg_ok(g, n_chunks), "n_chunks %d: neither in [1, %d] nor a balanced plan of the 32x32 passes",
+              n_chunks, g.in_n());
   BwdWs w = bwd_layout(g, n_chunks, workspace);
   if (workspace_bytes < w.bytes) {
     srf::set_error("backward workspace too small: %zu < %zu", workspace_bytes, w.bytes);
diff --git a/srf_amd/csrc/route_fwd32.h b/srf_amd/csrc/route_fwd32.h
--- a/srf_amd/csrc/route_fwd32.h
+++ b/srf_amd/csrc/route_fwd32.h
@@ -1,11 +1,23 @@
 #pragma once
 #include <hip/hip_runtime.h>
 #include <cstddef>
+#include <cstdint>
 
 namespace srf {
 
 constexpr int kFwd32TW = 4;
 __host__ __device__ inline int fwd32_frame_stride(int F) { return (F + 31) / 32 * 32; }
+
+__host__ __device__ inline int bal_first(int w, int U, int G) {
+  return (int)((uint32_t)w * (uint32_t)U / (uint32_t)G);
+}
+__host__ __device__ inline int bal_owner(int u, int U, int G) {
+  return (int)((((uint32_t)u + 1u) * (uint32_t)G - 1u) / (uint32_t)U);
+}
+__host__ __device__ inline int bal_tile_slots(int ft, int in_n, int U, int G) {
+  return bal_owner((ft + 1) * in_n - 1, U, G) - bal_owner(ft * in_n, U, G) + 1;
+}
+constexpr int kBalFlag = 1 << 20;
 
 struct Fwd32Plan {
   int NW;
@@ -13,6 +25,9 @@
   int JDp;
   int xpad;
   int n_chunks, chunk_len, n_ftiles;
+  int bal_G, bal_U;
+  int n_slots;
+  int plan_arg;
   size_t xplane;
   size_t ws_w, ws_b, ws_x, ws_h, ws_bsum, ws_slab;
 };
diff --git a/srf_amd/csrc/route_fwd32.hip b/srf_amd/csrc/route_fwd32.hip
--- a/srf_amd/csrc/route_fwd32.hip
+++ b/srf_amd/csrc/route_fwd32.hip
@@ -10,6 +10,10 @@
 
 #ifndef SRF_DR_IL
 #define SRF_DR_IL 1
+#endif
+
+#ifndef SRF_DR_BAL_AUTO
+#define SRF_DR_BAL_AUTO 1
 #endif
 
 namespace {
@@ -586,6 +590,58 @@
   float* cst;
   float* lzst;
   int JP, Fs;
+  int bal_G, bal_U;
+};
+
+struct Seg32 {
+  int ft, i0, i1, slot;
+};
+
+typedef const __attribute__((address_space(4))) char* kernarg_ptr;
+template <class T>
+__device__ __forceinline__ const __attribute__((address_space(4))) T* kernarg_reload(uint32_t off) {
+  kernarg_ptr p = (kernarg_ptr)__builtin_amdgcn_kernarg_segment_ptr();
+  asm volatile("" : "+s"(p));
+  return (const __attribute__((address_space(4))) T*)(p + off);
+}
+
+template <class ArgsT>
+__device__ __forceinline__ Seg32 seg32_at(const ArgsT& A, int bid, int u, int u1) {
+  int ft, i0, i1, slot;
+  if (A.bal_G > 0) {
+    ft = (int)((uint32_t)u / (uint32_t)A.in_n);
+    i0 = u - ft * A.in_n;
+    i1 = min(A.in_n, i0 + (u1 - u));
+    slot = bid - srf::bal_owner(ft * A.in_n, A.bal_U, A.bal_G);
+  } else {
+    ft = bid / A.n_chunks;
+    slot = bid - ft * A.n_chunks;
+    i0 = slot * A.chunk_len;
+    i1 = min(A.in_n, i0 + A.chunk_len);
+  }
+  return Seg32{__builtin_amdgcn_readfirstlane(ft), __builtin_amdgcn_readfirstlane(i0),
+               __builtin_amdgcn_readfirstlane(i1), __builtin_amdgcn_readfirstlane(slot)};
+}
+
+struct SegWalk {
+  int u;
+  __device__ __forceinline__ SegWalk(const Args32& A) : u(0) {
+    if (A.bal_G > 0) u = __builtin_amdgcn_readfirstlane(srf::bal_first((int)blockIdx.x, A.bal_U, A.bal_G));
+  }
+  __device__ __forceinline__ Seg32 seg() const {
+    const auto* K = kernarg_reload<Args32>(0);
+    const int bid = blockIdx.x;
+    return seg32_at(*K, bid, u, K->bal_G > 0 ? srf::bal_first(bid + 1, K->bal_U, K->bal_G) : 0);
+  }
+  __device__ __forceinline__ bool next(const Seg32& sg) {
+    const auto* K = kernarg_reload<Args32>(0);
+    if (K->bal_G <= 0) return false;
+    u += sg.i1 - sg.i0;
+    if (u >= __builtin_amdgcn_readfirstlane(srf::bal_first((int)blockIdx.x + 1, K->bal_U, K->bal_G))) return false;
+    asm volatile("s_waitcnt vmcnt(0)" ::: "memory");
+    __syncthreads();
+    return true;
+  }
 };
 
 
@@ -872,40 +928,41 @@
   constexpr int CP = TW * 32 / DOUT;
   constexpr int OWN = CP / 2;
   extern __shared__ __attribute__((aligned(16))) float lds[];
-  const int JD = A.J * DOUT;
-  const int lane = threadIdx.x & 63, wv = threadIdx.x >> 6;
+  const int wv = threadIdx.x >> 6;
   const int wvu = __builtin_amdgcn_readfirstlane(wv);
-  const int r = lane & 31, h = lane >> 5;
-  const int bid = blockIdx.x;
-  const int ft = bid / A.n_chunks, chunk = bid - ft * A.n_chunks;
-  const int f = ft * 32 + r;
-  const int fc = min(f, A.F - 1);
-  const int fb = fc / A.T, ftt = fc - fb * A.T;
-  const bool fvalid = f < A.F;
-  const int i0 = chunk * A.chunk_len, i1 = min(A.in_n, i0 + A.chunk_len);
   const int tbase = __builtin_amdgcn_readfirstlane(wv * TW);
   const int j0 = tbase * 32 / DOUT;
   const Rsrc3 rs{make_rsrc(A.Ws, A.ws_bytes), make_rsrc(A.bs, A.bs_bytes), make_rsrc(A.xs, A.xs_bytes)};
   if (DIN <= 16 && NW > 1 && wv >= NW / 2) __builtin_amdgcn_s_setprio(1);
-  const uint32_t wvo = (uint32_t)(((tbase * 32 + r) * DIN + (DIN >= 16 ? 8 * h : 0)) * 2);
-  const uint32_t bvo = (uint32_t)((tbase * 32 + r) * 8);
   const __amdgpu_buffer_rsrc_t crs = make_rsrc(A.cst, A.cst ? (size_t)A.in_n * A.JP * A.Fs * 4 : 0);
   const __amdgpu_buffer_rsrc_t lzs = make_rsrc(A.lzst, A.cst ? (size_t)A.in_n * A.Fs * 4 : 0);
 
-  f4* vcl = reinterpret_cast<f4*>(lds) + (size_t)wv * TW * 4 * 64;
+  f4* vcl = reinterpret_cast<f4*>(lds) + (size_t)tbase * 4 * 64;
   float2* st = reinterpret_cast<float2*>(lds + (size_t)NW * TW * 4 * 64 * 4);
   constexpr bool XJ = DIN == 32 && NW > 1;
   __shared__ __attribute__((aligned(16))) char xls[XJ ? 2 * 4 * kXlPiece : 16];
   const char* xs_b = static_cast<const char*>(A.xs);
+  auto xbuf = [&](int c) { return xls + (c & 1) * 4 * kXlPiece; };
+  for (SegWalk sw(A);;) {
+  const Seg32 sg = sw.seg();
+  const int ft = sg.ft, i0 = sg.i0, i1 = sg.i1;
+  const int lane = lane_asm(), r = lane & 31, h = lane >> 5;
+  const uint32_t wvo = (uint32_t)(((tbase * 32 + r) * DIN + (DIN >= 16 ? 8 * h : 0)) * 2);
+  const uint32_t bvo = (uint32_t)((tbase * 32 + r) * 8);
+  const int JD = kernarg_reload<Args32>(0)->J * DOUT;
+  const int Tk = kernarg_reload<Args32>(0)->T;
+  const int f = ft * 32 + r;
+  const int fc = min(f, A.F - 1);
+  const int fb = fc / Tk, ftt = fc - fb * Tk;
+  const bool fvalid = f < A.F;
   auto xsrc = [&](int c) { return x_voff<DIN>(min(c, i1 - 1), A.N, A.lpad, A.T, A.F, f, ftt, fvalid, h, A.zero_off); };
-  auto xbuf = [&](int c) { return xls + (c & 1) * 4 * kXlPiece; };
 #pragma unroll
   for (int t = 0; t < TW; ++t)
 #pragma unroll
     for (int q = 0; q < 4; ++q) {
       const int row = (tbase + t) * 32 + 8 * q + 4 * h;
       f4 v = {0.f, 0.f, 0.f, 0.f};
-      if (fvalid && row < JD) v = *reinterpret_cast<const f4*>(A.vc + (size_t)f * JD + row);
+      if (fvalid && row < JD) v = *reinterpret_cast<const f4*>(kernarg_reload<Args32>(0)->vc + (size_t)f * JD + row);
       vcl[(t * 4 + q) * 64 + lane] = v;
     }
   float mk[OWN];
@@ -1070,16 +1127,24 @@
         }
     }
   }
-#pragma unroll
-  for (int t = 0; t < TW; ++t)
-#pragma unroll
-    for (int q = 0; q < 4; ++q) {
-      const int row = (tbase + t) * 32 + 8 * q + 4 * h;
-      if (fvalid && row < JD) {
-        f4 v = {acc[t][4 * q], acc[t][4 * q + 1], acc[t][4 * q + 2], acc[t][4 * q + 3]};
-        *reinterpret_cast<f4*>(A.slab + ((size_t)chunk * A.F + f) * JD + row) = v * inv;
-      }
-    }
+  {
+    const auto* K = kernarg_reload<Args32>(0);
+    const int JD = K->J * DOUT;
+    const int le = lane_asm(), fe = ft * 32 + (le & 31), he = le >> 5;
+    float* const sl = K->slab + (size_t)sg.slot * A.F * JD;
+#pragma unroll
+    for (int t = 0; t < TW; ++t)
+#pragma unroll
+      for (int q = 0; q < 4; ++q) {
+        const int row = (tbase + t) * 32 + 8 * q + 4 * he;
+        if (fe < A.F && row < JD) {
+          f4 v = {acc[t][4 * q], acc[t][4 * q + 1], acc[t][4 * q + 2], acc[t][4 * q + 3]};
+          *reinterpret_cast<f4*>(sl + (size_t)fe * JD + row) = v * inv;
+        }
+      }
+  }
+  if (!sw.next(sg)) break;
+  }
 }
 
 
@@ -1089,16 +1154,8 @@
   constexpr int OWN = CP / 2;
   static_assert(NW > 1, "the pipelined pass exchanges softmax stats between waves");
   extern __shared__ __attribute__((aligned(16))) float lds[];
-  const int JD = A.J * DOUT;
   const int lane = threadIdx.x & 63, wv = threadIdx.x >> 6;
   const int r = lane & 31, h = lane >> 5;
-  const int bid = blockIdx.x;
-  const int ft = bid / A.n_chunks, chunk = bid - ft * A.n_chunks;
-  const int f = ft * 32 + r;
-  const int fc = min(f, A.F - 1);
-  const int fb = fc / A.T, ftt = fc - fb * A.T;
-  const bool fvalid = f < A.F;
-  const int i0 = chunk * A.chunk_len, i1 = min(A.in_n, i0 + A.chunk_len);
   const int tbase = __builtin_amdgcn_readfirstlane(wv * TW);
   const int j0 = tbase * 32 / DOUT;
   const Rsrc3 rs{make_rsrc(A.Ws, A.ws_bytes), make_rsrc(A.bs, A.bs_bytes), make_rsrc(A.xs, A.xs_bytes)};
@@ -1112,15 +1169,23 @@
   __shared__ __attribute__((aligned(16))) char xls[XL ? 2 * 4 * kXlPiece : 16];
   char* xb = xls;
   const char* xs_b = static_cast<const char*>(A.xs);
+  auto xbuf = [&](int c) { return xb + (c & 1) * 4 * kXlPiece; };
+  for (SegWalk sw(A);;) {
+  const Seg32 sg = sw.seg();
+  const int ft = sg.ft, i0 = sg.i0, i1 = sg.i1;
+  const int JD = kernarg_reload<Args32>(0)->J * DOUT;
+  const int f = ft * 32 + r;
+  const int fc = min(f, A.F - 1);
+  const int fb = fc / A.T, ftt = fc - fb * A.T;
+  const bool fvalid = f < A.F;
   auto xsrc = [&](int c) { return x_voff<DIN>(min(c, i1 - 1), A.N, A.lpad, A.T, A.F, f, ftt, fvalid, h, A.zero_off); };
-  auto xbuf = [&](int c) { return xb + (c & 1) * 4 * kXlPiece; };
 #pragma unroll
   for (int t = 0; t < TW; ++t)
 #pragma unroll
     for (int q = 0; q < 4; ++q) {
       const int row = (tbase + t) * 32 + 8 * q + 4 * h;
       f4 v = {0.f, 0.f, 0.f, 0.f};
-      if (fvalid && row < JD) v = *reinterpret_cast<const f4*>(A.vc + (size_t)f * JD + row);
+      if (fvalid && row < JD) v = *reinterpret_cast<const f4*>(kernarg_reload<Args32>(0)->vc + (size_t)f * JD + row);
       vcr[t][q] = v;
     }
   float mk[OWN];
@@ -1331,16 +1396,24 @@
     }
     if constexpr (XL) xl_wait();
   }
-#pragma unroll
-  for (int t = 0; t < TW; ++t)
-#pragma unroll
-    for (int q = 0; q < 4; ++q) {
-      const int row = (tbase + t) * 32 + 8 * q + 4 * h;
-      if (fvalid && row < JD) {
-        f4 v = {acc[t][4 * q], acc[t][4 * q + 1], acc[t][4 * q + 2], acc[t][4 * q + 3]};
-        *reinterpret_cast<f4*>(A.slab + ((size_t)chunk * A.F + f) * JD + row) = v * inv;
-      }
-    }
+  {
+    const auto* K = kernarg_reload<Args32>(0);
+    const int JD = K->J * DOUT;
+    const int le = lane_asm(), fe = ft * 32 + (le & 31), he = le >> 5;
+    float* const sl = K->slab + (size_t)sg.slot * A.F * JD;
+#pragma unroll
+    for (int t = 0; t < TW; ++t)
+#pragma unroll
+      for (int q = 0; q < 4; ++q) {
+        const int row = (tbase + t) * 32 + 8 * q + 4 * he;
+        if (fe < A.F && row < JD) {
+          f4 v = {acc[t][4 * q], acc[t][4 * q + 1], acc[t][4 * q + 2], acc[t][4 * q + 3]};
+          *reinterpret_cast<f4*>(sl + (size_t)fe * JD + row) = v * inv;
+        }
+      }
+  }
+  if (!sw.next(sg)) break;
+  }
 }
 
 struct Bwd32Args {
@@ -1363,39 +1436,40 @@
   constexpr int CP = TW * 32 / DOUT;
   constexpr int OWN = CP / 2;
   extern __shared__ __attribute__((aligned(16))) float lds[];
-  const int JD = A.J * DOUT;
-  const int lane = threadIdx.x & 63, wv = threadIdx.x >> 6;
+  const int wv = threadIdx.x >> 6;
   const int wvu = __builtin_amdgcn_readfirstlane(wv);
-  const int r = lane & 31, h = lane >> 5;
-  const int bid = blockIdx.x;
-  const int ft = bid / A.n_chunks, chunk = bid - ft * A.n_chunks;
-  const int f = ft * 32 + r;
-  const int fc = min(f, A.F - 1);
-  const int fb = fc / A.T, ftt = fc - fb * A.T;
-  const bool fvalid = f < A.F;
-  const int i0 = chunk * A.chunk_len, i1 = min(A.in_n, i0 + A.chunk_len);
   const int tbase = __builtin_amdgcn_readfirstlane(wv * TW);
   const int j0 = tbase * 32 / DOUT;
   const Rsrc3 rs{make_rsrc(A.Ws, A.ws_bytes), make_rsrc(A.bs, A.bs_bytes), make_rsrc(A.xs, A.xs_bytes)};
   if (DIN <= 16 && NW > 1 && wv >= NW / 2) __builtin_amdgcn_s_setprio(1);
-  const uint32_t wvo = (uint32_t)(((tbase * 32 + r) * DIN + (DIN >= 16 ? 8 * h : 0)) * 2);
-  const uint32_t bvo = (uint32_t)((tbase * 32 + r) * 8);
   const __amdgpu_buffer_rsrc_t lzr = make_rsrc(Bk.lz, (size_t)A.in_n * A.Fs * 4);
 
-  f4* gsl = reinterpret_cast<f4*>(lds) + (size_t)wv * TW * 4 * 64;
+  f4* gsl = reinterpret_cast<f4*>(lds) + (size_t)tbase * 4 * 64;
   float* st = lds + (size_t)NW * TW * 4 * 64 * 4;
   constexpr bool XJ = DIN == 32 && NW > 1;
   __shared__ __attribute__((aligned(16))) char xls[XJ ? 2 * 4 * kXlPiece : 16];
   const char* xs_b = static_cast<const char*>(A.xs);
+  auto xbuf = [&](int c) { return xls + (c & 1) * 4 * kXlPiece; };
+  for (SegWalk sw(A);;) {
+  const Seg32 sg = sw.seg();
+  const int ft = sg.ft, i0 = sg.i0, i1 = sg.i1;
+  const int lane = lane_asm(), r = lane & 31, h = lane >> 5;
+  const uint32_t wvo = (uint32_t)(((tbase * 32 + r) * DIN + (DIN >= 16 ? 8 * h : 0)) * 2);
+  const uint32_t bvo = (uint32_t)((tbase * 32 + r) * 8);
+  const int JD = kernarg_reload<Args32>(0)->J * DOUT;
+  const int Tk = kernarg_reload<Args32>(0)->T;
+  const int f = ft * 32 + r;
+  const int fc = min(f, A.F - 1);
+  const int fb = fc / Tk, ftt = fc - fb * Tk;
+  const bool fvalid = f < A.F;
   auto xsrc = [&](int c) { return x_voff<DIN>(min(c, i1 - 1), A.N, A.lpad, A.T, A.F, f, ftt, fvalid, h, A.zero_off); };
-  auto xbuf = [&](int c) { return xls + (c & 1) * 4 * kXlPiece; };
 #pragma unroll
   for (int t = 0; t < TW; ++t)
 #pragma unroll
     for (int q = 0; q < 4; ++q) {
       const int row = (tbase + t) * 32 + 8 * q + 4 * h;
       f4 v = {0.f, 0.f, 0.f, 0.f};
-      if (fvalid && row < JD) v = *reinterpret_cast<const f4*>(Bk.gs + (size_t)f * JD + row);
+      if (fvalid && row < JD) v = *reinterpret_cast<const f4*>(kernarg_reload<Bwd32Args>(sizeof(Args32))->gs + (size_t)f * JD + row);
       gsl[(t * 4 + q) * 64 + lane] = v;
     }
   const bf8 ones = ones_frag(h);
@@ -1549,16 +1623,24 @@
         }
     }
   }
-#pragma unroll
-  for (int t = 0; t < TW; ++t)
-#pragma unroll
-    for (int q = 0; q < 4; ++q) {
-      const int row = (tbase + t) * 32 + 8 * q + 4 * h;
-      if (fvalid && row < JD) {
-        f4 v = {acc[t][4 * q], acc[t][4 * q + 1], acc[t][4 * q + 2], acc[t][4 * q + 3]};
-        *reinterpret_cast<f4*>(A.slab + ((size_t)chunk * A.F + f) * JD + row) = v * inv;
-      }
-    }
+  {
+    const auto* K = kernarg_reload<Args32>(0);
+    const int JD = K->J * DOUT;
+    const int le = lane_asm(), fe = ft * 32 + (le & 31), he = le >> 5;
+    float* const sl = K->slab + (size_t)sg.slot * A.F * JD;
+#pragma unroll
+    for (int t = 0; t < TW; ++t)
+#pragma unroll
+      for (int q = 0; q < 4; ++q) {
+        const int row = (tbase + t) * 32 + 8 * q + 4 * he;
+        if (fe < A.F && row < JD) {
+          f4 v = {acc[t][4 * q], acc[t][4 * q + 1], acc[t][4 * q + 2], acc[t][4 * q + 3]};
+          *reinterpret_cast<f4*>(sl + (size_t)fe * JD + row) = v * inv;
+        }
+      }
+  }
+  if (!sw.next(sg)) break;
+  }
 }
 
 
@@ -1569,16 +1651,8 @@
   constexpr int OWN = CP / 2;
   static_assert(NW > 1, "the pipelined pass exchanges sigma partials between waves");
   extern __shared__ __attribute__((aligned(16))) float lds[];
-  const int JD = A.J * DOUT;
   const int lane = threadIdx.x & 63, wv = threadIdx.x >> 6;
   const int r = lane & 31, h = lane >> 5;
-  const int bid = blockIdx.x;
-  const int ft = bid / A.n_chunks, chunk = bid - ft * A.n_chunks;
-  const int f = ft * 32 + r;
-  const int fc = min(f, A.F - 1);
-  const int fb = fc / A.T, ftt = fc - fb * A.T;
-  const bool fvalid = f < A.F;
-  const int i0 = chunk * A.chunk_len, i1 = min(A.in_n, i0 + A.chunk_len);
   const int tbase = __builtin_amdgcn_readfirstlane(wv * TW);
   const int j0 = tbase * 32 / DOUT;
   const Rsrc3 rs{make_rsrc(A.Ws, A.ws_bytes), make_rsrc(A.bs, A.bs_bytes), make_rsrc(A.xs, A.xs_bytes)};
@@ -1590,15 +1664,23 @@
   __shared__ __attribute__((aligned(16))) char xls[XL ? 2 * 4 * kXlPiece : 16];
   char* xb = xls;
   const char* xs_b = static_cast<const char*>(A.xs);
+  auto xbuf = [&](int c) { return xb + (c & 1) * 4 * kXlPiece; };
+  for (SegWalk sw(A);;) {
+  const Seg32 sg = sw.seg();
+  const int ft = sg.ft, i0 = sg.i0, i1 = sg.i1;
+  const int JD = kernarg_reload<Args32>(0)->J * DOUT;
+  const int f = ft * 32 + r;
+  const int fc = min(f, A.F - 1);
+  const int fb = fc / A.T, ftt = fc - fb * A.T;
+  const bool fvalid = f < A.F;
   auto xsrc = [&](int c) { return x_voff<DIN>(min(c, i1 - 1), A.N, A.lpad, A.T, A.F, f, ftt, fvalid, h, A.zero_off); };
-  auto xbuf = [&](int c) { return xb + (c & 1) * 4 * kXlPiece; };
 #pragma unroll
   for (int t = 0; t < TW; ++t)
 #pragma unroll
     for (int q = 0; q < 4; ++q) {
       const int row = (tbase + t) * 32 + 8 * q + 4 * h;
       f4 v = {0.f, 0.f, 0.f, 0.f};
-      if (fvalid && row < JD) v = *reinterpret_cast<const f4*>(Bk.gs + (size_t)f * JD + row);
+      if (fvalid && row < JD) v = *reinterpret_cast<const f4*>(kernarg_reload<Bwd32Args>(sizeof(Args32))->gs + (size_t)f * JD + row);
       gsl[(t * 4 + q) * 64 + lane] = v;
     }
   const bf8 ones = ones_frag(h);
@@ -1795,16 +1877,24 @@
     }
     if constexpr (XL) xl_wait();
   }
-#pragma unroll
-  for (int t = 0; t < TW; ++t)
-#pragma unroll
-    for (int q = 0; q < 4; ++q) {
-      const int row = (tbase + t) * 32 + 8 * q + 4 * h;
-      if (fvalid && row < JD) {
-        f4 v = {acc[t][4 * q], acc[t][4 * q + 1], acc[t][4 * q + 2], acc[t][4 * q + 3]};
-        *reinterpret_cast<f4*>(A.slab + ((size_t)chunk * A.F + f) * JD + row) = v * inv;
-      }
-    }
+  {
+    const auto* K = kernarg_reload<Args32>(0);
+    const int JD = K->J * DOUT;
+    const int le = lane_asm(), fe = ft * 32 + (le & 31), he = le >> 5;
+    float* const sl = K->slab + (size_t)sg.slot * A.F * JD;
+#pragma unroll
+    for (int t = 0; t < TW; ++t)
+#pragma unroll
+      for (int q = 0; q < 4; ++q) {
+        const int row = (tbase + t) * 32 + 8 * q + 4 * he;
+        if (fe < A.F && row < JD) {
+          f4 v = {acc[t][4 * q], acc[t][4 * q + 1], acc[t][4 * q + 2], acc[t][4 * q + 3]};
+          *reinterpret_cast<f4*>(sl + (size_t)fe * JD + row) = v * inv;
+        }
+      }
+  }
+  if (!sw.next(sg)) break;
+  }
 }
 
 }
@@ -1833,15 +1923,17 @@
   p.xpad = din == 32 ? 32 : 16;
   const int F = B * T;
   const int n_ftiles = (F + 31) / 32;
+  constexpr int kSegCost = 3;
   const int per_cu = std::max(1, std::min(8 / p.NW, (int)(160 * 1024 / fwd32_lds(p))));
   const int slots = p.NW > 1 ? 256 * per_cu : 1024;
   int best = 1;
   double best_cost = 1e30;
-  const int forced = n_chunks;
+  const bool force_bal = n_chunks > 0 && (n_chunks & kBalFlag) != 0;
+  const int forced = force_bal ? 0 : n_chunks;
   for (int c = 1; c <= std::min(in_n, 96); ++c) {
     const int rounds = (n_ftiles * c + slots - 1) / slots;
     const int len = (in_n + c - 1) / c;
-    double cost = (double)rounds * (len + 3) * (1.0 + 0.002 * c);
+    double cost = (double)rounds * (len + kSegCost) * (1.0 + 0.002 * c);
     if (forced > 0) cost = (c == std::min(forced, in_n)) ? 0.0 : 1.0;
     if (cost < best_cost) {
       best_cost = cost;
@@ -1851,13 +1943,37 @@
   p.n_chunks = best;
   p.chunk_len = (in_n + best - 1) / best;
   p.n_ftiles = n_ftiles;
+  p.bal_G = 0;
+  p.bal_U = 0;
+  p.n_slots = best;
+  p.plan_arg = best;
+  {
+    const long long U = (long long)n_ftiles * in_n;
+    long long G = force_bal ? (n_chunks & (kBalFlag - 1)) : 0;
+    if (G <= 0) G = slots;
+    G = std::min(G, U);
+    const bool fits = U * (G + 1) < (1ll << 31);
+    if (fits && forced <= 0) {
+      const int len = (int)((U + G - 1) / G);
+      const int segs = (len - 1 + in_n - 1) / in_n + 1;
+      int n_slots = 1;
+      for (int ft = 0; ft < n_ftiles; ++ft) n_slots = std::max(n_slots, bal_tile_slots(ft, in_n, (int)U, (int)G));
+      const double cost = (double)(len + kSegCost * segs) * (1.0 + 0.002 * n_slots);
+      if (force_bal || (SRF_DR_BAL_AUTO && din == 32 && p.NW > 1 && p.TW == 2 && cost < best_cost)) {
+        p.bal_G = (int)G;
+        p.bal_U = (int)U;
+        p.n_slots = n_slots;
+        p.plan_arg = kBalFlag | (int)G;
+      }
+    }
+  }
   p.xplane = (size_t)F * N * din + p.xpad;
   p.ws_w = srf::align_up((size_t)2 * in_n * p.JDp * din * 2, 256);
   p.ws_b = srf::align_up((size_t)in_n * p.JDp * 4 * 2, 256);
   p.ws_x = srf::align_up((size_t)2 * p.xplane * 2, 256);
   p.ws_h = (size_t)(2 * kAbsBlocks + 64) * 4;
   p.ws_bsum = srf::align_up((size_t)best * JD * 4, 256);
-  p.ws_slab = srf::align_up((size_t)best * F * JD * 4, 256);
+  p.ws_slab = srf::align_up((size_t)std::max(best, p.n_slots) * F * JD * 4, 256);
   return p;
 }
 
@@ -1932,7 +2048,7 @@
                                                     : route_fwd32_kernel<DIN, DOUT, NW, TW>;
   if (lds > 64 * 1024)
     SRF_HIP_TRY(hipFuncSetAttribute((const void*)kern, hipFuncAttributeMaxDynamicSharedMemorySize, (int)lds));
-  hipLaunchKernelGGL(kern, dim3(p.n_ftiles * p.n_chunks), dim3(64 * NW), lds, st, a);
+  hipLaunchKernelGGL(kern, dim3(p.bal_G > 0 ? p.bal_G : p.n_ftiles * p.n_chunks), dim3(64 * NW), lds, st, a);
   SRF_LAUNCH_CHECK("route_fwd32");
   return SRF_OK;
 }
@@ -2002,6 +2118,8 @@
   a.lzst = nullptr;
   a.JP = p.JDp / dout;
   a.Fs = fwd32_frame_stride(B * T);
+  a.bal_G = p.bal_G;
+  a.bal_U = p.bal_U;
   return a;
 }
 
@@ -2095,7 +2213,7 @@
                                                     : route_bwd32_kernel<DIN, DOUT, NW, TW>;
   if (lds > 64 * 1024)
     SRF_HIP_TRY(hipFuncSetAttribute((const void*)kern, hipFuncAttributeMaxDynamicSharedMemorySize, (int)lds));
-  hipLaunchKernelGGL(kern, dim3(p.n_ftiles * p.n_chunks), dim3(64 * NW), lds, st, a, b);
+  hipLaunchKernelGGL(kern, dim3(p.bal_G > 0 ? p.bal_G : p.n_ftiles * p.n_chunks), dim3(64 * NW), lds, st, a, b);
   SRF_LAUNCH_CHECK("route_bwd32");
   return SRF_OK;
 }
```

After: 2.830 million frames/s (median of 6 runs). 1.8% higher.
